# Marcus-Forte/moptimizer_0

Hardware: NVIDIA B200
Metric: point2point_linearized_residuals_per_sec (higher is better)
Workload: dtype f32

## Files before the change

include/mopt_capi.h:

```cpp
#ifndef MOPT_CAPI_H
#define MOPT_CAPI_H

#ifndef __CUDACC_RTC__
#include <stdint.h>
#endif

#ifdef __cplusplus
extern "C" {
#endif

#define MOPT_MAX_PARAMETERS 16
#define MOPT_MAX_OUTPUTS 4
#define MOPT_MAX_COSTS 8
#define MOPT_MAX_TRACE 1024
#define MOPT_NCCL_ID_BYTES 128

#if defined(__GNUC__)
#define MOPT_API __attribute__((visibility("default")))
#else
#define MOPT_API
#endif

typedef struct mopt_ctx mopt_ctx;
typedef struct mopt_store mopt_store;

typedef enum mopt_status {
  MOPT_OK = 0,
  MOPT_ERR_INVALID_ARGUMENT = 1,
  MOPT_ERR_CUDA = 2,
  MOPT_ERR_COMM = 3,
  MOPT_ERR_UNSUPPORTED = 4,
  MOPT_ERR_OUT_OF_MEMORY = 5
} mopt_status;

typedef enum mopt_optimization_status {
  MOPT_CONVERGED = 0,
  MOPT_MAXIMUM_ITERATIONS_REACHED = 1,
  MOPT_SMALL_DELTA = 2,
  MOPT_NUMERIC_ERROR = 3,
  MOPT_FATAL_ERROR = 4
} mopt_optimization_status;

typedef enum mopt_dtype { MOPT_F32 = 0, MOPT_F64 = 1 } mopt_dtype;

typedef enum mopt_model {
  MOPT_MODEL_POINT2POINT = 0,
  MOPT_MODEL_EXP_CURVE = 1,
  MOPT_MODEL_MICHAELIS_MENTEN = 2,
  MOPT_MODEL_PINHOLE = 3,
  MOPT_MODEL_POWELL = 4,
  MOPT_MODEL_POINT_DIST = 5,
  MOPT_MODEL_PINHOLE_DISTORT = 6,
  MOPT_MODEL_COUNT_
} mopt_model;
#define MOPT_MODEL_USER_BASE 1000

typedef enum mopt_jacobian {
  MOPT_JAC_ANALYTICAL = 0,
  MOPT_JAC_FORWARD = 1,
  MOPT_JAC_CENTRAL = 2
} mopt_jacobian;

typedef enum mopt_p2p_variant {
  MOPT_P2P_EXACT = 0,
  MOPT_P2P_REFTEST = 1,
  MOPT_P2P_REFTEST_COLMAJOR = 2,
  MOPT_P2P_LEFT = 3
} mopt_p2p_variant;

typedef enum mopt_manifold { MOPT_MANIFOLD_ADDITIVE = 0, MOPT_MANIFOLD_SO3_LEFT = 1 } mopt_manifold;

typedef enum mopt_loss {
  MOPT_LOSS_NONE = 0,
  MOPT_LOSS_GEMAN_MCCLURE = 1,
  MOPT_LOSS_HUBER = 2
} mopt_loss;

typedef struct mopt_problem {
  int32_t model;
  int32_t variant;
  int32_t num_parameters;
  int32_t num_outputs;
  int32_t jacobian;
  int32_t compute_dtype;
  int32_t loss;
  int32_t has_covariance;
  double loss_param;
  double covariance[MOPT_MAX_OUTPUTS * MOPT_MAX_OUTPUTS];
  double consts[32];
  int32_t manifold;
  int32_t flags;
} mopt_problem;
typedef enum mopt_problem_flags {
  MOPT_FLAG_GENERIC_KERNEL = 1,
  MOPT_FLAG_STABLE_FD = 2,
  MOPT_FLAG_REFERENCE_FLOAT_GUARD = 4
} mopt_problem_flags;

typedef struct mopt_lm_options {
  int32_t max_iterations;
  int32_t lm_max_iterations;
  double lambda_factor;
  int32_t scalar_dtype;
  int32_t speculative;
  int32_t flags;
  int32_t reserved;
} mopt_lm_options;
typedef enum mopt_lm_flags { MOPT_LM_STAGNATION_STOP = 1 } mopt_lm_flags;

typedef struct mopt_lm_trial {
  int32_t outer_iteration, k, accepted, reserved;
  double y0, yi, rho, lambda, nu;
} mopt_lm_trial;

typedef struct mopt_lm_report {
  int32_t status;
  int32_t executed_iterations;
  int32_t num_trials;
  int32_t num_passes;
  double final_cost;
  mopt_lm_trial trials[MOPT_MAX_TRACE];
} mopt_lm_report;

typedef struct mopt_synth {
  uint64_t seed;
  int64_t first_index;
  double gt[MOPT_MAX_PARAMETERS];
  double lo[3], hi[3];
  int64_t n_total;
  double noise_sigma;
  double outlier_fraction, outlier_range;
  double consts[32];
} mopt_synth;

MOPT_API const char* mopt_last_error(void);
MOPT_API const char* mopt_version(void);
MOPT_API int mopt_device_count(int* count);

MOPT_API int mopt_ctx_create(int device, mopt_ctx** out);
MOPT_API int mopt_ctx_create_sharded(int device, int rank, int world_size, const void* nccl_unique_id, mopt_ctx** out);
MOPT_API int mopt_comm_unique_id(void* out_id);
#define MOPT_PEER_HANDLE_BYTES 64
MOPT_API int mopt_ctx_peer_handle(mopt_ctx* ctx, void* out_handle);
MOPT_API int mopt_ctx_open_peers(mopt_ctx* ctx, const void* handles_in_rank_order);
MOPT_API int mopt_ctx_set_exchange_enabled(mopt_ctx* ctx, int enabled);
MOPT_API int mopt_ctx_destroy(mopt_ctx* ctx);
MOPT_API int mopt_ctx_synchronize(mopt_ctx* ctx);
MOPT_API int mopt_ctx_stream(mopt_ctx* ctx, uint64_t* out_stream);
MOPT_API int mopt_ctx_set_launch(mopt_ctx* ctx, int ctas_per_sm, int threads);

MOPT_API int mopt_store_create(mopt_ctx* ctx, int model, int dtype, int64_t n, mopt_store** out);
MOPT_API int mopt_store_destroy(mopt_store* store);
MOPT_API int mopt_store_size(const mopt_store* store, int64_t* n);
MOPT_API int mopt_store_upload(mopt_store* store, int group, const void* host, int host_dtype, int64_t host_stride,
                      int64_t first, int64_t count);
MOPT_API int mopt_store_download(mopt_store* store, int group, void* host, int host_dtype, int64_t first, int64_t count);
MOPT_API int mopt_store_generate(mopt_store* store, const mopt_synth* desc);

MOPT_API int mopt_linearize(mopt_ctx* ctx, mopt_store* store, const mopt_problem* problem, const double* x, double* H,
                   double* b, double* sum);
MOPT_API int mopt_compute_cost(mopt_ctx* ctx, mopt_store* store, const mopt_problem* problem, const double* x, double* sum);
MOPT_API int mopt_linearize_async(mopt_ctx* ctx, mopt_store* store, const mopt_problem* problem, const double* x);
MOPT_API int mopt_ctx_result(mopt_ctx* ctx, int num_parameters, double* H, double* b, double* sum);

MOPT_API int mopt_upload_and_linearize(mopt_ctx* ctx, mopt_store* store, const mopt_problem* problem, const void* host_a,
                              const void* host_b, int host_dtype, int64_t count, const double* x, double* H,
                              double* b, double* sum);

MOPT_API int mopt_lm_minimize(mopt_ctx* ctx, int n_costs, mopt_store* const* stores, const mopt_problem* problems,
                     const mopt_lm_options* options, double* x, mopt_lm_report* report);
MOPT_API void mopt_lm_default_options(mopt_lm_options* options);

MOPT_API int mopt_so3_convert6dof(const double* x, double* T16_rowmajor);
MOPT_API int mopt_ldlt_solve(int n, const double* A_colmajor, const double* rhs, double* out);

typedef struct mopt_nn_index mopt_nn_index;
MOPT_API int mopt_nn_index_create(mopt_ctx* ctx, const void* host_xyz, int host_dtype, int index_dtype, int64_t m,
                                  double max_distance, mopt_nn_index** out);
MOPT_API int mopt_nn_index_destroy(mopt_nn_index* index);
MOPT_API int mopt_store_set_target(mopt_store* store, mopt_nn_index* index);
MOPT_API int mopt_store_reassociate(mopt_store* store, const double* x, int64_t* matched);

MOPT_API int mopt_cloud_read_text(const char* path, int columns, int keep, int host_dtype, int pinned, void** out,
                                  int64_t* n);
MOPT_API int mopt_cloud_write_binary(const char* path, const void* data, int host_dtype, int keep, int64_t n);
MOPT_API int mopt_cloud_read_binary(const char* path, int pinned, int* host_dtype, int* keep, void** out, int64_t* n);
MOPT_API int mopt_cloud_free(void* ptr, int pinned);

typedef struct mopt_user_model_desc {
  int32_t num_parameters;
  int32_t num_outputs;
// ... 29 lines not shown
```

moptimizer_0_b200/capi.py:

```python
from __future__ import annotations

import ctypes as C
import os
from typing import Optional, Sequence

import numpy as np

_PKG = os.path.dirname(os.path.abspath(__file__))
LIB_PATH = os.path.join(_PKG, "libmopt_b200.so")

MAX_PARAMETERS, MAX_OUTPUTS, MAX_COSTS, MAX_TRACE, NCCL_ID_BYTES = 16, 4, 8, 1024, 128
OK = 0
F32, F64 = 0, 1
(MODEL_POINT2POINT, MODEL_EXP_CURVE, MODEL_MICHAELIS_MENTEN, MODEL_PINHOLE, MODEL_POWELL,
 MODEL_POINT_DIST, MODEL_PINHOLE_DISTORT) = range(7)
JAC_ANALYTICAL, JAC_FORWARD, JAC_CENTRAL = range(3)
P2P_EXACT, P2P_REFTEST, P2P_REFTEST_COLMAJOR, P2P_LEFT = range(4)
MANIFOLD_ADDITIVE, MANIFOLD_SO3_LEFT = 0, 1
FLAG_GENERIC_KERNEL = 1
FLAG_STABLE_FD = 2
FLAG_REFERENCE_FLOAT_GUARD = 4
LM_STAGNATION_STOP = 1
LOSS_NONE, LOSS_GEMAN_MCCLURE, LOSS_HUBER = range(3)
STATUS = ["CONVERGED", "MAXIMUM_ITERATIONS_REACHED", "SMALL_DELTA", "NUMERIC_ERROR", "FATAL_ERROR"]
MODEL_SHAPE = {
    MODEL_POINT2POINT: (6, 3, 3, 3), MODEL_EXP_CURVE: (2, 1, 1, 1), MODEL_MICHAELIS_MENTEN: (2, 1, 1, 1),
    MODEL_PINHOLE: (6, 2, 3, 2), MODEL_POWELL: (4, 4, 0, 0), MODEL_POINT_DIST: (0, 3, 3, 3),
    MODEL_PINHOLE_DISTORT: (15, 2, 3, 2),
}

EXPORTS = [
    "mopt_last_error", "mopt_version", "mopt_device_count", "mopt_ctx_create", "mopt_ctx_create_sharded",
    "mopt_comm_unique_id", "mopt_ctx_destroy", "mopt_ctx_synchronize", "mopt_ctx_stream", "mopt_ctx_set_launch",
    "mopt_store_create", "mopt_store_destroy", "mopt_store_size", "mopt_store_upload", "mopt_store_download",
    "mopt_store_generate", "mopt_linearize", "mopt_compute_cost", "mopt_linearize_async", "mopt_ctx_result",
    "mopt_upload_and_linearize", "mopt_lm_minimize", "mopt_lm_default_options", "mopt_so3_convert6dof",
    "mopt_ldlt_solve", "mopt_host_alloc", "mopt_host_free",
    "mopt_cloud_read_text", "mopt_cloud_write_binary", "mopt_cloud_read_binary", "mopt_cloud_free",
    "mopt_nn_index_create", "mopt_nn_index_destroy", "mopt_store_set_target", "mopt_store_reassociate",
    "mopt_ctx_peer_handle", "mopt_ctx_open_peers", "mopt_ctx_set_exchange_enabled",
    "mopt_user_model_compile", "mopt_user_model_release", "mopt_user_model_log",
    "mopt_measure_peaks", "mopt_measure_h2d",
]
MODEL_USER_BASE = 1000
PEER_HANDLE_BYTES = 64


class Problem(C.Structure):
    _fields_ = [("model", C.c_int32), ("variant", C.c_int32), ("num_parameters", C.c_int32),
                ("num_outputs", C.c_int32), ("jacobian", C.c_int32), ("compute_dtype", C.c_int32),
                ("loss", C.c_int32), ("has_covariance", C.c_int32), ("loss_param", C.c_double),
                ("covariance", C.c_double * (MAX_OUTPUTS * MAX_OUTPUTS)), ("consts", C.c_double * 32),
                ("manifold", C.c_int32), ("flags", C.c_int32)]


class LmOptions(C.Structure):
    _fields_ = [("max_iterations", C.c_int32), ("lm_max_iterations", C.c_int32), ("lambda_factor", C.c_double),
                ("scalar_dtype", C.c_int32), ("speculative", C.c_int32), ("flags", C.c_int32),
                ("reserved", C.c_int32)]


class LmTrial(C.Structure):
    _fields_ = [("outer_iteration", C.c_int32), ("k", C.c_int32), ("accepted", C.c_int32), ("reserved", C.c_int32),
                ("y0", C.c_double), ("yi", C.c_double), ("rho", C.c_double), ("lambda_", C.c_double),
                ("nu", C.c_double)]


_TRIAL_DTYPE = np.dtype([("outer_iteration", "<i4"), ("k", "<i4"), ("accepted", "<i4"), ("reserved", "<i4"),
                         ("y0", "<f8"), ("yi", "<f8"), ("rho", "<f8"), ("lambda_", "<f8"), ("nu", "<f8")])


class LmReport(C.Structure):
    _fields_ = [("status", C.c_int32), ("executed_iterations", C.c_int32), ("num_trials", C.c_int32),
                ("num_passes", C.c_int32), ("final_cost", C.c_double), ("trials", LmTrial * MAX_TRACE)]


class Synth(C.Structure):
    _fields_ = [("seed", C.c_uint64), ("first_index", C.c_int64), ("gt", C.c_double * MAX_PARAMETERS),
                ("lo", C.c_double * 3), ("hi", C.c_double * 3), ("n_total", C.c_int64),
                ("noise_sigma", C.c_double), ("outlier_fraction", C.c_double), ("outlier_range", C.c_double),
                ("consts", C.c_double * 32)]


class UserModelDesc(C.Structure):
    _fields_ = [("num_parameters", C.c_int32), ("num_outputs", C.c_int32), ("ncomp_a", C.c_int32),
                ("ncomp_b", C.c_int32), ("has_jacobian", C.c_int32), ("set_size", C.c_int32),
                ("rot_offset", C.c_int32), ("reserved", C.c_int32)]


class Peaks(C.Structure):
    _fields_ = [("fp32_fma_tflops", C.c_double), ("fp32_fma2_tflops", C.c_double),
                ("issue_gwarp_inst_per_s", C.c_double), ("hbm_read_gbs", C.c_double), ("reserved", C.c_double * 4)]


class MoptError(RuntimeError):
    def __init__(self, code: int, msg: str):
        super().__init__(f"mopt error {code}: {msg}")
        self.code = code


_lib = None


def lib():
    global _lib
# ... 128 lines not shown
    @property
    def handle(self):
        return self._h

    def peer_handle(self) -> bytes:
        buf = C.create_string_buffer(PEER_HANDLE_BYTES)
        check(lib().mopt_ctx_peer_handle(self._h, C.cast(buf, C.c_void_p)))
        return buf.raw

    def open_peers(self, handles_in_rank_order: Sequence[bytes]):
        blob = b"".join(bytes(h) for h in handles_in_rank_order)
        buf = C.create_string_buffer(blob, len(blob))
        check(lib().mopt_ctx_open_peers(self._h, C.cast(buf, C.c_void_p)))

    def set_exchange_enabled(self, enabled: bool):
        check(lib().mopt_ctx_set_exchange_enabled(self._h, 1 if enabled else 0))

    def synchronize(self):
        check(lib().mopt_ctx_synchronize(self._h))

    def stream(self) -> int:
        s = C.c_uint64(0)
        check(lib().mopt_ctx_stream(self._h, C.byref(s)))
        return s.value

    def measure_peaks(self) -> dict:
        p = Peaks()
        check(lib().mopt_measure_peaks(self._h, C.byref(p)))
        return {"fp32_fma_tflops": p.fp32_fma_tflops, "fp32_fma2_tflops": p.fp32_fma2_tflops,
                "issue_gwarp_inst_per_s": p.issue_gwarp_inst_per_s, "hbm_read_gbs": p.hbm_read_gbs}

    def measure_h2d(self, nbytes: int = 1 << 30, seconds: float = 1.0) -> float:
        g = C.c_double(0)
        check(lib().mopt_measure_h2d(self._h, int(nbytes), float(seconds), C.byref(g)))
        return g.value

    def set_launch(self, ctas_per_sm: int = 0, threads: int = 0):
        check(lib().mopt_ctx_set_launch(self._h, ctas_per_sm, threads))

    def close(self):
        if self._h:
            lib().mopt_ctx_destroy(self._h)
            self._h = C.c_void_p()

    def linearize(self, store: "Store", problem: Problem, x):
        P = problem.num_parameters
        xs = np.ascontiguousarray(np.asarray(x, dtype=np.float64))
        H = np.zeros((P, P), dtype=np.float64)
        b = np.zeros(P, dtype=np.float64)
        s = C.c_double(0)
        check(lib().mopt_linearize(self._h, store.handle, C.byref(problem), _dp(xs), _dp(H), _dp(b), C.byref(s)))
        return H, b, s.value

    def compute_cost(self, store: "Store", problem: Problem, x) -> float:
        xs = np.ascontiguousarray(np.asarray(x if len(x) else [0.0], dtype=np.float64))
        s = C.c_double(0)
        check(lib().mopt_compute_cost(self._h, store.handle, C.byref(problem), _dp(xs), C.byref(s)))
        return s.value

    def linearize_async(self, store: "Store", problem: Problem, xs: np.ndarray):
        check(lib().mopt_linearize_async(self._h, store.handle, C.byref(problem), _dp(xs)))

    def result(self, P: int):
        H = np.zeros((P, P), dtype=np.float64)
        b = np.zeros(P, dtype=np.float64)
        s = C.c_double(0)
        check(lib().mopt_ctx_result(self._h, P, _dp(H), _dp(b), C.byref(s)))
        return H, b, s.value

    def upload_and_linearize(self, store: "Store", problem: Problem, host_a: np.ndarray, host_b: np.ndarray, x):
        assert host_a.dtype == host_b.dtype and host_a.dtype in (np.float32, np.float64)
        P = problem.num_parameters
        xs = np.ascontiguousarray(np.asarray(x, dtype=np.float64))
        H = np.zeros((P, P), dtype=np.float64)
        b = np.zeros(P, dtype=np.float64)
        s = C.c_double(0)
        dt = F32 if host_a.dtype == np.float32 else F64
        check(lib().mopt_upload_and_linearize(self._h, store.handle, C.byref(problem), host_a.ctypes.data,
                                              host_b.ctypes.data, dt, store.n, _dp(xs), _dp(H), _dp(b), C.byref(s)))
        return H, b, s.value

    def lm_minimize(self, stores: Sequence["Store"], problems: Sequence[Problem], x0, max_iterations: int = 15,
                    lm_iterations: int = 3, scalar_dtype: int = F64, speculative: bool = True,
                    stagnation_stop: bool = True) -> "LmResult":
        n = len(stores)
        hs = (C.c_void_p * n)(*[s.handle for s in stores])
        ps = (Problem * n)(*problems)
        opt = self.__dict__.get("_lm_options")
        if opt is None:
            opt = self._lm_options = LmOptions()
            lib().mopt_lm_default_options(C.byref(opt))
        opt.max_iterations, opt.lm_max_iterations = max_iterations, lm_iterations
        opt.scalar_dtype, opt.speculative = scalar_dtype, 1 if speculative else 0
        opt.flags = LM_STAGNATION_STOP if stagnation_stop else 0
        x = np.array(x0, dtype=np.float64)
        rep = self.__dict__.get("_lm_report")
        if rep is None:
            rep = self._lm_report = LmReport()
        check(lib().mopt_lm_minimize(self._h, n, hs, ps, C.byref(opt), _dp(x), C.byref(rep)))
        return LmResult(x, rep)


class LmResult:
    def __init__(self, x: np.ndarray, rep: LmReport):
        self.x = x
        self.status = STATUS[rep.status]
        self.executed_iterations = rep.executed_iterations
        self.num_passes = rep.num_passes
        self.final_cost = rep.final_cost
        self._raw = C.string_at(C.addressof(rep) + LmReport.trials.offset, rep.num_trials * _TRIAL_DTYPE.itemsize)
        self._trials_arr = None
        self._trace = None

    @property
    def _trials(self) -> np.ndarray:
        if self._trials_arr is None:
            self._trials_arr = np.frombuffer(self._raw, dtype=_TRIAL_DTYPE)
        return self._trials_arr

    @property
    def trace(self) -> np.ndarray:
        if self._trace is None:
            t = self._trials
            self._trace = np.stack([t[f].astype(np.float64) for f in
                                    ("outer_iteration", "k", "y0", "yi", "rho", "lambda_", "nu", "accepted")],
                                   axis=1).reshape(len(t), 8)
        return self._trace

    @property
    def sequence(self) -> str:
        return "".join("A" if a else "R" for a in self._trials["accepted"])


class Store:

    def __init__(self, ctx: Context, model: int, n: int, dtype: int = F32):
        self.ctx, self.model, self.n, self.dtype = ctx, model, int(n), dtype
        self._h = C.c_void_p()
        check(lib().mopt_store_create(ctx.handle, model, dtype, int(n), C.byref(self._h)))

    @property
    def handle(self):
        return self._h

    def upload(self, group: int, host: np.ndarray, first: int = 0, stride: int = 0):
        host = np.ascontiguousarray(host)
        if host.dtype not in (np.float32, np.float64):
            host = host.astype(np.float64)
        ncomp = MODEL_SHAPE[self.model][2 + group]
        count = host.size // (stride if stride else ncomp)
        dt = F32 if host.dtype == np.float32 else F64
        check(lib().mopt_store_upload(self._h, group, host.ctypes.data, dt, stride, first, count))

    def download(self, group: int, dtype=np.float64, first: int = 0, count: Optional[int] = None) -> np.ndarray:
        ncomp = MODEL_SHAPE[self.model][2 + group]
        count = self.n - first if count is None else count
        out = np.zeros((count, ncomp), dtype=dtype)
        dt = F32 if out.dtype == np.float32 else F64
        check(lib().mopt_store_download(self._h, group, out.ctypes.data, dt, first, count))
        return out

    def generate(self, seed: int, gt: Sequence[float], lo=(0, 0, 0), hi=(10, 10, 10), first_index: int = 0,
                 n_total: int = 0, noise_sigma: float = 0.0, outlier_fraction: float = 0.0,
                 outlier_range: float = 0.0, consts=None):
        d = Synth()
        d.seed, d.first_index, d.n_total = seed, first_index, n_total
        for i, v in enumerate(gt):
            d.gt[i] = float(v)
        for k in range(3):
            d.lo[k], d.hi[k] = float(lo[k]), float(hi[k])
        d.noise_sigma, d.outlier_fraction, d.outlier_range = noise_sigma, outlier_fraction, outlier_range
        if consts is not None:
            for i, v in enumerate(np.asarray(consts, dtype=np.float64).reshape(-1)):
                d.consts[i] = float(v)
        check(lib().mopt_store_generate(self._h, C.byref(d)))

    def close(self):
# ... 82 lines not shown
```

moptimizer_0_b200/csrc/mopt_capi.cu:

```cuda
#include <dlfcn.h>

#include <cmath>
#include <atomic>
#include <chrono>
#include <cstdlib>
#include <cstring>
#include <mutex>

#include "mopt_internal.h"

using namespace mopt;

namespace {
thread_local std::string g_last_error;
}
namespace mopt {
void set_last_error(const std::string& msg) { g_last_error = msg; }
int store_upload_async(mopt_store* st, int group, const void* host, int host_dtype, int64_t host_stride, int64_t first,
                       int64_t count);
}

namespace {
struct NcclApi {
  typedef struct ncclComm* comm_t;
  struct unique_id { char internal[MOPT_NCCL_ID_BYTES]; };
  int (*GetUniqueId)(unique_id*) = nullptr;
  int (*CommInitRank)(comm_t*, int, unique_id, int) = nullptr;
  int (*CommDestroy)(comm_t) = nullptr;
  int (*AllReduce)(const void*, void*, size_t, int, int, comm_t, cudaStream_t) = nullptr;
  const char* (*GetErrorString)(int) = nullptr;
  bool ok = false;
  std::string why;
};
NcclApi& nccl() {
  static NcclApi api;
  static std::once_flag once;
  std::call_once(once, [] {
    const char* names[] = {getenv("MOPT_NCCL_LIB"), "libnccl.so.2", "libnccl.so"};
    void* h = nullptr;
    for (const char* n : names) {
      if (!n) continue;
      h = dlopen(n, RTLD_NOW | RTLD_GLOBAL);
      if (h) break;
    }
    if (!h) {
      api.why = std::string("cannot dlopen libnccl: ") + (dlerror() ? dlerror() : "?");
      return;
    }
    api.GetUniqueId = reinterpret_cast<decltype(api.GetUniqueId)>(dlsym(h, "ncclGetUniqueId"));
    api.CommInitRank = reinterpret_cast<decltype(api.CommInitRank)>(dlsym(h, "ncclCommInitRank"));
    api.CommDestroy = reinterpret_cast<decltype(api.CommDestroy)>(dlsym(h, "ncclCommDestroy"));
    api.AllReduce = reinterpret_cast<decltype(api.AllReduce)>(dlsym(h, "ncclAllReduce"));
    api.GetErrorString = reinterpret_cast<decltype(api.GetErrorString)>(dlsym(h, "ncclGetErrorString"));
    api.ok = api.GetUniqueId && api.CommInitRank && api.CommDestroy && api.AllReduce && api.GetErrorString;
    if (!api.ok) api.why = "libnccl is missing required symbols";
  });
  return api;
}
constexpr int kNcclFloat64 = 8;
constexpr int kNcclSum = 0;

#define MOPT_NCCL_TRY(expr)                                                                       \
  do {                                                                                            \
    int _r = (expr);                                                                              \
    if (_r != 0) {                                                                                \
      set_last_error(std::string(#expr) + " failed: " + nccl().GetErrorString(_r));               \
      return MOPT_ERR_COMM;                                                                       \
    }                                                                                             \
  } while (0)
}

namespace {

__global__ void setup_kernel(CostSlot* slot, XArg x) { setup_cost(slot->cost, x.v, &slot->pb, threadIdx.x, blockDim.x); }

__global__ void lm_init_kernel(LmState* st, CostSlot* slots, LmInit in) {
  __shared__ LmStepShared s_sh;
  lm_init_warp(st, slots, in, &s_sh, threadIdx.x);
}

__device__ long long g_step_prof[8];

__global__ void lm_step_kernel(LmState* st, const PassResult* trial, CostSlot* slots, int* flag, const int* xerr, int prof,
                               int P, int scalar_f32) {
  __shared__ LmStepShared s_sh;
  const int lane = threadIdx.x;
  if (*reinterpret_cast<const volatile int*>(xerr)) {
    if (lane == 0) {
      if (!st->done) lm_finish(st, MOPT_FATAL_ERROR);
      *flag = 1;
    }
    return;
  }
  long long stamps[16] = {0};
  const int done = lm_step_warp(st, trial, slots, &s_sh, lane, P, scalar_f32 != 0, LmStepIo{}, prof ? stamps : nullptr);
  if (lane == 0) {
    *flag = done;
    if (prof && stamps[3] - stamps[2] > 1000)
      for (int i = 0; i < 6; ++i) g_step_prof[i] = stamps[i];
  }
}

__global__ void ldlt_warp_test_kernel(int n, const double* A, const double* rhs, double* out) {
  __shared__ LmSolveScratch sc;
  const int lane = threadIdx.x;
  for (int i = lane; i < n * n; i += 32) sc.A[i] = A[i];
  if (lane < n) sc.nb[lane] = rhs[lane];
  __syncwarp();
  if (n == 6) ldlt_solve_warp<double, 6>(n, sc.A, sc.nb, sc.d, sc.tmp, sc.y, sc.tr, lane);
  else ldlt_solve_warp<double>(n, sc.A, sc.nb, sc.d, sc.tmp, sc.y, sc.tr, lane);
  if (lane < n) out[lane] = sc.d[lane];
}

__global__ void peer_reduce_kernel(XSlot* local, int world, unsigned long long seq, PassResult* out, int npk,
                                   const int* mode_ptr, int mode_override, int* err, int* err_dev) {
  const int mode = mode_override >= 0 ? mode_override : *mode_ptr;
  if (mode == PASS_SKIP) return;
  if (*reinterpret_cast<const volatile int*>(err_dev)) return;
  const int base = int(seq & 1ull) * kMaxWorld;
  __shared__ int s_ok;
  if (threadIdx.x == 0) {
    bool ok = true;
    const long long t0 = clock64();
    for (int r = 0; r < world && ok; ++r) {
      const unsigned long long* flag = &local[base + r].seq;
      for (;;) {
        unsigned long long v;
        asm volatile("ld.acquire.sys.global.u64 %0, [%1];" : "=l"(v) : "l"(flag) : "memory");
        if (v == seq) break;
        if (clock64() - t0 > 20000000000LL) {
          ok = false;
          break;
        }
        __nanosleep(64);
      }
    }
    if (!ok) {
      *err = 1;
      *err_dev = 1;
    }
    s_ok = ok ? 1 : 0;
    __threadfence_system();
  }
  __syncthreads();
  if (!s_ok) return;
  for (int k = threadIdx.x; k < npk; k += blockDim.x) {
    double s = 0.0;
    for (int r = 0; r < world; ++r) s += *reinterpret_cast<volatile double*>(&local[base + r].v[k]);
    out->v[k] = s;
  }
}

__global__ void ldlt_test_kernel(int n, double* A, const double* rhs, double* out) { ldlt_solve_dev<double>(n, A, rhs, out); }

}

namespace {

int validate_problem(const mopt_store* st, const mopt_problem* p, bool need_linearize) {
  MOPT_REQUIRE(st && p, "null store/problem");
  MOPT_REQUIRE(p->model == st->model, "problem.model differs from the store's model");
  const ModelShape sh = model_shape(p->model);
  MOPT_REQUIRE(sh.P >= 0, "unknown model kind");
  MOPT_REQUIRE(p->num_parameters == sh.P, "num_parameters does not match the builtin model");
  MOPT_REQUIRE(p->num_outputs == sh.O, "num_outputs does not match the builtin model");
  MOPT_REQUIRE(p->compute_dtype == MOPT_F32 || p->compute_dtype == MOPT_F64, "bad compute dtype");
  MOPT_REQUIRE(p->loss >= MOPT_LOSS_NONE && p->loss <= MOPT_LOSS_HUBER, "unknown loss kind");
  MOPT_REQUIRE(p->jacobian >= MOPT_JAC_ANALYTICAL && p->jacobian <= MOPT_JAC_CENTRAL, "unknown jacobian mode");
  if (need_linearize) {
    MOPT_REQUIRE(sh.P > 0, "this model has no parameters; only mopt_compute_cost is defined for it");
    if (p->jacobian == MOPT_JAC_ANALYTICAL && !sh.has_analytical) {
      set_last_error("Non implemented non-jacobian model function `f_df` being used.");
      return MOPT_ERR_UNSUPPORTED;
    }
  }
  if (p->model == MOPT_MODEL_POINT2POINT)
    MOPT_REQUIRE(p->variant >= MOPT_P2P_EXACT && p->variant <= MOPT_P2P_LEFT, "unknown point2point variant");
  MOPT_REQUIRE(p->manifold == MOPT_MANIFOLD_ADDITIVE || p->manifold == MOPT_MANIFOLD_SO3_LEFT, "unknown manifold");
  if (p->manifold == MOPT_MANIFOLD_SO3_LEFT)
    MOPT_REQUIRE(p->model == MOPT_MODEL_POINT2POINT || p->model == MOPT_MODEL_PINHOLE ||
                     p->model == MOPT_MODEL_PINHOLE_DISTORT ||
                     (p->model >= MOPT_MODEL_USER_BASE && user_model_rot_offset(p->model) >= 0),
                 "MOPT_MANIFOLD_SO3_LEFT needs a model whose x[3..5] is a rotation vector");
  if (p->has_covariance) {
    const int O = sh.O;
    for (int r = 0; r < O; ++r)
      for (int c = 0; c < r; ++c)
        if (p->covariance[r + c * O] != p->covariance[c + r * O]) {
          set_last_error("covariance must be symmetric (only the upper triangle of H is accumulated)");
          return MOPT_ERR_UNSUPPORTED;
        }
  }
  return MOPT_OK;
}

void fill_cost(const mopt_problem* p, CostDev* c) {
  std::memset(c, 0, sizeof(*c));
  c->model = p->model; c->variant = p->variant; c->P = p->num_parameters; c->O = p->num_outputs;
  c->jacobian = p->jacobian; c->loss = p->loss; c->has_cov = p->has_covariance ? 1 : 0;
  c->compute_dtype = p->compute_dtype; c->loss_param = p->loss_param;
  c->manifold = p->manifold;
  c->rot_offset = (p->model == MOPT_MODEL_POINT2POINT || p->model == MOPT_MODEL_PINHOLE ||
                   p->model == MOPT_MODEL_PINHOLE_DISTORT) ? 3 : -1;
  if (p->model >= MOPT_MODEL_USER_BASE) c->rot_offset = user_model_rot_offset(p->model);
  c->so3_guard = ((p->flags & MOPT_FLAG_REFERENCE_FLOAT_GUARD) && p->compute_dtype == MOPT_F32) ? kSo3GuardF32 : kSo3GuardF64;
  const int O = p->num_outputs;
  for (int i = 0; i < O * O; ++i) c->cov[i] = p->has_covariance ? p->covariance[i] : ((i % (O + 1) == 0) ? 1.0 : 0.0);
  std::memcpy(c->consts, p->consts, sizeof(c->consts));
}

int stage_cost(mopt_ctx* ctx, int i, const mopt_problem* p) {
  CostDev c;
  fill_cost(p, &c);
  if (ctx->cached_valid[i] && std::memcmp(&c, &ctx->cached_cost[i], sizeof(c)) == 0) return MOPT_OK;
  MOPT_CUDA_TRY(cudaStreamSynchronize(ctx->stream));
  ctx->h_slot->cost = c;
  MOPT_CUDA_TRY(cudaMemcpyAsync(&ctx->d_slots[i].cost, &ctx->h_slot->cost, sizeof(CostDev), cudaMemcpyHostToDevice, ctx->stream));
  MOPT_CUDA_TRY(cudaStreamSynchronize(ctx->stream));
  ctx->cached_cost[i] = c;
  ctx->cached_valid[i] = true;
  return MOPT_OK;
}

PassArgs make_args(mopt_ctx* ctx, const mopt_store* st, int slot, int accumulate, int mode_override) {
  PassArgs a;
  std::memset(&a, 0, sizeof(a));
  for (int s = 0; s < kMaxStreams; ++s) a.streams.p[s] = st->streams[s];
  a.n = st->n;
  a.pb = &ctx->d_slots[slot].pb;
  a.cost = &ctx->d_slots[slot].cost;
  a.partials = ctx->d_partials;
  a.ticket = ctx->d_ticket;
  a.out = ctx->d_trial;
  a.accumulate = accumulate;
  a.mode_ptr = &ctx->d_lm->pass_mode;
  a.mode_override = mode_override;
  a.masked = st->may_have_invalid ? 1 : 0;
  return a;
}

bool can_fuse_setup(const mopt_ctx* ctx, const mopt_problem* p, const mopt_store* st) {
  static const int env = [] {
    const char* e = getenv("MOPT_FUSED_SETUP");
    return (e && e[0]) ? (e[0] == '0' ? 0 : 1) : -1;
  }();
  if (env == 0) return false;
  if (p->model == MOPT_MODEL_EXP_CURVE && p->jacobian != MOPT_JAC_ANALYTICAL && st->dtype == MOPT_F32 &&
      p->compute_dtype == MOPT_F32 && !(p->flags & MOPT_FLAG_GENERIC_KERNEL) && !p->has_covariance &&
      !st->may_have_invalid && ctx->threads != 1024)
    return true;
  return p->model == MOPT_MODEL_POINT2POINT && p->jacobian == MOPT_JAC_ANALYTICAL &&
         p->manifold == MOPT_MANIFOLD_ADDITIVE;
}

int launch_pass(mopt_ctx* ctx, const mopt_store* st, const mopt_problem* p, int slot, int accumulate, int mode_override,
                bool push, const XArg* fused_x = nullptr) {
  PassArgs a = make_args(ctx, st, slot, accumulate, mode_override);
  if (fused_x) {
    a.fused_setup = 1;
    a.x = *fused_x;
  }
  if (push && ctx->world > 1 && ctx->peers_open && ctx->exchange_enabled) {
    for (int r = 0; r < ctx->world; ++r) a.peer.base[r] = ctx->peer_base[r];
    a.peer.world = ctx->world;
    a.peer.rank = ctx->rank;
    a.peer.push = 1;
    a.peer.fused = ctx->fused_consumer ? 1 : 0;
    a.peer.err = ctx->d_xerr;
    a.peer.err_dev = ctx->d_xerr_dev;
    a.peer.seq = ++ctx->xseq;
  }
  PassLaunch L{ctx->stream, ctx->num_sms, ctx->ctas_per_sm, ctx->threads};
  L.affine_fd = (p->compute_dtype == MOPT_F32) ? !(p->flags & MOPT_FLAG_GENERIC_KERNEL)
                                               : ((p->flags & MOPT_FLAG_STABLE_FD) && !(p->flags & MOPT_FLAG_GENERIC_KERNEL));
  L.identity_cov = !p->has_covariance;
  if (p->model >= MOPT_MODEL_USER_BASE)
    return launch_user(L, ctx->device, p->model, p->jacobian != MOPT_JAC_ANALYTICAL, st->dtype, p->compute_dtype, a);
  if (p->model == MOPT_MODEL_POINT2POINT && p->jacobian == MOPT_JAC_ANALYTICAL)
    return launch_p2p_moment(L, st->dtype, p->compute_dtype, p->loss,
                             p->variant == MOPT_P2P_EXACT || p->variant == MOPT_P2P_LEFT, a);
  if (p->model == MOPT_MODEL_POINT2POINT && !(p->flags & MOPT_FLAG_GENERIC_KERNEL) &&
      !(st->dtype == MOPT_F64 && p->compute_dtype == MOPT_F32))
    return launch_p2p_moment(L, st->dtype, p->compute_dtype, p->loss, false, a);
  if (p->model == MOPT_MODEL_PINHOLE_DISTORT) return launch_wide(L, p->model, st->dtype, p->compute_dtype, a);
  return launch_dense(L, p->model, p->jacobian != MOPT_JAC_ANALYTICAL, st->dtype, p->compute_dtype, a);
}

int allreduce_trial(mopt_ctx* ctx, int P, int mode_override) {
  if (ctx->world <= 1 || !ctx->exchange_enabled) return MOPT_OK;
  if (ctx->peers_open) {
    if (ctx->fused_consumer) return MOPT_OK;
    peer_reduce_kernel<<<1, 64, 0, ctx->stream>>>(ctx->d_xbuf, ctx->world, ctx->xseq, ctx->d_trial, packed_size(P),
                                                  &ctx->d_lm->pass_mode, mode_override, ctx->d_xerr, ctx->d_xerr_dev);
    MOPT_CUDA_TRY(cudaGetLastError());
    return MOPT_OK;
  }
  if (!ctx->nccl_comm) {
    set_last_error("sharded context has neither a NCCL communicator nor an open peer exchange");
    return MOPT_ERR_COMM;
  }
  MOPT_NCCL_TRY(nccl().AllReduce(ctx->d_trial, ctx->d_trial, size_t(packed_size(P)), kNcclFloat64, kNcclSum,
                                 static_cast<NcclApi::comm_t>(ctx->nccl_comm), ctx->stream));
  return MOPT_OK;
}

void unpack_result(const PassResult& r, int P, double* H, double* b, double* sum) {
  if (H)
    for (int i = 0; i < P; ++i)
      for (int j = i; j < P; ++j) {
        const double v = r.v[tri_index(P, i, j)];
        H[i + j * P] = v;
        H[j + i * P] = v;
      }
  if (b)
    for (int i = 0; i < P; ++i) b[i] = r.v[P * (P + 1) / 2 + i];
  if (sum) *sum = r.v[packed_size(P) - 1];
}

int check_exchange_alive(const mopt_ctx* ctx) {
  if (ctx->h_xerr && *reinterpret_cast<volatile int*>(ctx->h_xerr)) {
    set_last_error("an earlier peer exchange on this context timed out (a rank died); destroy the context");
    return MOPT_ERR_COMM;
  }
  return MOPT_OK;
}

int enqueue_pass(mopt_ctx* ctx, mopt_store* st, const mopt_problem* p, const double* x, int mode) {
  MOPT_TRY(check_exchange_alive(ctx));
  MOPT_CUDA_TRY(cudaSetDevice(ctx->device));
  MOPT_TRY(stage_cost(ctx, 0, p));
  const int P = p->num_parameters;
  XArg xa;
  std::memset(&xa, 0, sizeof(xa));
  if (P > 0) {
    MOPT_REQUIRE(x != nullptr, "null parameter vector");
    for (int i = 0; i < P; ++i) xa.v[i] = x[i];
  }
  if (can_fuse_setup(ctx, p, st)) {
    MOPT_TRY(launch_pass(ctx, st, p, 0, 0, mode, true, &xa));
  } else {
    setup_kernel<<<1, 32, 0, ctx->stream>>>(&ctx->d_slots[0], xa);
    MOPT_CUDA_TRY(cudaGetLastError());
    if (user_model_has_setup(p->model))
      MOPT_TRY(launch_user_setup(ctx->stream, ctx->device, p->model, &ctx->d_slots[0], nullptr, xa.v, P));
    MOPT_TRY(launch_pass(ctx, st, p, 0, 0, mode, true));
  }
  MOPT_TRY(allreduce_trial(ctx, P, mode));
  return MOPT_OK;
}

}

namespace mopt {
int setup_slot(mopt_ctx* ctx, int slot, const mopt_problem* problem, const double* x) {
  MOPT_TRY(stage_cost(ctx, slot, problem));
  XArg xa;
  std::memset(&xa, 0, sizeof(xa));
  for (int i = 0; i < problem->num_parameters; ++i) xa.v[i] = x[i];
  setup_kernel<<<1, 32, 0, ctx->stream>>>(&ctx->d_slots[slot], xa);
  MOPT_CUDA_TRY(cudaGetLastError());
  if (user_model_has_setup(problem->model))
    MOPT_TRY(launch_user_setup(ctx->stream, ctx->device, problem->model, &ctx->d_slots[slot], nullptr, xa.v,
                               problem->num_parameters));
  return MOPT_OK;
}
}

namespace {

int fetch_result(mopt_ctx* ctx, int P, double* H, double* b, double* sum) {
  MOPT_CUDA_TRY(cudaMemcpyAsync(ctx->h_result, ctx->d_trial, sizeof(double) * packed_size(P), cudaMemcpyDeviceToHost, ctx->stream));
  MOPT_CUDA_TRY(cudaStreamSynchronize(ctx->stream));
  if (ctx->h_xerr && *reinterpret_cast<volatile int*>(ctx->h_xerr)) {
    set_last_error("peer exchange timed out waiting for another rank");
    return MOPT_ERR_COMM;
  }
  unpack_result(*ctx->h_result, P, H, b, sum);
  return MOPT_OK;
}

int finish_lm(mopt_ctx* ctx, int P, double* x, mopt_lm_report* report, bool on_host = false) {
  LmState* hs = ctx->h_lm;
  constexpr int kFirstTrials = 48;
  const size_t first = offsetof(LmState, trials) + sizeof(mopt_lm_trial) * kFirstTrials;
  if (!on_host) {
    MOPT_CUDA_TRY(cudaMemcpyAsync(hs, ctx->d_lm, first, cudaMemcpyDeviceToHost, ctx->stream));
    MOPT_CUDA_TRY(cudaStreamSynchronize(ctx->stream));
  }
  if (!on_host && hs->num_trials > kFirstTrials) {
    const int more = (hs->num_trials < MOPT_MAX_TRACE ? hs->num_trials : MOPT_MAX_TRACE) - kFirstTrials;
    MOPT_CUDA_TRY(cudaMemcpyAsync(reinterpret_cast<char*>(hs) + first, reinterpret_cast<const char*>(ctx->d_lm) + first,
                                  sizeof(mopt_lm_trial) * size_t(more), cudaMemcpyDeviceToHost, ctx->stream));
    MOPT_CUDA_TRY(cudaStreamSynchronize(ctx->stream));
  }
  if (ctx->h_xerr && *reinterpret_cast<volatile int*>(ctx->h_xerr)) {
    set_last_error("peer exchange timed out waiting for another rank; this context cannot be used any more");
    return MOPT_ERR_COMM;
  }
  if (!hs->done) {
    set_last_error("internal error: the LM state machine did not terminate within its slot budget");
    return MOPT_ERR_CUDA;
  }
  for (int i = 0; i < P; ++i) x[i] = hs->x[i];
  report->status = hs->status;
  report->executed_iterations = hs->executed;
  report->num_trials = hs->num_trials < MOPT_MAX_TRACE ? hs->num_trials : MOPT_MAX_TRACE;
  report->num_passes = hs->num_passes;
  report->final_cost = hs->cur.v[packed_size(P) - 1];
  std::memcpy(report->trials, hs->trials, sizeof(mopt_lm_trial) * size_t(report->num_trials));
  return MOPT_OK;
}

int ctx_alloc(mopt_ctx* ctx) {
  MOPT_CUDA_TRY(cudaSetDevice(ctx->device));
  cudaDeviceProp prop;
  MOPT_CUDA_TRY(cudaGetDeviceProperties(&prop, ctx->device));
  ctx->num_sms = prop.multiProcessorCount;
  MOPT_CUDA_TRY(cudaStreamCreateWithFlags(&ctx->stream, cudaStreamNonBlocking));
  MOPT_CUDA_TRY(cudaStreamCreateWithFlags(&ctx->copy_stream, cudaStreamNonBlocking));
  MOPT_CUDA_TRY(cudaMalloc(&ctx->d_partials, sizeof(double) * kMaxRaw * kMaxGrid));
  MOPT_CUDA_TRY(cudaMalloc(&ctx->d_ticket, sizeof(unsigned int)));
  MOPT_CUDA_TRY(cudaMemset(ctx->d_ticket, 0, sizeof(unsigned int)));
// ... 322 lines not shown
    static const int64_t mono_max = [] {
      const char* e = getenv("MOPT_LM_MONO");
      if (e && e[0] == '0') return int64_t(0);
      const char* m = getenv("MOPT_LM_MONO_MAX");
      return (m && m[0]) ? int64_t(atoll(m)) : int64_t(1) << 22;
    }();
    const mopt_problem& p0 = problems[0];
    const bool moment_path = p0.model == MOPT_MODEL_POINT2POINT &&
                             (p0.jacobian == MOPT_JAC_ANALYTICAL ||
                              (!(p0.flags & MOPT_FLAG_GENERIC_KERNEL) && !(stores[0]->dtype == MOPT_F64 && p0.compute_dtype == MOPT_F32)));
    if (n_costs == 1 && ctx->world == 1 && !has_update && !any_user_setup && moment_path && stores[0]->n <= mono_max &&
        !(stores[0]->dtype == MOPT_F64 && p0.compute_dtype == MOPT_F32)) {
      PassArgs a = make_args(ctx, stores[0], 0, 0, -1);
      PassLaunch L{ctx->stream, ctx->num_sms, ctx->ctas_per_sm, ctx->threads};
      MonoArgs m;
      m.st = ctx->d_lm;
      m.host_st = ctx->d_lm_host;
      m.host_flag = ctx->d_flags;
      reinterpret_cast<volatile int*>(ctx->h_flags)[0] = 0;
      static const int generic_p = [] { const char* e = getenv("MOPT_LM_GENERIC_P"); return (e && e[0] == '1') ? 1 : 0; }();
      m.generic_p = generic_p;
      ctx->h_lm->done = 0;
      m.slots = ctx->d_slots;
      m.rt_words = ctx->d_gen;
      const int64_t slots64 = int64_t(opt.max_iterations) * (int64_t(opt.lm_max_iterations) + 1) + 2;
      m.max_slots = int(slots64 < INT32_MAX ? slots64 : INT32_MAX);
      m.init = in;
      m.gen_base = ctx->mono_gen;
      ctx->mono_gen += (unsigned long long)(m.max_slots) + 2ull;
      m.dbg = nullptr;
      static const bool trace = [] { const char* e = getenv("MOPT_LM_MONO_TRACE"); return e && e[0] == '1'; }();
      unsigned long long* d_dbg = nullptr;
      if (trace) {
        MOPT_CUDA_TRY(cudaMalloc(&d_dbg, sizeof(unsigned long long) * 512));
        MOPT_CUDA_TRY(cudaMemsetAsync(d_dbg, 0, sizeof(unsigned long long) * 512, ctx->stream));
        m.dbg = d_dbg;
      }
      const bool qrot = p0.jacobian == MOPT_JAC_ANALYTICAL && (p0.variant == MOPT_P2P_EXACT || p0.variant == MOPT_P2P_LEFT);
      const auto h0 = std::chrono::steady_clock::now();
      MOPT_TRY(launch_p2p_lm_mono(L, stores[0]->dtype, p0.compute_dtype, p0.loss, qrot, a, m));
      const auto h1 = std::chrono::steady_clock::now();
      if (trace) {
        MOPT_CUDA_TRY(cudaStreamSynchronize(ctx->stream));
      } else {
        for (int spins = 0;; ++spins) {
          if (reinterpret_cast<volatile int*>(ctx->h_flags)[0] != 0) break;
          if ((spins & 4095) == 4095) {
            const cudaError_t q = cudaStreamQuery(ctx->stream);
            if (q == cudaSuccess) break;
            if (q != cudaErrorNotReady) MOPT_CUDA_TRY(q);
          }
        }
        std::atomic_thread_fence(std::memory_order_acquire);
      }
      const auto h2 = std::chrono::steady_clock::now();
      if (d_dbg) {
        std::fprintf(stderr, "mono host: launch call %.1f us, wait for the kernel %.1f us\n",
                     std::chrono::duration<double, std::micro>(h1 - h0).count(),
                     std::chrono::duration<double, std::micro>(h2 - h1).count());
        unsigned long long h[512];
        MOPT_CUDA_TRY(cudaMemcpy(h, d_dbg, sizeof(h), cudaMemcpyDeviceToHost));
        cudaFree(d_dbg);
        std::fprintf(stderr, "mono kernel: init %.2f us, loop %.2f us (CTA 0), last data CTA leaves %+.2f us after CTA 0\n",
                     (h[501] - h[500]) * 1e-3, (h[502] - h[501]) * 1e-3, (double(h[503]) - double(h[502])) * 1e-3);
        for (int s = 0; s < 64 && h[s * 4 + 3]; ++s)
          std::fprintf(stderr, "mono trial %2d: pass %6.2f us  step %6.2f us  open %5.2f us  (next begins +%6.2f us)\n", s,
                       (h[s * 4 + 1] - h[s * 4]) * 1e-3, (h[s * 4 + 2] - h[s * 4 + 1]) * 1e-3, (h[s * 4 + 3] - h[s * 4 + 2]) * 1e-3,
                       h[(s + 1) * 4] ? (double(h[(s + 1) * 4]) - double(h[s * 4 + 3])) * 1e-3 : 0.0);
        for (int s = 0; s < 15 && h[256 + s * 16 + 5]; ++s) {
          const unsigned long long* q = h + 256 + s * 16;
          std::fprintf(stderr, "mono step %2d (cycles): stage-in %llu  state machine %llu  solve+propose %llu  setup %llu  write-back %llu",
                       s, q[1] - q[0], q[2] - q[1], q[3] - q[2], q[4] - q[3], q[5] - q[4]);
          if (q[10] > q[6] && q[6] > q[2])
            std::fprintf(stderr, "  | build A %llu  factor %llu  forward %llu  D %llu  backward %llu  propose %llu", q[6] - q[2],
                         q[7] - q[6], q[8] - q[7], q[9] - q[8], q[10] - q[9], q[3] - q[10]);
          if (q[11] > q[3]) std::fprintf(stderr, "  | barrier opened %llu cycles into the setup", q[11] - q[3]);
          std::fprintf(stderr, "\n");
        }
      }
      return finish_lm(ctx, P, x, report, true);
    }
  }

  MOPT_TRY(launch_init());
  static const bool step_prof = [] { const char* e = getenv("MOPT_LM_MONO_TRACE"); return e && e[0] == '1'; }();
  const int64_t max_slots = int64_t(opt.max_iterations) * (int64_t(opt.lm_max_iterations) + 1) + 2;
  const int kBatch = 2;
  int64_t enq = 0;
  auto slot_index = [&](int64_t slot) { return int(slot % ctx->flags_capacity); };
  auto enqueue_batch = [&](int par, int64_t* last_slot) -> int {
    *last_slot = -1;
    for (int s = 0; s < kBatch && enq < max_slots; ++s, ++enq) {
      ctx->h_flags[slot_index(enq)] = 0;
      for (int c = 0; c < n_costs; ++c) MOPT_TRY(enqueue_reassociate(stores[c], &ctx->d_slots[c].pb, ctx->d_lm));
      for (int c = 0; c < n_costs; ++c)
        MOPT_TRY(launch_pass(ctx, stores[c], &problems[c], c, c > 0 ? 1 : 0, -1, c == n_costs - 1));
      MOPT_TRY(allreduce_trial(ctx, P, -1));
      lm_step_kernel<<<1, 32, 0, ctx->stream>>>(ctx->d_lm, ctx->d_trial, ctx->d_slots, ctx->d_flags + slot_index(enq),
                                                ctx->d_xerr_dev, step_prof ? 1 : 0, in.P, in.scalar_f32);
      MOPT_CUDA_TRY(cudaGetLastError());
      MOPT_TRY(user_setups());
      *last_slot = enq;
    }
    if (*last_slot >= 0) MOPT_CUDA_TRY(cudaEventRecord(ctx->ev_batch[par], ctx->stream));
    return MOPT_OK;
  };
  int par = 0;
  int64_t cur_last = -1, next_last = -1;
  MOPT_TRY(enqueue_batch(par, &cur_last));
  while (cur_last >= 0) {
    MOPT_TRY(enqueue_batch(par ^ 1, &next_last));
    MOPT_CUDA_TRY(cudaEventSynchronize(ctx->ev_batch[par]));
    if (reinterpret_cast<volatile int*>(ctx->h_flags)[slot_index(cur_last)] != 0) break;
    if (ctx->h_xerr && *reinterpret_cast<volatile int*>(ctx->h_xerr)) break;
    par ^= 1;
    cur_last = next_last;
  }
  MOPT_CUDA_TRY(cudaStreamSynchronize(ctx->stream));
  if (step_prof) {
    long long q[8];
    MOPT_CUDA_TRY(cudaMemcpyFromSymbol(q, g_step_prof, sizeof(q)));
    std::fprintf(stderr, "lm_step_kernel (cycles): stage-in %lld  state machine %lld  solve+propose %lld  setup %lld  write-back %lld\n",
                 q[1] - q[0], q[2] - q[1], q[3] - q[2], q[4] - q[3], q[5] - q[4]);
  }

  return finish_lm(ctx, P, x, report);
}
MOPT_ABI_CATCH

int mopt_so3_convert6dof(const double* x, double* T) try {
  MOPT_REQUIRE(x && T, "null argument");
  const double w[3] = {x[3], x[4], x[5]};
  const double n = std::sqrt(w[0] * w[0] + w[1] * w[1] + w[2] * w[2]);
  double R[9] = {1, 0, 0, 0, 1, 0, 0, 0, 1};
  if (n > 10.0 * 2.220446049250313e-16) {
    const double a[3] = {w[0] / n, w[1] / n, w[2] / n};
    const double K[9] = {0, -a[2], a[1], a[2], 0, -a[0], -a[1], a[0], 0};
    const double s = std::sin(n), c = std::cos(n);
    for (int r = 0; r < 3; ++r)
      for (int col = 0; col < 3; ++col) {
        double kk = 0;
        for (int k = 0; k < 3; ++k) kk += K[r * 3 + k] * K[k * 3 + col];
        R[r * 3 + col] += s * K[r * 3 + col] + (1.0 - c) * kk;
      }
  }
  for (int r = 0; r < 3; ++r) {
    for (int c = 0; c < 3; ++c) T[r * 4 + c] = R[r * 3 + c];
    T[r * 4 + 3] = x[r];
  }
  T[12] = T[13] = T[14] = 0.0;
  T[15] = 1.0;
  return MOPT_OK;
}
MOPT_ABI_CATCH

int mopt_ldlt_solve(int n, const double* A, const double* rhs, double* out) try {
  MOPT_REQUIRE(n >= 1 && n <= kMaxP && A && rhs && out, "bad argument");
  double *dA = nullptr, *dr = nullptr, *dout = nullptr;
  MOPT_CUDA_TRY(cudaMalloc(&dA, sizeof(double) * n * n));
  MOPT_CUDA_TRY(cudaMalloc(&dr, sizeof(double) * n));
  MOPT_CUDA_TRY(cudaMalloc(&dout, sizeof(double) * n));
  MOPT_CUDA_TRY(cudaMemcpy(dA, A, sizeof(double) * n * n, cudaMemcpyHostToDevice));
  MOPT_CUDA_TRY(cudaMemcpy(dr, rhs, sizeof(double) * n, cudaMemcpyHostToDevice));
  double out_warp[kMaxP], *dA2 = nullptr;
  ldlt_warp_test_kernel<<<1, 32>>>(n, dA, dr, dout);
  MOPT_CUDA_TRY(cudaGetLastError());
  MOPT_CUDA_TRY(cudaMemcpy(out_warp, dout, sizeof(double) * n, cudaMemcpyDeviceToHost));
  MOPT_CUDA_TRY(cudaMalloc(&dA2, sizeof(double) * n * n));
  MOPT_CUDA_TRY(cudaMemcpy(dA2, A, sizeof(double) * n * n, cudaMemcpyHostToDevice));
  ldlt_test_kernel<<<1, 1>>>(n, dA2, dr, dout);
  MOPT_CUDA_TRY(cudaGetLastError());
  MOPT_CUDA_TRY(cudaMemcpy(out, dout, sizeof(double) * n, cudaMemcpyDeviceToHost));
  cudaFree(dA); cudaFree(dA2); cudaFree(dr); cudaFree(dout);
  if (std::memcmp(out, out_warp, sizeof(double) * n) != 0) {
    set_last_error("internal error: warp-cooperative and serial LDL^T disagree");
    return MOPT_ERR_CUDA;
  }
  return MOPT_OK;
}
MOPT_ABI_CATCH
// ... 16 lines not shown
```

moptimizer_0_b200/csrc/mopt_common.cuh:

```cuda
#pragma once

#ifndef __CUDACC_RTC__
#include <cuda_runtime.h>
#include <stdint.h>

#include <cstdio>
#include <exception>
#include <new>
#include <string>
#else
typedef int int32_t;
typedef unsigned int uint32_t;
typedef long long int64_t;
typedef unsigned long long uint64_t;
#endif

#include "mopt_capi.h"

namespace mopt {

#ifndef __CUDACC_RTC__
void set_last_error(const std::string& msg);

#define MOPT_CUDA_TRY(expr)                                                                  \
  do {                                                                                       \
    cudaError_t _e = (expr);                                                                 \
    if (_e != cudaSuccess) {                                                                 \
      (void)cudaGetLastError();  \
      ::mopt::set_last_error(std::string(#expr) + " failed: " + cudaGetErrorString(_e) +     \
                             " (" __FILE__ ":" + std::to_string(__LINE__) + ")");            \
      return (_e == cudaErrorMemoryAllocation) ? MOPT_ERR_OUT_OF_MEMORY : MOPT_ERR_CUDA;     \
    }                                                                                        \
  } while (0)

#define MOPT_REQUIRE(cond, msg)                                                  \
  do {                                                                           \
    if (!(cond)) {                                                               \
      ::mopt::set_last_error(std::string("invalid argument: ") + (msg));         \
      return MOPT_ERR_INVALID_ARGUMENT;                                          \
    }                                                                            \
  } while (0)

#define MOPT_ABI_CATCH                                                        \
  catch (const std::bad_alloc&) {                                             \
    ::mopt::set_last_error("out of host memory");                             \
    return MOPT_ERR_OUT_OF_MEMORY;                                            \
  }                                                                           \
  catch (const std::exception& e) {                                           \
    ::mopt::set_last_error(std::string("internal error: ") + e.what());       \
    return MOPT_ERR_INVALID_ARGUMENT;                                         \
  }                                                                           \
  catch (...) {                                                               \
    ::mopt::set_last_error("internal error: unknown exception");              \
    return MOPT_ERR_INVALID_ARGUMENT;                                         \
  }

#define MOPT_TRY(expr)              \
  do {                              \
    int _s = (expr);                \
    if (_s != MOPT_OK) return _s;   \
  } while (0)
#endif

constexpr int kMaxP = MOPT_MAX_PARAMETERS;
constexpr int kMaxO = MOPT_MAX_OUTPUTS;
constexpr int kMaxStreams = 6;
constexpr int kSetSize = 24;
constexpr int kMaxRaw = 160;
constexpr int kMaxSets = 1 + 2 * kMaxP;
constexpr int kPackedMax = kMaxP * (kMaxP + 1) / 2 + kMaxP + 1;
constexpr int kMaxGrid = 148 * 8;

enum PassMode : int { PASS_SKIP = 0, PASS_LINEARIZE = 1, PASS_COST = 2 };

struct ParamBlock {
  double x[kMaxP];
  double h[kMaxP];
  double sets[kMaxSets][kSetSize];
  double jaff[4][18];
  double hstep_fwd[kMaxP];
  double hstep_cen[kMaxP];
};

struct CostDev {
  int model, variant, P, O;
  int jacobian, loss, has_cov, compute_dtype;
  double loss_param;
  double cov[kMaxO * kMaxO];
  double consts[32];
  int manifold;
  int rot_offset;
  double so3_guard;
};

struct CostSlot {
  CostDev cost;
  ParamBlock pb;
};

struct XArg {
  double v[kMaxP];
};

struct PassResult {
  double v[kPackedMax];
};

__host__ __device__ inline int packed_size(int P) { return P * (P + 1) / 2 + P + 1; }
__host__ __device__ inline int tri_index(int P, int r, int c) {
  return r * P - r * (r - 1) / 2 + (c - r);
}

struct StreamPtrs {
  const void* p[kMaxStreams];
};

#ifdef __CUDACC__

template <typename T>
__device__ __forceinline__ T shfl_xor(T v, int off) {
  return __shfl_xor_sync(0xffffffffu, v, off);
}

template <int V, typename T>
__device__ __forceinline__ T warp_reduce_transpose(T (&v)[V]) {
  static_assert(V >= 1 && V <= 32 && (V & (V - 1)) == 0, "V must be a power of two <= 32");
  const int lane = threadIdx.x & 31;
  int off = 16;
#pragma unroll
  for (int cnt = V; cnt > 1; cnt >>= 1) {
    const bool up = (lane & off) != 0;
    const int half = cnt >> 1;
#pragma unroll
    for (int k = 0; k < half; ++k) {
      const T keep = up ? v[k + half] : v[k];
      const T send = up ? v[k] : v[k + half];
      v[k] = keep + shfl_xor(send, off);
    }
    off >>= 1;
  }
  T r = v[0];
#pragma unroll
  for (int o = 16; o >= 1; o >>= 1) {
    if (o <= off) r += shfl_xor(r, o);
  }
  return r;
}

template <int V>
struct Log2 {
  static constexpr int value = 1 + Log2<V / 2>::value;
};
template <>
struct Log2<1> {
  static constexpr int value = 0;
};

__host__ __device__ constexpr int next_pow2(int v) {
  int p = 1;
  while (p < v) p <<= 1;
  return p;
}

__device__ __forceinline__ float4 ld_stream(const float4* p) {
  float4 r;
  asm volatile("ld.global.nc.L1::no_allocate.v4.f32 {%0,%1,%2,%3}, [%4];"
               : "=f"(r.x), "=f"(r.y), "=f"(r.z), "=f"(r.w)
               : "l"(p));
  return r;
}
__device__ __forceinline__ double2 ld_stream(const double2* p) {
  double2 r;
  asm volatile("ld.global.nc.L1::no_allocate.v2.f64 {%0,%1}, [%2];" : "=d"(r.x), "=d"(r.y) : "l"(p));
  return r;
}

__device__ __forceinline__ void lds16_reload(const float* p, float (&v)[4]) {
  const unsigned addr = static_cast<unsigned>(__cvta_generic_to_shared(p));
  asm volatile("ld.shared.v4.f32 {%0,%1,%2,%3}, [%4];" : "=f"(v[0]), "=f"(v[1]), "=f"(v[2]), "=f"(v[3]) : "r"(addr));
}
__device__ __forceinline__ void lds16_reload(const double* p, double (&v)[2]) {
  const unsigned addr = static_cast<unsigned>(__cvta_generic_to_shared(p));
  asm volatile("ld.shared.v2.f64 {%0,%1}, [%2];" : "=d"(v[0]), "=d"(v[1]) : "r"(addr));
}

__host__ __device__ __forceinline__ float fast_rcp(float x) {
#ifdef __CUDA_ARCH__
  float r;
  asm("rcp.approx.ftz.f32 %0, %1;" : "=f"(r) : "f"(x));
  return r;
#else
// ... 73 lines not shown
```

moptimizer_0_b200/csrc/mopt_icp.cu:

```cuda
#include <cmath>
#include <cstring>
#include <vector>

#include "mopt_internal.h"

using namespace mopt;

struct mopt_nn_index {
  mopt_ctx* ctx = nullptr;
  int dtype = MOPT_F64;
  int64_t m = 0;
  double max_dist = 0.0, cell = 0.0;
  double origin[3] = {0, 0, 0};
  int dims[3] = {1, 1, 1};
  int64_t ncells = 1;
  void* d_pts = nullptr;
  int* d_orig = nullptr;
  unsigned int* d_start = nullptr;
  long long* d_matched = nullptr;
};

namespace {

struct GridDesc {
// ... 170 lines not shown
template <typename T>
int build_index(mopt_nn_index* ix, const void* host, int host_dtype) {
  mopt_ctx* ctx = ix->ctx;
  const int64_t m = ix->m;
  const size_t esz = sizeof(T);
  T* d_aos = nullptr;
  MOPT_CUDA_TRY(cudaMalloc(&d_aos, esz * 3 * size_t(m > 0 ? m : 1)));
  if ((host_dtype == MOPT_F32) == (sizeof(T) == 4)) {
    MOPT_CUDA_TRY(cudaMemcpyAsync(d_aos, host, esz * 3 * size_t(m), cudaMemcpyHostToDevice, ctx->stream));
  } else {
    std::vector<T> tmp(size_t(m) * 3);
    if (host_dtype == MOPT_F32) { const float* h = static_cast<const float*>(host); for (size_t i = 0; i < tmp.size(); ++i) tmp[i] = T(h[i]); }
    else { const double* h = static_cast<const double*>(host); for (size_t i = 0; i < tmp.size(); ++i) tmp[i] = T(h[i]); }
    MOPT_CUDA_TRY(cudaMemcpyAsync(d_aos, tmp.data(), esz * 3 * size_t(m), cudaMemcpyHostToDevice, ctx->stream));
    MOPT_CUDA_TRY(cudaStreamSynchronize(ctx->stream));
  }
  const int bb_blocks = 296;
  double* d_part = nullptr;
  MOPT_CUDA_TRY(cudaMalloc(&d_part, sizeof(double) * 6 * bb_blocks));
  bbox_kernel<T><<<bb_blocks, 256, 0, ctx->stream>>>(d_aos, m, d_part);
  MOPT_CUDA_TRY(cudaGetLastError());
  std::vector<double> part(6 * bb_blocks);
  MOPT_CUDA_TRY(cudaMemcpyAsync(part.data(), d_part, sizeof(double) * part.size(), cudaMemcpyDeviceToHost, ctx->stream));
  MOPT_CUDA_TRY(cudaStreamSynchronize(ctx->stream));
  cudaFree(d_part);
  double lo[3] = {1e300, 1e300, 1e300}, hi[3] = {-1e300, -1e300, -1e300};
  for (int b = 0; b < bb_blocks; ++b)
    for (int k = 0; k < 3; ++k) {
      lo[k] = std::fmin(lo[k], part[b * 6 + k]);
      hi[k] = std::fmax(hi[k], part[b * 6 + 3 + k]);
    }
  if (m == 0) for (int k = 0; k < 3; ++k) lo[k] = hi[k] = 0.0;
  double cell = ix->max_dist;
  for (;;) {
    double dims[3], total = 1.0;
    for (int k = 0; k < 3; ++k) {
      dims[k] = std::floor((hi[k] - lo[k]) / cell) + 1.0;
      total *= dims[k];
    }
    if (total <= double(1 << 24)) {
      for (int k = 0; k < 3; ++k) ix->dims[k] = int(dims[k]);
      break;
    }
    cell *= 1.26;
  }
  ix->cell = cell;
  ix->ncells = int64_t(ix->dims[0]) * ix->dims[1] * ix->dims[2];
  for (int k = 0; k < 3; ++k) ix->origin[k] = lo[k];
  GridDesc g;
  for (int k = 0; k < 3; ++k) { g.origin[k] = ix->origin[k]; g.dims[k] = ix->dims[k]; }
  g.inv_cell = 1.0 / cell;

  unsigned int *d_cell_of = nullptr, *d_cursor = nullptr, *d_tiles = nullptr;
  const int ntiles = int((ix->ncells + 1 + kScanTile - 1) / kScanTile);
  MOPT_CUDA_TRY(cudaMalloc(&ix->d_start, sizeof(unsigned int) * size_t(ix->ncells + 1)));
  MOPT_CUDA_TRY(cudaMalloc(&d_cursor, sizeof(unsigned int) * size_t(ix->ncells)));
  MOPT_CUDA_TRY(cudaMalloc(&d_cell_of, sizeof(unsigned int) * size_t(m > 0 ? m : 1)));
  MOPT_CUDA_TRY(cudaMalloc(&d_tiles, sizeof(unsigned int) * size_t(ntiles)));
  MOPT_CUDA_TRY(cudaMemsetAsync(ix->d_start, 0, sizeof(unsigned int) * size_t(ix->ncells + 1), ctx->stream));
  MOPT_CUDA_TRY(cudaMemsetAsync(d_cursor, 0, sizeof(unsigned int) * size_t(ix->ncells), ctx->stream));
  int blocks = int(std::min<int64_t>((m + 255) / 256, 148 * 16));
  if (blocks < 1) blocks = 1;
  count_kernel<T><<<blocks, 256, 0, ctx->stream>>>(d_aos, m, g, ix->d_start, d_cell_of);
  MOPT_CUDA_TRY(cudaGetLastError());
  scan_tiles_kernel<<<ntiles, kScanThreads, 0, ctx->stream>>>(ix->d_start, ix->ncells + 1, d_tiles);
  scan_sums_kernel<<<1, 32, 0, ctx->stream>>>(d_tiles, ntiles);
  scan_add_kernel<<<ntiles, kScanThreads, 0, ctx->stream>>>(ix->d_start, ix->ncells + 1, d_tiles);
  MOPT_CUDA_TRY(cudaGetLastError());
  T* pts = nullptr;
  MOPT_CUDA_TRY(cudaMalloc(&pts, esz * 3 * size_t(m > 0 ? m : 1)));
  MOPT_CUDA_TRY(cudaMalloc(&ix->d_orig, sizeof(int) * size_t(m > 0 ? m : 1)));
  ix->d_pts = pts;
  scatter_kernel<T><<<blocks, 256, 0, ctx->stream>>>(d_aos, m, d_cell_of, ix->d_start, d_cursor, pts, pts + m, pts + 2 * m,
                                                     ix->d_orig);
  MOPT_CUDA_TRY(cudaGetLastError());
  MOPT_CUDA_TRY(cudaStreamSynchronize(ctx->stream));
  cudaFree(d_aos); cudaFree(d_cell_of); cudaFree(d_cursor); cudaFree(d_tiles);
  MOPT_CUDA_TRY(cudaMalloc(&ix->d_matched, sizeof(long long)));
  return MOPT_OK;
}

template <typename ST, typename T>
void launch_reassoc(mopt_store* st, mopt_nn_index* ix, const ParamBlock* pb, const LmState* gate) {
  GridDesc g;
  for (int k = 0; k < 3; ++k) { g.origin[k] = ix->origin[k]; g.dims[k] = ix->dims[k]; }
  g.inv_cell = 1.0 / ix->cell;
  const T* pts = static_cast<const T*>(ix->d_pts);
  int blocks = int(std::min<int64_t>((st->n + 255) / 256, 148 * 32));
  if (blocks < 1) blocks = 1;
  reassociate_kernel<ST, T><<<blocks, 256, 0, st->ctx->stream>>>(
      static_cast<const ST*>(st->streams[0]), static_cast<const ST*>(st->streams[1]), static_cast<const ST*>(st->streams[2]),
      static_cast<ST*>(st->streams[3]), static_cast<ST*>(st->streams[4]), static_cast<ST*>(st->streams[5]), st->n, pb, g,
      ix->max_dist, pts, pts + ix->m, pts + 2 * ix->m, ix->d_orig, ix->d_start, ix->d_matched, gate);
}

}

namespace mopt {

int enqueue_reassociate(mopt_store* st, const ParamBlock* pb, const LmState* gate) {
  mopt_nn_index* ix = st->index;
  if (!ix) return MOPT_OK;
  MOPT_CUDA_TRY(cudaMemsetAsync(ix->d_matched, 0, sizeof(long long), st->ctx->stream));
  if (st->dtype == MOPT_F32 && ix->dtype == MOPT_F32) launch_reassoc<float, float>(st, ix, pb, gate);
  else if (st->dtype == MOPT_F32 && ix->dtype == MOPT_F64) launch_reassoc<float, double>(st, ix, pb, gate);
  else if (st->dtype == MOPT_F64 && ix->dtype == MOPT_F32) launch_reassoc<double, float>(st, ix, pb, gate);
  else launch_reassoc<double, double>(st, ix, pb, gate);
  MOPT_CUDA_TRY(cudaGetLastError());
  st->may_have_invalid = true;
  return MOPT_OK;
}

}

extern "C" {

int mopt_nn_index_create(mopt_ctx* ctx, const void* host_xyz, int host_dtype, int index_dtype, int64_t m,
                         double max_distance, mopt_nn_index** out) try {
  MOPT_REQUIRE(ctx && out && (host_xyz || m == 0), "null argument");
  MOPT_REQUIRE(m >= 0 && m < (int64_t(1) << 31), "target cloud size must be below 2^31");
  MOPT_REQUIRE(max_distance > 0.0 && std::isfinite(max_distance), "max_distance must be positive");
  MOPT_REQUIRE((host_dtype == MOPT_F32 || host_dtype == MOPT_F64) && (index_dtype == MOPT_F32 || index_dtype == MOPT_F64),
               "bad dtype");
  MOPT_CUDA_TRY(cudaSetDevice(ctx->device));
  mopt_nn_index* ix = new mopt_nn_index();
  ix->ctx = ctx;
  ix->dtype = index_dtype;
  ix->m = m;
  ix->max_dist = max_distance;
  const int s = index_dtype == MOPT_F32 ? build_index<float>(ix, host_xyz, host_dtype) : build_index<double>(ix, host_xyz, host_dtype);
  if (s != MOPT_OK) {
    mopt_nn_index_destroy(ix);
    return s;
  }
  *out = ix;
  return MOPT_OK;
}
MOPT_ABI_CATCH

int mopt_nn_index_destroy(mopt_nn_index* ix) try {
  if (!ix) return MOPT_OK;
  cudaSetDevice(ix->ctx->device);
  cudaStreamSynchronize(ix->ctx->stream);
  cudaFree(ix->d_pts); cudaFree(ix->d_orig); cudaFree(ix->d_start); cudaFree(ix->d_matched);
  delete ix;
  return MOPT_OK;
}
MOPT_ABI_CATCH

int mopt_store_set_target(mopt_store* store, mopt_nn_index* index) try {
  MOPT_REQUIRE(store, "null store");
  MOPT_REQUIRE(store->model == MOPT_MODEL_POINT2POINT, "correspondence re-association is defined for point2point stores");
  MOPT_REQUIRE(!index || index->ctx == store->ctx, "index and store live on different contexts");
  store->index = index;
  return MOPT_OK;
}
MOPT_ABI_CATCH

int mopt_store_reassociate(mopt_store* store, const double* x, int64_t* matched) try {
  MOPT_REQUIRE(store && x, "null argument");
  MOPT_REQUIRE(store->index, "no target index attached (mopt_store_set_target)");
  mopt_ctx* ctx = store->ctx;
  MOPT_CUDA_TRY(cudaSetDevice(ctx->device));
  mopt_problem p;
  std::memset(&p, 0, sizeof(p));
  p.model = MOPT_MODEL_POINT2POINT; p.num_parameters = 6; p.num_outputs = 3; p.jacobian = MOPT_JAC_ANALYTICAL;
// ... 13 lines not shown
```

moptimizer_0_b200/csrc/mopt_internal.h:

```cpp
#pragma once

#include <cuda_runtime.h>

#include "mopt_common.cuh"
#include "mopt_lm.cuh"
#include "mopt_lm_mono.cuh"
#include "mopt_models.cuh"
#include "mopt_pass.cuh"

struct mopt_ctx {
  int device = 0;
  int num_sms = 148;
  cudaStream_t stream = nullptr;
  cudaStream_t copy_stream = nullptr;
  double* d_partials = nullptr;
  unsigned int* d_ticket = nullptr;
  mopt::PassResult* d_trial = nullptr;
  mopt::CostSlot* d_slots = nullptr;
  mopt::LmState* d_lm = nullptr;
  mopt::PassResult* h_result = nullptr;
  mopt::LmState* h_lm = nullptr;
  mopt::LmState* d_lm_host = nullptr;
  mopt::CostSlot* h_slot = nullptr;
  int* h_flags = nullptr;
  int* d_flags = nullptr;
  int flags_capacity = 0;
  mopt::CostDev cached_cost[MOPT_MAX_COSTS];
  bool cached_valid[MOPT_MAX_COSTS] = {false};
  void* d_stage[2] = {nullptr, nullptr};
  size_t stage_bytes = 0;
  cudaEvent_t ev_copy[2] = {nullptr, nullptr};
  cudaEvent_t ev_free[2] = {nullptr, nullptr};
  cudaEvent_t ev_batch[2] = {nullptr, nullptr};
  int ctas_per_sm = 0;
  int threads = 0;
  void* nccl_comm = nullptr;
  int rank = 0, world = 1;
  mopt::XSlot* d_xbuf = nullptr;
  mopt::XSlot* peer_base[mopt::kMaxWorld] = {nullptr};
  bool peers_open = false;
  bool exchange_enabled = true;
  bool fused_consumer = true;
  unsigned long long xseq = 0;
  int* h_xerr = nullptr;
  int* d_xerr = nullptr;
  unsigned long long* d_gen = nullptr;
  unsigned long long mono_gen = 0;
  int* d_xerr_dev = nullptr;
};

struct mopt_store {
  mopt_ctx* ctx = nullptr;
  int model = 0;
  int dtype = 0;
  int64_t n = 0;
  int nstreams = 0;
  void* streams[mopt::kMaxStreams] = {nullptr};
  struct mopt_nn_index* index = nullptr;
  bool may_have_invalid = false;
};

namespace mopt {

struct PassLaunch {
  cudaStream_t stream;
  int num_sms;
  int ctas_per_sm;
  int threads;
  bool affine_fd = true;
  bool identity_cov = false;
};

int launch_p2p_moment(const PassLaunch& L, int store_dtype, int compute_dtype, int loss, bool qrot, const PassArgs& a);
int launch_p2p_moment_gen2(const PassLaunch& L, int loss, bool qrot, const PassArgs& a);
int launch_p2p_lm_mono(const PassLaunch& L, int store_dtype, int compute_dtype, int loss, bool qrot, const PassArgs& a,
                       const MonoArgs& m);
int launch_dense(const PassLaunch& L, int model, bool numeric, int store_dtype, int compute_dtype, const PassArgs& a);

int setup_slot(mopt_ctx* ctx, int slot, const mopt_problem* problem, const double* x);
int enqueue_reassociate(mopt_store* st, const ParamBlock* pb, const LmState* gate);

int launch_wide(const PassLaunch& L, int model, int store_dtype, int compute_dtype, const PassArgs& a);

int launch_user(const PassLaunch& L, int device, int model, bool numeric, int store_dtype, int compute_dtype,
                const PassArgs& a);
int launch_user_setup(cudaStream_t stream, int device, int model, CostSlot* slot, const double* x_dev,
                      const double* x_host, int P);
int user_model_rot_offset(int model);
bool user_model_has_setup(int model);

int pick_grid(const void* kernel, int threads, const PassLaunch& L, int64_t work_items);

}
```

moptimizer_0_b200/csrc/mopt_lm.cuh:

```cuda
#pragma once

#include <cstddef>

#include "mopt_common.cuh"
#include "mopt_setup.cuh"

namespace mopt {

enum LmPhase : int { LM_PHASE_LIN = 0, LM_PHASE_TRIAL = 1 };

struct LmState {
  int P, n_costs, max_it, lm_max_it, speculative, scalar_f32;
  double lambda_factor;
  int flags;
  int pad0_;
  double x[kMaxP], xi[kMaxP], delta[kMaxP], x_eval[kMaxP];
  PassResult cur;
  double lambda, nu;
  int it, k, phase, status, done, executed, num_trials, num_passes;
  int pass_mode;
  int pad_;
  mopt_lm_trial trials[MOPT_MAX_TRACE];
};

constexpr int kLmHotWords = int(offsetof(LmState, trials) / 8);
static_assert(offsetof(LmState, trials) % 8 == 0, "LmState hot part is copied in 8-byte words");
static_assert(kPackedMax <= 160, "lm_step_warp_t stages the pass result with five loads per lane");

struct LmInit {
  int P, n_costs, max_it, lm_max_it, speculative, scalar_f32;
  double lambda_factor;
  int flags;
  double x0[kMaxP];
};

#ifdef __CUDACC__

template <typename S>
__device__ inline void ldlt_solve_dev(int n, S* A, const S* rhs, S* out) {
  int tr[kMaxP];
  S tmp[kMaxP], y[kMaxP];
#define MOPT_A(r, c) A[(r) + (c) * n]
  bool zero_matrix = false;
  for (int k = 0; k < n && !zero_matrix; ++k) {
    int piv = k;
    S best = fabs(MOPT_A(k, k));
    for (int i = k + 1; i < n; ++i) {
      const S v = fabs(MOPT_A(i, i));
      if (v > best) { best = v; piv = i; }
    }
    tr[k] = piv;
    if (piv != k) {
      for (int c = 0; c < k; ++c) { const S t = MOPT_A(k, c); MOPT_A(k, c) = MOPT_A(piv, c); MOPT_A(piv, c) = t; }
      for (int r = piv + 1; r < n; ++r) { const S t = MOPT_A(r, k); MOPT_A(r, k) = MOPT_A(r, piv); MOPT_A(r, piv) = t; }
      { const S t = MOPT_A(k, k); MOPT_A(k, k) = MOPT_A(piv, piv); MOPT_A(piv, piv) = t; }
      for (int i = k + 1; i < piv; ++i) { const S t = MOPT_A(i, k); MOPT_A(i, k) = MOPT_A(piv, i); MOPT_A(piv, i) = t; }
    }
    if (k > 0) {
      for (int c = 0; c < k; ++c) tmp[c] = MOPT_A(c, c) * MOPT_A(k, c);
      S s = S(0);
      for (int c = 0; c < k; ++c) s += MOPT_A(k, c) * tmp[c];
      MOPT_A(k, k) -= s;
      for (int r = k + 1; r < n; ++r) {
        S t = S(0);
        for (int c = 0; c < k; ++c) t += MOPT_A(r, c) * tmp[c];
        MOPT_A(r, k) -= t;
      }
    }
    const S akk = MOPT_A(k, k);
    const bool valid = fabs(akk) > S(0);
    if (k == 0 && !valid) {
      for (int j = 0; j < n; ++j) tr[j] = j;
      zero_matrix = true;
      break;
    }
    if (valid)
      for (int r = k + 1; r < n; ++r) MOPT_A(r, k) /= akk;
  }
  for (int i = 0; i < n; ++i) y[i] = rhs[i];
  for (int k = 0; k < n; ++k) { const S t = y[k]; y[k] = y[tr[k]]; y[tr[k]] = t; }
  for (int r = 0; r < n; ++r)
    for (int c = 0; c < r; ++c) y[r] -= MOPT_A(r, c) * y[c];
  const S tol = (sizeof(S) == 4) ? S(1.17549435e-38) : S(2.2250738585072014e-308);
  for (int i = 0; i < n; ++i) y[i] = (fabs(MOPT_A(i, i)) > tol) ? y[i] / MOPT_A(i, i) : S(0);
  for (int r = n - 1; r >= 0; --r)
    for (int c = r + 1; c < n; ++c) y[r] -= MOPT_A(c, r) * y[c];
  for (int k = n - 1; k >= 0; --k) { const S t = y[k]; y[k] = y[tr[k]]; y[tr[k]] = t; }
  for (int i = 0; i < n; ++i) out[i] = y[i];
#undef MOPT_A
}

template <typename S>
__device__ inline S scalar_eps() { return (sizeof(S) == 4) ? S(1.1920928955078125e-07) : S(2.220446049250313e-16); }

template <typename S>
__device__ inline bool is_cost_small(S c) { return fabs(c) < S(8) * scalar_eps<S>(); }

__device__ inline void lm_finish(LmState* st, int status) {
  st->status = status;
  st->executed = st->it;
  st->done = 1;
  st->pass_mode = PASS_SKIP;
}

template <typename S, int NC = 0>
__device__ inline void ldlt_solve_warp(int n_rt, S* A, const S* rhs, S* out, S* tmp, S* y, int* tr, int lane,
                                       long long* prof = nullptr) {
  const int n = NC > 0 ? NC : n_rt;
  unsigned long long perm = 0xFEDCBA9876543210ull;
  auto PH = [&](int i) { return int((perm >> (4 * i)) & 15ull); };
#define MOPT_A(pr, pc) A[(pr) + (pc) * n]
  bool zero_matrix = false;
#pragma unroll
  for (int k = 0; k < n && !zero_matrix; ++k) {
    int piv = k;
// ... 31 lines not shown
    }
    if (valid && lane > k && lane < n) MOPT_A(PH(lane), pk) /= akk;
    __syncwarp();
  }
  if (prof && lane == 0) prof[7] = clock64();
  if (lane == 0) {
    for (int i = 0; i < n; ++i) y[i] = rhs[i];
    for (int k = 0; k < n; ++k) { const S t = y[k]; y[k] = y[tr[k]]; y[tr[k]] = t; }
    for (int r = 0; r < n; ++r) {
      const int pr = PH(r);
      S v = y[r];
      for (int c = 0; c < r; ++c) v -= MOPT_A(pr, PH(c)) * y[c];
      y[r] = v;
    }
  }
  __syncwarp();
  if (prof && lane == 0) prof[8] = clock64();
  if (lane < n) {
    const S tol = (sizeof(S) == 4) ? S(1.17549435e-38) : S(2.2250738585072014e-308);
    const S dd = MOPT_A(PH(lane), PH(lane));
    y[lane] = (fabs(dd) > tol) ? y[lane] / dd : S(0);
  }
  __syncwarp();
  if (prof && lane == 0) prof[9] = clock64();
  if (lane == 0) {
    for (int r = n - 1; r >= 0; --r) {
      const int pr = PH(r);
      S v = y[r];
      for (int c = r + 1; c < n; ++c) v -= MOPT_A(PH(c), pr) * y[c];
      y[r] = v;
    }
    for (int k = n - 1; k >= 0; --k) { const S t = y[k]; y[k] = y[tr[k]]; y[tr[k]] = t; }
    for (int i = 0; i < n; ++i) out[i] = y[i];
  }
  __syncwarp();
  if (prof && lane == 0) prof[10] = clock64();
#undef MOPT_A
}

struct LmSolveScratch {
  double A[kMaxP * kMaxP], nb[kMaxP], d[kMaxP], tmp[kMaxP], y[kMaxP];
  int tr[kMaxP];
};

template <typename S, int PC = 0>
__device__ inline void lm_solve_propose_warp(LmState* st, const CostDev& cost0, LmSolveScratch* sc, int lane,
                                             long long* prof = nullptr) {
  const int P = PC > 0 ? PC : st->P;
  S* A = reinterpret_cast<S*>(sc->A);
  S* nb = reinterpret_cast<S*>(sc->nb);
  S* d = reinterpret_cast<S*>(sc->d);
  const S lam = S(st->lambda);
  for (int e = lane; e < P * P; e += 32) {
    const int r = e % P, c = e / P;
    const S h = S(st->cur.v[r <= c ? tri_index(P, r, c) : tri_index(P, c, r)]);
    A[r + c * P] = (r == c) ? h + lam * h : h;
  }
  if (lane < P) nb[lane] = -S(st->cur.v[P * (P + 1) / 2 + lane]);
  __syncwarp();
  if (prof && lane == 0) prof[6] = clock64();
  ldlt_solve_warp<S, PC>(P, A, nb, d, reinterpret_cast<S*>(sc->tmp), reinterpret_cast<S*>(sc->y), sc->tr, lane, prof);
  if (cost0.manifold == MOPT_MANIFOLD_SO3_LEFT) {
    if (lane == 0) {
      for (int i = 0; i < P; ++i) st->delta[i] = double(d[i]);
      retract_dev(cost0, st->x, st->delta, st->xi, sizeof(S) == 4);
      for (int i = 0; i < P; ++i) st->x_eval[i] = st->xi[i];
    }
  } else if (lane < P) {
    const S dl = d[lane];
    const double xi = double(S(st->x[lane]) + dl);
    st->delta[lane] = double(dl);
    st->xi[lane] = xi;
    st->x_eval[lane] = xi;
  }
  if (lane == 0) {
    st->phase = LM_PHASE_TRIAL;
    st->pass_mode = st->speculative ? PASS_LINEARIZE : PASS_COST;
  }
  __syncwarp();
}

constexpr int kLmCopyTrial = 4;
template <typename S, int PC = 0>
__device__ inline int lm_step_thread(LmState* st, const PassResult* trial, const CostDev& cost0, mopt_lm_trial* trials) {
  if (st->done) return 0;
  const int P = PC > 0 ? PC : st->P;
  const int npk = packed_size(P);
  st->num_passes += 1;
  int copy = 0;
  const PassResult* lin = &st->cur;
  if (st->phase == LM_PHASE_LIN) {
    copy = kLmCopyTrial;
    lin = trial;
  } else {
    const S yi = S(trial->v[npk - 1]);
    const S y0 = S(st->cur.v[npk - 1]);
    if (isnan(yi)) {
      lm_finish(st, MOPT_NUMERIC_ERROR);
      return 0;
    }
    const S lam = S(st->lambda);
    S den = S(0);
    for (int i = 0; i < P; ++i) {
      const S d = S(st->delta[i]);
      den += d * (lam * d - S(st->cur.v[P * (P + 1) / 2 + i]));
    }
    const S rho = (y0 - yi) / den;
    if (st->num_trials < MOPT_MAX_TRACE) {
      mopt_lm_trial& t = trials[st->num_trials];
      t.outer_iteration = st->it; t.k = st->k; t.accepted = !(rho < S(0)); t.reserved = 0;
      t.y0 = double(y0); t.yi = double(yi); t.rho = double(rho); t.lambda = st->lambda; t.nu = st->nu;
    }
    st->num_trials += 1;
    if (rho < S(0)) {
      S m = S(0);
      for (int i = 0; i < P; ++i) m = fmax(m, fabs(S(st->delta[i])));
      if (m < sqrt(scalar_eps<S>())) {
        lm_finish(st, is_cost_small<S>(yi) ? MOPT_CONVERGED : MOPT_SMALL_DELTA);
        return 0;
      }
      st->lambda = double(S(st->nu) * lam);
      st->nu = double(S(2) * S(st->nu));
      st->k += 1;
      if (st->k < st->lm_max_it) {
        return 2;
      }
      st->it += 1;
      if (st->it >= st->max_it) {
        lm_finish(st, MOPT_MAXIMUM_ITERATIONS_REACHED);
        return 0;
      }
    } else {
      for (int i = 0; i < P; ++i) st->x[i] = st->xi[i];
      if ((st->flags & MOPT_LM_STAGNATION_STOP) && yi == y0) {
        S m = S(0);
        for (int i = 0; i < P; ++i) m = fmax(m, fabs(S(st->delta[i])));
        if (m < sqrt(scalar_eps<S>())) {
          lm_finish(st, is_cost_small<S>(yi) ? MOPT_CONVERGED : MOPT_SMALL_DELTA);
          return 0;
        }
      }
      const double v = double(S(2) * rho - S(1));
      const double f = fmax(1.0 / 3.0, 1.0 - v * v * v);
      st->lambda = double(S(double(lam) * f));
      st->it += 1;
      if (st->it >= st->max_it) {
        if (st->speculative) {
          lm_finish(st, MOPT_MAXIMUM_ITERATIONS_REACHED);
          return kLmCopyTrial;
        }
        st->cur.v[npk - 1] = trial->v[npk - 1];
        lm_finish(st, MOPT_MAXIMUM_ITERATIONS_REACHED);
        return 0;
      }
      if (st->speculative) {
        copy = kLmCopyTrial;
        lin = trial;
      } else {
        st->cur.v[npk - 1] = trial->v[npk - 1];
        for (int i = 0; i < P; ++i) st->x_eval[i] = st->x[i];
        st->phase = LM_PHASE_LIN;
        st->pass_mode = PASS_LINEARIZE;
        return 1;
      }
    }
  }
  for (;;) {
    const S y0 = S(lin->v[npk - 1]);
    if (is_cost_small<S>(y0)) {
      lm_finish(st, MOPT_CONVERGED);
      return copy;
    }
    if (st->lambda < 0.0) {
      S mx = S(0);
      for (int i = 0; i < P; ++i) mx = fmax(mx, fabs(S(lin->v[tri_index(P, i, i)])));
      st->lambda = double(S(st->lambda_factor) * mx);
    }
    st->nu = 2.0;
    st->k = 0;
    if (st->lm_max_it > 0) {
      return 2 | copy;
    }
    st->it += 1;
    if (st->it >= st->max_it) {
      lm_finish(st, MOPT_MAXIMUM_ITERATIONS_REACHED);
      return copy;
    }
  }
}

struct LmStepShared {
  LmSolveScratch sc;
  double hot[kLmHotWords];
  PassResult trial;
};

struct LmStepIo {
  bool load_state = true, store_state = true, trial_staged = false;
  const CostDev* cost0 = nullptr;
  unsigned long long* rt_words = nullptr;
  unsigned long long gen_target = 0;
  int* opened = nullptr;
  bool generic_p = false;
  LmState* host_state = nullptr;
  int* host_flag = nullptr;
};

static __device__ __noinline__ void lm_init_warp(LmState* st, CostSlot* slots, const LmInit& in, LmStepShared* sh, int lane,
                                                 bool resident = false, const CostDev* cost0 = nullptr) {
  if (lane == 0) {
    st->P = in.P; st->n_costs = in.n_costs; st->max_it = in.max_it; st->lm_max_it = in.lm_max_it;
    st->speculative = in.speculative; st->scalar_f32 = in.scalar_f32; st->lambda_factor = in.lambda_factor;
    st->flags = in.flags;
    st->pad0_ = 0;
    st->lambda = -1.0; st->nu = 2.0;
    st->it = 0; st->k = 0; st->phase = LM_PHASE_LIN; st->status = MOPT_MAXIMUM_ITERATIONS_REACHED;
    st->done = 0; st->executed = 0; st->num_trials = 0; st->num_passes = 0;
    st->pass_mode = PASS_LINEARIZE;
    st->pad_ = 0;
  }
  if (lane < kMaxP) {
    const double v = lane < in.P ? (in.scalar_f32 ? double(float(in.x0[lane])) : in.x0[lane]) : 0.0;
    st->x[lane] = v; st->xi[lane] = v; st->x_eval[lane] = v; st->delta[lane] = 0.0;
    if (!resident) sh->hot[lane] = v;
  }
  for (int i = lane; i < kPackedMax; i += 32) st->cur.v[i] = 0.0;
  __syncwarp();
  const double* x = resident ? st->x_eval : sh->hot;
  for (int c = 0; c < in.n_costs; ++c)
    setup_cost((c == 0 && cost0) ? *cost0 : slots[c].cost, x, &slots[c].pb, lane, 32, sh->sc.tmp);
}

template <typename S, int PC>
__device__ inline int lm_step_warp_t(LmState* gst, const PassResult* gtrial, CostSlot* slots, LmStepShared* sh, int lane,
                                     int P_rt, const LmStepIo& io, long long* prof = nullptr) {
  LmState* st = reinterpret_cast<LmState*>(sh->hot);
  if (prof && lane == 0) prof[0] = clock64();
  const int npk = packed_size(PC > 0 ? PC : P_rt);
  {
    const double* g = reinterpret_cast<const double*>(gst);
    constexpr int kPerLane = (kLmHotWords + 31) / 32;
    double tmp[kPerLane];
    if (io.load_state) {
#pragma unroll
      for (int q = 0; q < kPerLane; ++q) tmp[q] = (lane + 32 * q < kLmHotWords) ? __ldcg(g + lane + 32 * q) : 0.0;
    }
    double tr0 = 0.0, tr1 = 0.0, tr2 = 0.0, tr3 = 0.0, tr4 = 0.0;
    if (!io.trial_staged) {
      if (lane < npk) tr0 = __ldcg(&gtrial->v[lane]);
      if (lane + 32 < npk) tr1 = __ldcg(&gtrial->v[lane + 32]);
      if (lane + 64 < npk) tr2 = __ldcg(&gtrial->v[lane + 64]);
      if (lane + 96 < npk) tr3 = __ldcg(&gtrial->v[lane + 96]);
      if (lane + 128 < npk) tr4 = __ldcg(&gtrial->v[lane + 128]);
    }
    if (io.load_state) {
#pragma unroll
      for (int q = 0; q < kPerLane; ++q)
        if (lane + 32 * q < kLmHotWords) sh->hot[lane + 32 * q] = tmp[q];
    }
    if (!io.trial_staged) {
      if (lane < npk) sh->trial.v[lane] = tr0;
      if (lane + 32 < npk) sh->trial.v[lane + 32] = tr1;
      if (lane + 64 < npk) sh->trial.v[lane + 64] = tr2;
      if (lane + 96 < npk) sh->trial.v[lane + 96] = tr3;
      if (lane + 128 < npk) sh->trial.v[lane + 128] = tr4;
    }
  }
  __syncwarp();
  if (prof && lane == 0) prof[1] = clock64();
  const CostDev& cost0 = io.cost0 ? *io.cost0 : slots[0].cost;
  int act = 0;
  if (lane == 0) act = lm_step_thread<S, PC>(st, &sh->trial, cost0, io.host_state ? io.host_state->trials : gst->trials);
  act = __shfl_sync(0xffffffffu, act, 0);
  __syncwarp();
  if (act & kLmCopyTrial) {
    for (int i = lane; i < npk; i += 32) st->cur.v[i] = sh->trial.v[i];
    __syncwarp();
    act &= ~kLmCopyTrial;
  }
  if (prof && lane == 0) prof[2] = clock64();
  if (act == 2) {
    lm_solve_propose_warp<S, PC>(st, cost0, &sh->sc, lane, prof);
    __syncwarp();
  }
  if (prof && lane == 0) prof[3] = clock64();
  if (act) {
    const int nc = st->n_costs;
    const SetupEarlyOpen eo{io.rt_words, (io.gen_target << 2) | (unsigned long long)(st->pass_mode), io.opened, prof};
    for (int c = 0; c < nc; ++c)
      setup_cost(c == 0 ? cost0 : slots[c].cost, st->x_eval, &slots[c].pb, lane, 32, sh->sc.tmp,
                 (io.rt_words != nullptr && nc == 1) ? &eo : nullptr);
  }
  __syncwarp();
  if (prof && lane == 0) prof[4] = clock64();
  if (io.store_state || st->done) {
    double* g = reinterpret_cast<double*>(gst);
    for (int i = lane; i < kLmHotWords; i += 32) g[i] = sh->hot[i];
    if (io.host_state) {
      double* h = reinterpret_cast<double*>(io.host_state);
      for (int i = lane; i < kLmHotWords; i += 32) h[i] = sh->hot[i];
      __threadfence_system();
      __syncwarp();
      if (lane == 0 && io.host_flag) *reinterpret_cast<volatile int*>(io.host_flag) = 1;
    }
  }
  __syncwarp();
  if (prof && lane == 0) prof[5] = clock64();
  return st->done;
}
static __device__ __noinline__ int lm_step_warp(LmState* st, const PassResult* trial, CostSlot* slots, LmStepShared* sh, int lane,
                                                int P, bool f32, const LmStepIo& io, long long* prof = nullptr) {
  if (P == 6 && !io.generic_p) {
    return f32 ? lm_step_warp_t<float, 6>(st, trial, slots, sh, lane, P, io, prof)
               : lm_step_warp_t<double, 6>(st, trial, slots, sh, lane, P, io, prof);
  }
  return f32 ? lm_step_warp_t<float, 0>(st, trial, slots, sh, lane, P, io, prof)
             : lm_step_warp_t<double, 0>(st, trial, slots, sh, lane, P, io, prof);
}

#endif
}
```

moptimizer_0_b200/csrc/mopt_pass.cuh:

```cuda
#pragma once

#include "mopt_common.cuh"
#include "mopt_setup.cuh"

namespace mopt {

constexpr int kMaxWorld = 8;
struct XSlot {
  double v[kPackedMax];
  unsigned long long seq;
  unsigned long long pad;
};
struct PeerArgs {
  XSlot* base[kMaxWorld];
  int world, rank, push;
  int fused;
  unsigned long long seq;
  int* err;
  int* err_dev;
};

struct PassArgs {
  PeerArgs peer;
  StreamPtrs streams;
  int64_t n;
  const ParamBlock* pb;
  const CostDev* cost;
  double* partials;
  unsigned int* ticket;
  PassResult* out;
  int accumulate;
  const int* mode_ptr;
  int mode_override;
  int masked;
  int fused_setup;
  int no_ring;
  XArg x;
};

#ifdef __CUDACC__

template <int NRAW, int THREADS>
__device__ __forceinline__ void grid_final_reduce(const double* partials, int G, double* s_tot) {
  constexpr int NW = THREADS / 32;
  const int lane = threadIdx.x & 31, warp = threadIdx.x >> 5;
  constexpr int ROWS = (NRAW + NW - 1) / NW;
  constexpr int RB = ROWS < 4 ? ROWS : 4;
  for (int q0 = 0; q0 < ROWS; q0 += RB) {
    double s[RB];
#pragma unroll
    for (int q = 0; q < RB; ++q) s[q] = 0.0;
    for (int c = lane; c < G; c += 32) {
      double v[RB];
#pragma unroll
      for (int q = 0; q < RB; ++q) {
        const int i = warp + (q0 + q) * NW;
        v[q] = (i < NRAW) ? __ldcg(partials + size_t(i) * G + c) : 0.0;
      }
#pragma unroll
      for (int q = 0; q < RB; ++q) s[q] += v[q];
    }
#pragma unroll
    for (int o = 16; o >= 1; o >>= 1) {
#pragma unroll
      for (int q = 0; q < RB; ++q) s[q] += shfl_xor(s[q], o);
    }
    if (lane == 0) {
#pragma unroll
      for (int q = 0; q < RB; ++q)
        if (warp + (q0 + q) * NW < NRAW) s_tot[warp + (q0 + q) * NW] = s[q];
    }
  }
}

template <int NRAW, int STRIDE, int THREADS, bool MASTER = false>
__device__ __forceinline__ bool grid_reduce_shared(const PassArgs& a, double* s_tot, const double* s_warp) {
  constexpr int NW = THREADS / 32;
  __shared__ bool s_last;
  const int G = MASTER ? int(gridDim.x) - 1 : int(gridDim.x);
  const int bid = MASTER ? int(blockIdx.x) - 1 : int(blockIdx.x);
  for (int i = threadIdx.x; i < NRAW; i += THREADS) {
    double s = 0.0;
#pragma unroll
    for (int w = 0; w < NW; ++w) s += s_warp[w * STRIDE + i];
    a.partials[size_t(i) * G + bid] = s;
  }
  __threadfence();
  __syncthreads();
  if constexpr (MASTER) {
    if (threadIdx.x == 0) atomicAdd(a.ticket, 1u);
    return false;
  } else {
    if (threadIdx.x == 0) {
      const unsigned int t = atomicAdd(a.ticket, 1u);
      s_last = (t == unsigned(G - 1));
    }
    __syncthreads();
    if (!s_last) return false;
  }
  __threadfence();
  grid_final_reduce<NRAW, THREADS>(a.partials, G, s_tot);
  if (threadIdx.x == 0) *a.ticket = 0u;
  __syncthreads();
  return true;
}

template <int NRAW, int V, int NCH, int THREADS, bool MASTER = false>
__device__ __forceinline__ bool grid_reduce(const double (&lane_val)[NCH], const PassArgs& a, double* s_tot,
                                            double* s_warp ) {
  constexpr int SHIFT = 5 - Log2<V>::value;
  const int lane = threadIdx.x & 31, warp = threadIdx.x >> 5;
  if ((lane & ((1 << SHIFT) - 1)) == 0) {
#pragma unroll
    for (int ch = 0; ch < NCH; ++ch) s_warp[warp * (NCH * V) + ch * V + (lane >> SHIFT)] = lane_val[ch];
  }
  __syncthreads();
  return grid_reduce_shared<NRAW, NCH * V, THREADS, MASTER>(a, s_tot, s_warp);
}

__device__ __forceinline__ bool peer_failed(const PassArgs& a) {
// ... 90 lines not shown
  const CT e2 = fma(r0, r0, fma(r1, r1, r2 * r2));
  acc[22] += (masked && (yx != yx)) ? CT(0) : e2;
}

static __device__ __noinline__ void p2p_fused_set0(const CostDev* c, const double* x, double* set) {
  const bool f32 = (c->compute_dtype == MOPT_F32);
  double xs[6];
  for (int i = 0; i < 6; ++i) xs[i] = f32 ? double(float(x[i])) : x[i];
  const double w[3] = {xs[3], xs[4], xs[5]};
  double R[9];
  if (f32) so3_exp_dev<float>(w, R, c->so3_guard); else so3_exp_dev<double>(w, R, c->so3_guard);
  for (int i = 0; i < 9; ++i) set[i] = R[i];
  set[9] = xs[0]; set[10] = xs[1]; set[11] = xs[2];
}
static __device__ __noinline__ void p2p_fused_left_jacobian(const CostDev* c, const double* x, double* Jl) {
  for (int i = 0; i < 9; ++i) Jl[i] = (i % 4 == 0) ? 1.0 : 0.0;
  if (c->variant == MOPT_P2P_EXACT) {
    const double w[3] = {x[3], x[4], x[5]};
    so3_left_jacobian_dev(w, Jl);
  }
}
__device__ inline void p2p_assemble_inner(const double (*jaff)[18], const CostDev* cost, bool has_cov, int tid, int nthreads,
                                          double* scratch) {
  constexpr int P = 6, NH = P * (P + 1) / 2;
  double C[9];
  for (int i = 0; i < 9; ++i) C[i] = has_cov ? cost->cov[i] : ((i % 4 == 0) ? 1.0 : 0.0);
  for (int w = tid; w < NH * 16; w += nthreads) {
    const int e = w >> 4, k = (w >> 2) & 3, l = w & 3;
    int i = 0, rem = e;
    while (rem >= P - i) { rem -= P - i; ++i; }
    const int j = i + rem;
    double s = 0.0;
    if (has_cov) {
      for (int a = 0; a < 3; ++a)
        for (int b = 0; b < 3; ++b) s = __fma_rn(__dmul_rn(jaff[k][a * 6 + i], C[a + 3 * b]), jaff[l][b * 6 + j], s);
    } else {
      for (int a = 0; a < 3; ++a) s = __fma_rn(jaff[k][a * 6 + i], jaff[l][a * 6 + j], s);
    }
    scratch[w] = s;
  }
}
__device__ inline void p2p_assemble_outer(const double* tot, const double (*jaff)[18], const CostDev* cost, bool has_cov,
                                          PassResult* out, int accumulate, int tid, int nthreads, const double* scratch) {
  constexpr int P = 6, NH = P * (P + 1) / 2;
  double C[9];
  for (int i = 0; i < 9; ++i) C[i] = has_cov ? cost->cov[i] : ((i % 4 == 0) ? 1.0 : 0.0);
  double Mt[4][4], St[4][3];
  Mt[0][0] = tot[0];
  for (int k = 0; k < 3; ++k) Mt[0][k + 1] = Mt[k + 1][0] = tot[1 + k];
  Mt[1][1] = tot[4]; Mt[1][2] = Mt[2][1] = tot[5]; Mt[1][3] = Mt[3][1] = tot[6];
  Mt[2][2] = tot[7]; Mt[2][3] = Mt[3][2] = tot[8]; Mt[3][3] = tot[9];
  for (int m = 0; m < 3; ++m) St[0][m] = tot[10 + m];
  for (int k = 0; k < 3; ++k)
    for (int m = 0; m < 3; ++m) St[k + 1][m] = tot[13 + k * 3 + m];
  const int npk = packed_size(P);
  for (int e = tid; e < npk; e += nthreads) {
    double val = 0.0;
    if (e < NH) {
      for (int k = 0; k < 4; ++k)
        for (int l = 0; l < 4; ++l) val = __fma_rn(Mt[k][l], scratch[e * 16 + k * 4 + l], val);
    } else if (e < npk - 1) {
      const int i = e - NH;
      if (has_cov) {
        for (int k = 0; k < 4; ++k)
          for (int a = 0; a < 3; ++a)
            for (int b = 0; b < 3; ++b) val = __fma_rn(__dmul_rn(jaff[k][a * 6 + i], C[a + 3 * b]), St[k][b], val);
      } else {
        for (int k = 0; k < 4; ++k)
          for (int a = 0; a < 3; ++a) val = __fma_rn(jaff[k][a * 6 + i], St[k][a], val);
      }
    } else {
      val = tot[22];
    }
    out->v[e] = accumulate ? out->v[e] + val : val;
  }
}
__device__ inline void p2p_assemble(const double* tot, const double (*jaff)[18], const CostDev* cost, bool has_cov,
                                    PassResult* out, int accumulate, int tid, int nthreads, double* scratch) {
  p2p_assemble_inner(jaff, cost, has_cov, tid, nthreads, scratch);
  __syncthreads();
  p2p_assemble_outer(tot, jaff, cost, has_cov, out, accumulate, tid, nthreads, scratch);
}

template <bool FUSED, int THREADS, bool COHERENT = false>
__device__ __forceinline__ bool p2p_finish(const PassArgs& a, int mode, const double (&dacc)[1], double* s_tot,
                                           double* s_warp) {
  if (!grid_reduce<kP2PRaw, 32, 1, THREADS, COHERENT>(dacc, a, s_tot, s_warp)) return false;
  if constexpr (COHERENT) {
    return false;
  } else {
    const bool has_cov = a.cost->has_cov != 0;
    if (mode == PASS_COST) {
      if (threadIdx.x == 0) {
        const int e = packed_size(6) - 1;
        a.out->v[e] = a.accumulate ? a.out->v[e] + s_tot[22] : s_tot[22];
      }
    } else {
      __shared__ double s_jl[FUSED ? 9 : 1];
      __shared__ double s_jaff[FUSED ? 4 : 1][18];
      const double(*jaff)[18] = FUSED ? s_jaff : a.pb->jaff;
      if constexpr (FUSED) {
        if (threadIdx.x == 0) {
          double xl[6];
#pragma unroll
          for (int i = 0; i < 6; ++i) xl[i] = a.x.v[i];
          p2p_fused_left_jacobian(a.cost, xl, s_jl);
        }
        __syncthreads();
        for (int i = threadIdx.x; i < 4 * 18; i += THREADS) s_jaff[i / 18][i % 18] = p2p_affine_entry(a.cost->variant, s_jl, i / 18, i % 18);
        __syncthreads();
      }
      __shared__ double s_asm[21 * 16];
      p2p_assemble(s_tot, jaff, a.cost, has_cov, a.out, a.accumulate, threadIdx.x, THREADS, s_asm);
    }
    peer_push(a, packed_size(6));
    return true;
  }
}

template <int THREADS>
__device__ __forceinline__ void p2p_master_tail(const PassArgs& a, int mode, PassResult* out) {
  static_assert(THREADS >= 4 * 18, "one ParamBlock::jaff entry per thread");
  __shared__ double s_tot[32];
  __shared__ double s_jaff[4][18];
  __shared__ double s_asm[21 * 16];
  const int G = int(gridDim.x) - 1;
  const bool has_cov = a.cost->has_cov != 0;
  if (mode != PASS_COST) {
    if (threadIdx.x < 4 * 18) (&s_jaff[0][0])[threadIdx.x] = __ldcg(&a.pb->jaff[0][0] + threadIdx.x);
    __syncthreads();
    p2p_assemble_inner(s_jaff, a.cost, has_cov, threadIdx.x, THREADS, s_asm);
  }
  if (threadIdx.x == 0) {
    while (*reinterpret_cast<volatile unsigned int*>(a.ticket) != unsigned(G)) {}
  }
  __syncthreads();
  __threadfence();
  grid_final_reduce<kP2PRaw, THREADS>(a.partials, G, s_tot);
  if (threadIdx.x == 0) *a.ticket = 0u;
  __syncthreads();
  if (mode == PASS_COST) {
    if (threadIdx.x == 0) {
      const int e = packed_size(6) - 1;
      out->v[e] = a.accumulate ? out->v[e] + s_tot[22] : s_tot[22];
    }
  } else {
    p2p_assemble_outer(s_tot, s_jaff, a.cost, has_cov, out, a.accumulate, threadIdx.x, THREADS, s_asm);
  }
}

template <typename ST, typename CT, int LOSS, bool QROT, int THREADS, int UNROLL, int FLUSH_ROUNDS, int PF, bool SWP,
          bool FUSED, bool COHERENT>
__device__ __forceinline__ bool p2p_moment_body(const PassArgs& a, const int mode, const double* rt = nullptr) {
  const int bid = COHERENT ? int(blockIdx.x) - 1 : int(blockIdx.x);
  const int nb = COHERENT ? int(gridDim.x) - 1 : int(gridDim.x);
  constexpr int VEC = VecOf<ST>::N;
  constexpr bool kFp32Acc = (sizeof(CT) == 4);

  __shared__ double s_warp[(THREADS / 32) * 32];
  __shared__ double s_tot[32];

  __shared__ double s_set0[FUSED ? 12 : 1];
  const double* set0 = FUSED ? s_set0 : (COHERENT ? rt : a.pb->sets[0]);
  if constexpr (FUSED) {
    if (threadIdx.x == 0) {
      double xl[6];
#pragma unroll
      for (int i = 0; i < 6; ++i) xl[i] = a.x.v[i];
      p2p_fused_set0(a.cost, xl, s_set0);
    }
    __syncthreads();
  }
  CT R[9], t[3];
#pragma unroll
  for (int i = 0; i < 9; ++i) R[i] = CT(set0[i]);
#pragma unroll
  for (int i = 0; i < 3; ++i) t[i] = CT(set0[9 + i]);
  const CT lossp = CT(a.cost->loss_param);
  const bool masked = a.masked != 0;

  const ST* __restrict__ sx = static_cast<const ST*>(a.streams.p[0]);
  const ST* __restrict__ sy = static_cast<const ST*>(a.streams.p[1]);
  const ST* __restrict__ sz = static_cast<const ST*>(a.streams.p[2]);
  const ST* __restrict__ tx = static_cast<const ST*>(a.streams.p[3]);
  const ST* __restrict__ ty = static_cast<const ST*>(a.streams.p[4]);
  const ST* __restrict__ tz = static_cast<const ST*>(a.streams.p[5]);

  CT acc[32];
#pragma unroll
  for (int i = 0; i < 32; ++i) acc[i] = CT(0);
  double dacc[1] = {0.0};

  const int64_t ngroups = a.n / VEC;
  const int64_t stride = int64_t(nb) * THREADS;
  const int64_t full_rounds = ngroups / stride;
  const int64_t g0 = int64_t(bid) * THREADS + threadIdx.x;

  auto flush = [&]() {
// ... 740 lines not shown
```

moptimizer_0_b200/csrc/mopt_pass_p2p2.cu:

```cuda
#include "mopt_internal.h"
#include "mopt_pass_p2p2.cuh"

namespace mopt {
namespace {

struct ShapeGen2 {
  static constexpr int THREADS = 384, STAGES = 2, U = 2, FLUSH = 16;
};

template <int LOSS, bool QROT, bool MASKED, bool FUSED, class S>
int launch_gen2_one(const PassLaunch& L, const PassArgs& a0) {
  auto kern = p2p_moment2_kernel<LOSS, QROT, MASKED, FUSED, S::THREADS, 1, S::STAGES, S::U, S::FLUSH, 0>;
  constexpr size_t smem = p2p2_ring_bytes(S::THREADS, S::STAGES, S::U);
  static bool configured[64] = {false};
  int dev = 0;
  MOPT_CUDA_TRY(cudaGetDevice(&dev));
  if (dev < 0 || dev >= 64 || !configured[dev]) {
    MOPT_CUDA_TRY(cudaFuncSetAttribute(kern, cudaFuncAttributeMaxDynamicSharedMemorySize, int(smem)));
    if (dev >= 0 && dev < 64) configured[dev] = true;
  }
  PassArgs a = a0;
  for (int k = 0; k < 6; ++k)
    if (reinterpret_cast<uintptr_t>(a.streams.p[k]) & 15u) a.no_ring = 1;
  const int64_t groups = a.n / 4;
  int64_t grid = int64_t(L.ctas_per_sm > 0 ? L.ctas_per_sm : 1) * L.num_sms;
  if (grid > L.num_sms) grid = L.num_sms;
  const int64_t need = (groups + S::THREADS - 1) / S::THREADS;
  if (need < grid) grid = need;
  if (grid < 1) grid = 1;
  kern<<<int(grid), S::THREADS, smem, L.stream>>>(a);
  MOPT_CUDA_TRY(cudaGetLastError());
  return MOPT_OK;
}

template <int LOSS, bool QROT, class S>
int launch_gen2_flags(const PassLaunch& L, const PassArgs& a) {
  if (a.masked)
    return a.fused_setup ? launch_gen2_one<LOSS, QROT, true, true, S>(L, a) : launch_gen2_one<LOSS, QROT, true, false, S>(L, a);
  return a.fused_setup ? launch_gen2_one<LOSS, QROT, false, true, S>(L, a) : launch_gen2_one<LOSS, QROT, false, false, S>(L, a);
}

template <class S>
int launch_gen2(const PassLaunch& L, int loss, bool qrot, const PassArgs& a) {
  switch (loss) {
    case MOPT_LOSS_NONE:
      return qrot ? launch_gen2_flags<MOPT_LOSS_NONE, true, S>(L, a) : launch_gen2_flags<MOPT_LOSS_NONE, false, S>(L, a);
    case MOPT_LOSS_GEMAN_MCCLURE:
      return qrot ? launch_gen2_flags<MOPT_LOSS_GEMAN_MCCLURE, true, S>(L, a)
                  : launch_gen2_flags<MOPT_LOSS_GEMAN_MCCLURE, false, S>(L, a);
    case MOPT_LOSS_HUBER:
      return qrot ? launch_gen2_flags<MOPT_LOSS_HUBER, true, S>(L, a) : launch_gen2_flags<MOPT_LOSS_HUBER, false, S>(L, a);
    default:
      set_last_error("unknown loss kind");
      return MOPT_ERR_INVALID_ARGUMENT;
  }
}

}

int launch_p2p_moment_gen2(const PassLaunch& L, int loss, bool qrot, const PassArgs& a) {
  return launch_gen2<ShapeGen2>(L, loss, qrot, a);
}

}
```

moptimizer_0_b200/csrc/mopt_pass_p2p2.cuh:

```cuda
#pragma once

#include "mopt_pass.cuh"

namespace mopt {
#ifdef __CUDACC__

__device__ __forceinline__ float2 bc2(float a) { return make_float2(a, a); }
__device__ __forceinline__ float2 neg2(float2 a) { return make_float2(-a.x, -a.y); }
__device__ __forceinline__ float2 fma2(float2 a, float2 b, float2 c) { return __ffma2_rn(a, b, c); }
__device__ __forceinline__ float2 add2(float2 a, float2 b) { return __fadd2_rn(a, b); }
__device__ __forceinline__ float2 sub2(float2 a, float2 b) { return __fadd2_rn(a, neg2(b)); }
__device__ __forceinline__ float2 mul2(float2 a, float2 b) { return __fmul2_rn(a, b); }

__device__ __forceinline__ unsigned smem_u32(const void* p) { return static_cast<unsigned>(__cvta_generic_to_shared(p)); }
__device__ __forceinline__ void mbar_init(uint64_t* bar, unsigned count) {
  asm volatile("mbarrier.init.shared::cta.b64 [%0], %1;" ::"r"(smem_u32(bar)), "r"(count) : "memory");
}
__device__ __forceinline__ void mbar_expect_tx(uint64_t* bar, unsigned bytes) {
  asm volatile("mbarrier.arrive.expect_tx.shared::cta.b64 _, [%0], %1;" ::"r"(smem_u32(bar)), "r"(bytes) : "memory");
}
__device__ __forceinline__ void mbar_arrive(uint64_t* bar) {
  asm volatile("mbarrier.arrive.shared::cta.b64 _, [%0];" ::"r"(smem_u32(bar)) : "memory");
}
__device__ __forceinline__ void mbar_wait(uint64_t* bar, unsigned parity) {
  asm volatile(
      "{\n"
      ".reg .pred p;\n"
      "MOPT_WAIT:\n"
      "mbarrier.try_wait.parity.shared::cta.b64 p, [%0], %1;\n"
      "@p bra MOPT_DONE;\n"
      "bra MOPT_WAIT;\n"
      "MOPT_DONE:\n"
      "}\n" ::"r"(smem_u32(bar)),
      "r"(parity)
      : "memory");
}
__device__ __forceinline__ void bulk_g2s(void* dst, const void* src, unsigned bytes, uint64_t* bar) {
  asm volatile("cp.async.bulk.shared::cluster.global.mbarrier::complete_tx::bytes [%0], [%1], %2, [%3];" ::"r"(smem_u32(dst)),
               "l"(src), "r"(bytes), "r"(smem_u32(bar))
               : "memory");
}

template <int LOSS>
__device__ __forceinline__ float loss_weight_fast(float k, float e2) {
  if constexpr (LOSS == MOPT_LOSS_HUBER) {
    float rs;
    asm("rsqrt.approx.ftz.f32 %0, %1;" : "=f"(rs) : "f"(fmaxf(e2, 1.17549435e-38f)));
    return (e2 <= k * k) ? 1.0f : k * rs;
  } else {
    return loss_weight<float>(LOSS, k, e2);
  }
}

template <int LOSS, bool QROT, bool MASKED>
__device__ __forceinline__ void p2p_moments_x2(const float (&R)[9], const float (&t)[3], float lossp, float2 px, float2 py,
                                               float2 pz, float2 yx, float2 yy, float2 yz, float2 (&acc)[kP2PRaw]) {
  bool skip0 = false, skip1 = false;
  if constexpr (MASKED) {
    skip0 = yx.x != yx.x; skip1 = yx.y != yx.y;
    if (skip0) { px.x = py.x = pz.x = 0.f; yx.x = t[0]; yy.x = t[1]; yz.x = t[2]; }
    if (skip1) { px.y = py.y = pz.y = 0.f; yx.y = t[0]; yy.y = t[1]; yz.y = t[2]; }
  }
  const float2 q0 = fma2(px, bc2(R[0]), fma2(py, bc2(R[1]), mul2(pz, bc2(R[2]))));
  const float2 q1 = fma2(px, bc2(R[3]), fma2(py, bc2(R[4]), mul2(pz, bc2(R[5]))));
  const float2 q2 = fma2(px, bc2(R[6]), fma2(py, bc2(R[7]), mul2(pz, bc2(R[8]))));
  const float2 r0 = sub2(add2(q0, bc2(t[0])), yx);
  const float2 r1 = sub2(add2(q1, bc2(t[1])), yy);
  const float2 r2 = sub2(add2(q2, bc2(t[2])), yz);
  const float2 e2 = fma2(r0, r0, fma2(r1, r1, mul2(r2, r2)));
  float2 w;
  w.x = loss_weight_fast<LOSS>(lossp, e2.x);
  w.y = loss_weight_fast<LOSS>(lossp, e2.y);
  if constexpr (MASKED) {
    if (skip0) w.x = 0.f;
    if (skip1) w.y = 0.f;
  }
  const float2 a0 = QROT ? q0 : px, a1 = QROT ? q1 : py, a2 = QROT ? q2 : pz;
  const float2 w0 = mul2(w, a0), w1 = mul2(w, a1), w2 = mul2(w, a2);
  acc[0] = add2(acc[0], w);
  acc[1] = add2(acc[1], w0); acc[2] = add2(acc[2], w1); acc[3] = add2(acc[3], w2);
  acc[4] = fma2(w0, a0, acc[4]); acc[5] = fma2(w0, a1, acc[5]); acc[6] = fma2(w0, a2, acc[6]);
  acc[7] = fma2(w1, a1, acc[7]); acc[8] = fma2(w1, a2, acc[8]); acc[9] = fma2(w2, a2, acc[9]);
  acc[10] = fma2(w, r0, acc[10]); acc[11] = fma2(w, r1, acc[11]); acc[12] = fma2(w, r2, acc[12]);
  acc[13] = fma2(w0, r0, acc[13]); acc[14] = fma2(w0, r1, acc[14]); acc[15] = fma2(w0, r2, acc[15]);
  acc[16] = fma2(w1, r0, acc[16]); acc[17] = fma2(w1, r1, acc[17]); acc[18] = fma2(w1, r2, acc[18]);
  acc[19] = fma2(w2, r0, acc[19]); acc[20] = fma2(w2, r1, acc[20]); acc[21] = fma2(w2, r2, acc[21]);
  acc[22] = add2(acc[22], e2);
}

template <bool MASKED>
__device__ __forceinline__ void p2p_cost_x2(const float (&R)[9], const float (&t)[3], float2 px, float2 py, float2 pz,
                                            float2 yx, float2 yy, float2 yz, float2 (&acc)[kP2PRaw]) {
  const float2 r0 = sub2(add2(fma2(px, bc2(R[0]), fma2(py, bc2(R[1]), mul2(pz, bc2(R[2])))), bc2(t[0])), yx);
  const float2 r1 = sub2(add2(fma2(px, bc2(R[3]), fma2(py, bc2(R[4]), mul2(pz, bc2(R[5])))), bc2(t[1])), yy);
  const float2 r2 = sub2(add2(fma2(px, bc2(R[6]), fma2(py, bc2(R[7]), mul2(pz, bc2(R[8])))), bc2(t[2])), yz);
  float2 e2 = fma2(r0, r0, fma2(r1, r1, mul2(r2, r2)));
  if constexpr (MASKED) {
    if (yx.x != yx.x) e2.x = 0.f;
    if (yx.y != yx.y) e2.y = 0.f;
  }
  acc[22] = add2(acc[22], e2);
}

constexpr size_t p2p2_ring_bytes(int threads, int stages, int u) { return size_t(stages) * 6 * size_t(u) * threads * 16; }

template <int LOSS, bool QROT, bool MASKED, bool FUSED, int THREADS, int MINB, int STAGES, int U, int FLUSH_ROUNDS,
          int PF = 0>
__global__ void __launch_bounds__(THREADS, MINB) p2p_moment2_kernel(const PassArgs a) {
  const int mode = a.mode_override >= 0 ? a.mode_override : *a.mode_ptr;
  if (mode == PASS_SKIP) return;
  if (peer_failed(a)) return;
  constexpr int NW = THREADS / 32;
  constexpr int CHUNK = THREADS * U;

  __shared__ double s_warp[NW * 32];
  __shared__ double s_tot[32];
  __shared__ double s_set0[FUSED ? 12 : 1];
  __shared__ __align__(8) uint64_t s_full[STAGES > 0 ? STAGES : 1];
  __shared__ __align__(8) uint64_t s_empty[STAGES > 0 ? STAGES : 1];
  extern __shared__ __align__(128) unsigned char p2p2_ring[];
  float4* ring = reinterpret_cast<float4*>(p2p2_ring);

  const int lane = threadIdx.x & 31;
  const double* set0 = FUSED ? s_set0 : a.pb->sets[0];
  if constexpr (FUSED) {
    if (threadIdx.x == 0) {
      double xl[6];
#pragma unroll
      for (int i = 0; i < 6; ++i) xl[i] = a.x.v[i];
      p2p_fused_set0(a.cost, xl, s_set0);
    }
  }
  if constexpr (STAGES > 0) {
    if (threadIdx.x == 0) {
#pragma unroll
      for (int s = 0; s < STAGES; ++s) {
        mbar_init(&s_full[s], 1);
        mbar_init(&s_empty[s], NW);
      }
      asm volatile("fence.mbarrier_init.release.cluster;" ::: "memory");
    }
  }
  if constexpr (FUSED || STAGES > 0) __syncthreads();

  const float* __restrict__ sp[6];
#pragma unroll
  for (int k = 0; k < 6; ++k) sp[k] = static_cast<const float*>(a.streams.p[k]);

  const int64_t ngroups = a.n / 4;
  const int64_t stride = int64_t(gridDim.x) * CHUNK;
  const int64_t full_rounds = (STAGES > 0 && a.no_ring) ? 0 : ngroups / stride;

  auto issue_to = [&](int64_t rr, int s) {
    const int64_t g = rr * stride + int64_t(blockIdx.x) * CHUNK;
    mbar_expect_tx(&s_full[s], 6u * CHUNK * 16u);
#pragma unroll
    for (int k = 0; k < 6; ++k)
      bulk_g2s(ring + (size_t(s) * 6 + k) * CHUNK, reinterpret_cast<const float4*>(sp[k]) + g, CHUNK * 16u, &s_full[s]);
  };
  if constexpr (STAGES > 0) {
    if (threadIdx.x == 0)
      for (int rr = 0; rr < STAGES && rr < full_rounds; ++rr) issue_to(rr, rr);
  }
  auto prefetch_round = [&](int64_t rr) {
    if (PF > 0 && threadIdx.x == 0 && rr < full_rounds) {
      const int64_t g = rr * stride + int64_t(blockIdx.x) * CHUNK;
#pragma unroll
      for (int k = 0; k < 6; ++k) l2_prefetch_bulk(reinterpret_cast<const float4*>(sp[k]) + g, CHUNK * 16u);
    }
  };
  if constexpr (STAGES == 0 && PF > 0)
    for (int64_t rr = 0; rr < PF; ++rr) prefetch_round(rr);

  float R[9], t[3];
#pragma unroll
  for (int i = 0; i < 9; ++i) R[i] = float(set0[i]);
#pragma unroll
  for (int i = 0; i < 3; ++i) t[i] = float(set0[9 + i]);
  const float lossp = float(a.cost->loss_param);

  float2 acc[kP2PRaw];
#pragma unroll
  for (int i = 0; i < kP2PRaw; ++i) acc[i] = make_float2(0.f, 0.f);
  double dacc[1] = {0.0};

  auto flush = [&]() {
    float s[32];
#pragma unroll
    for (int i = 0; i < kP2PRaw; ++i) s[i] = acc[i].x + acc[i].y;
#pragma unroll
    for (int i = kP2PRaw; i < 32; ++i) s[i] = 0.f;
    const float v = warp_reduce_transpose<32>(s);
    dacc[0] += double(v);
#pragma unroll
    for (int i = 0; i < kP2PRaw; ++i) acc[i] = make_float2(0.f, 0.f);
  };

  auto consume = [&](const float4 (&v)[6]) {
    if (mode == PASS_COST) {
      p2p_cost_x2<MASKED>(R, t, make_float2(v[0].x, v[0].y), make_float2(v[1].x, v[1].y), make_float2(v[2].x, v[2].y),
                          make_float2(v[3].x, v[3].y), make_float2(v[4].x, v[4].y), make_float2(v[5].x, v[5].y), acc);
      p2p_cost_x2<MASKED>(R, t, make_float2(v[0].z, v[0].w), make_float2(v[1].z, v[1].w), make_float2(v[2].z, v[2].w),
                          make_float2(v[3].z, v[3].w), make_float2(v[4].z, v[4].w), make_float2(v[5].z, v[5].w), acc);
    } else {
      p2p_moments_x2<LOSS, QROT, MASKED>(R, t, lossp, make_float2(v[0].x, v[0].y), make_float2(v[1].x, v[1].y),
                                         make_float2(v[2].x, v[2].y), make_float2(v[3].x, v[3].y),
                                         make_float2(v[4].x, v[4].y), make_float2(v[5].x, v[5].y), acc);
      p2p_moments_x2<LOSS, QROT, MASKED>(R, t, lossp, make_float2(v[0].z, v[0].w), make_float2(v[1].z, v[1].w),
                                         make_float2(v[2].z, v[2].w), make_float2(v[3].z, v[3].w),
                                         make_float2(v[4].z, v[4].w), make_float2(v[5].z, v[5].w), acc);
    }
  };
  auto direct_group = [&](int64_t g) {
    float4 v[6];
#pragma unroll
    for (int k = 0; k < 6; ++k) v[k] = ld_stream(reinterpret_cast<const float4*>(sp[k]) + g);
    consume(v);
  };

  int since_flush = 0;
  if constexpr (STAGES > 0) {
    int s = 0;
    unsigned ph = 0;
    const float4* st = ring + threadIdx.x;
    for (int64_t r = 0; r < full_rounds; ++r) {
      mbar_wait(&s_full[s], ph);
      float4 v[U][6];
#pragma unroll
      for (int u = 0; u < U; ++u)
#pragma unroll
        for (int k = 0; k < 6; ++k) v[u][k] = st[(s * 6 + k) * CHUNK + u * THREADS];
      __syncwarp();
      if (lane == 0) mbar_arrive(&s_empty[s]);
      if (threadIdx.x == 0 && r + STAGES < full_rounds) {
        mbar_wait(&s_empty[s], ph);
        issue_to(r + STAGES, s);
      }
#pragma unroll
      for (int u = 0; u < U; ++u) consume(v[u]);
      if (++since_flush >= FLUSH_ROUNDS) {
        flush();
        since_flush = 0;
      }
      if (++s == STAGES) {
        s = 0;
        ph ^= 1u;
      }
    }
  } else {
    for (int64_t r = 0; r < full_rounds; ++r) {
      if (PF > 0) prefetch_round(r + PF);
      const int64_t g = r * stride + int64_t(blockIdx.x) * CHUNK + threadIdx.x;
      float4 v[U][6];
#pragma unroll
      for (int u = 0; u < U; ++u)
#pragma unroll
        for (int k = 0; k < 6; ++k) v[u][k] = ld_stream(reinterpret_cast<const float4*>(sp[k]) + g + u * THREADS);
#pragma unroll
      for (int u = 0; u < U; ++u) consume(v[u]);
      if (++since_flush >= FLUSH_ROUNDS) {
        flush();
        since_flush = 0;
      }
    }
  }
  {
    for (int64_t g = full_rounds * stride + int64_t(blockIdx.x) * THREADS + threadIdx.x; g < ngroups;
         g += int64_t(gridDim.x) * THREADS) {
      direct_group(g);
      if (++since_flush >= FLUSH_ROUNDS) {
        flush();
        since_flush = 0;
      }
    }
    if (blockIdx.x == 0 && threadIdx.x == 0) {
      for (int64_t i = ngroups * 4; i < a.n; ++i) {
        float2 one[kP2PRaw];
#pragma unroll
        for (int k = 0; k < kP2PRaw; ++k) one[k] = make_float2(0.f, 0.f);
        const float2 px = make_float2(sp[0][i], 0.f), py = make_float2(sp[1][i], 0.f), pz = make_float2(sp[2][i], 0.f);
        const float2 yx = make_float2(sp[3][i], t[0]), yy = make_float2(sp[4][i], t[1]), yz = make_float2(sp[5][i], t[2]);
        if (mode == PASS_COST) p2p_cost_x2<MASKED>(R, t, px, py, pz, yx, yy, yz, one);
        else p2p_moments_x2<LOSS, QROT, MASKED>(R, t, lossp, px, py, pz, yx, yy, yz, one);
#pragma unroll
        for (int k = 0; k < kP2PRaw; ++k) acc[k].x += one[k].x;
      }
    }
  }
  flush();
  p2p_finish<FUSED, THREADS>(a, mode, dacc, s_tot, s_warp);
}

#endif
}
```

moptimizer_0_b200/csrc/mopt_setup.cuh:

```cuda
#pragma once

#include "mopt_common.cuh"

namespace mopt {

constexpr double kSo3GuardF64 = 10.0 * 2.220446049250313e-16;
constexpr double kSo3GuardF32 = 10.0 * 1.1920928955078125e-07;
__device__ inline double so3_norm2_dev(const double w[3]) {
  return __fma_rn(w[2], w[2], __fma_rn(w[1], w[1], __dmul_rn(w[0], w[0])));
}
__device__ inline double so3_hat_entry(const double v[3], int i, int j) {
  if (i == j) return 0.0;
  const int k = 3 - i - j;
  const double x = k == 0 ? v[0] : (k == 1 ? v[1] : v[2]);
  return ((j - i + 3) % 3 == 1) ? -x : x;
}
__device__ inline double so3_hat2_entry(const double v[3], int r, int c) {
  return __fma_rn(so3_hat_entry(v, r, 2), so3_hat_entry(v, 2, c),
                  __fma_rn(so3_hat_entry(v, r, 1), so3_hat_entry(v, 1, c),
                           __dmul_rn(so3_hat_entry(v, r, 0), so3_hat_entry(v, 0, c))));
}
__device__ inline double so3_exp_entry(const double a[3], double sn, double cs, int r, int c) {
  const double omc = __dsub_rn(1.0, cs);
  return __dadd_rn(r == c ? 1.0 : 0.0, __fma_rn(sn, so3_hat_entry(a, r, c), __dmul_rn(omc, so3_hat2_entry(a, r, c))));
// ... 260 lines not shown
  if (lane == 0) {
    for (int i = 0; i < P; ++i) pb->x[i] = x[i];
    if (c.model == MOPT_MODEL_POINT2POINT && c.jacobian == MOPT_JAC_ANALYTICAL) setup_p2p_affine(c, x, pb->jaff);
    if (c.model == MOPT_MODEL_POINT2POINT && c.jacobian != MOPT_JAC_ANALYTICAL) {
      const bool central = (c.jacobian == MOPT_JAC_CENTRAL);
      for (int k = 0; k < 4; ++k)
        for (int i = 0; i < 18; ++i) pb->jaff[k][i] = 0.0;
      for (int j = 0; j < P; ++j) {
        const double* sp = pb->sets[1 + j];
        const double* sm = central ? pb->sets[1 + P + j] : pb->sets[0];
        const double inv = 1.0 / (central ? 2.0 * pb->h[j] : pb->h[j]);
        for (int r = 0; r < 3; ++r) {
          const double dt = f32 ? double(float(sp[9 + r])) - double(float(sm[9 + r])) : sp[9 + r] - sm[9 + r];
          pb->jaff[0][r * 6 + j] = dt * inv;
          for (int k = 0; k < 3; ++k) {
            const double dr = f32 ? double(float(sp[r * 3 + k])) - double(float(sm[r * 3 + k])) : sp[r * 3 + k] - sm[r * 3 + k];
            pb->jaff[k + 1][r * 6 + j] = dr * inv;
          }
        }
      }
    }
  }
}

__device__ inline double p2p_affine_entry(int variant, const double* Jl, int k, int idx) {
  int r = idx / 6, col = idx % 6;
  if (variant == MOPT_P2P_REFTEST_COLMAJOR) {
    const int cc = idx / 3, rr = idx % 3;
    r = rr; col = cc;
  }
  if (k == 0) return (col < 3 && r == col) ? 1.0 : 0.0;
  if (col < 3) return 0.0;
  const double E[3][9] = {{0, 0, 0, 0, 0, 1, 0, -1, 0}, {0, 0, -1, 0, 0, 0, 1, 0, 0}, {0, 1, 0, -1, 0, 0, 0, 0, 0}};
  double s = 0.0;
  for (int m = 0; m < 3; ++m) s += E[k - 1][r * 3 + m] * Jl[m * 3 + (col - 3)];
  return s;
}

__device__ inline void setup_p2p_analytical_warp(const CostDev& c, const double* x, ParamBlock* pb, int lane, double* Jl,
                                                 const SetupEarlyOpen* early) {
  const bool f32 = (c.compute_dtype == MOPT_F32);
  double xs[6];
#pragma unroll
  for (int i = 0; i < 6; ++i) xs[i] = f32 ? double(float(x[i])) : x[i];
  const double w[3] = {xs[3], xs[4], xs[5]};
  const double wj[3] = {x[3], x[4], x[5]};
  double R[9], J[9], A, B;
  so3_exp_jl_warp(w, wj, c.so3_guard, lane, R, A, B);
  if (early && early->rt_words) {
    const int idx = lane >> 1;
    double v = R[0];
#pragma unroll
    for (int i = 1; i < 9; ++i) v = (idx == i) ? R[i] : v;
    v = (idx == 9) ? xs[0] : (idx == 10 ? xs[1] : (idx == 11 ? xs[2] : v));
    publish_rt(early->rt_words, early->value, v, lane);
    if (lane == 0) {
      *early->opened = 1;
      if (early->prof) early->prof[11] = clock64();
    }
  }
#pragma unroll
  for (int i = 0; i < 9; ++i) J[i] = (i % 4 == 0) ? 1.0 : 0.0;
  if (c.variant == MOPT_P2P_EXACT) so3_left_jacobian_entries(wj, A, B, J);
  if (lane < 9) {
    double v = R[0];
#pragma unroll
    for (int i = 1; i < 9; ++i) v = (lane == i) ? R[i] : v;
    pb->sets[0][lane] = v;
    double j = J[0];
#pragma unroll
    for (int i = 1; i < 9; ++i) j = (lane == i) ? J[i] : j;
    Jl[lane] = j;
  } else if (lane < 12) {
    pb->sets[0][lane] = lane == 9 ? xs[0] : (lane == 10 ? xs[1] : xs[2]);
  } else if (lane < kSetSize) {
    pb->sets[0][lane] = 0.0;
  }
  if (lane < c.P) pb->x[lane] = x[lane];
  __syncwarp();
  for (int i = lane; i < 4 * 18; i += 32) pb->jaff[i / 18][i % 18] = p2p_affine_entry(c.variant, Jl, i / 18, i % 18);
  __syncwarp();
}

}
```

moptimizer_0_b200/csrc/mopt_store.cu:

```cuda
#include <cstring>

#include "mopt_internal.h"

using namespace mopt;

namespace {

template <typename HT, typename ST>
__global__ void deinterleave_kernel(const HT* __restrict__ aos, int64_t stride, int ncomp, ST* __restrict__ s0,
                                    ST* __restrict__ s1, ST* __restrict__ s2, int64_t first, int64_t count) {
  for (int64_t i = int64_t(blockIdx.x) * blockDim.x + threadIdx.x; i < count; i += int64_t(gridDim.x) * blockDim.x) {
    const HT* e = aos + i * stride;
    s0[first + i] = ST(e[0]);
    if (ncomp > 1) s1[first + i] = ST(e[1]);
    if (ncomp > 2) s2[first + i] = ST(e[2]);
  }
}

template <typename HT, typename ST>
__global__ void interleave_kernel(HT* __restrict__ aos, int ncomp, const ST* __restrict__ s0, const ST* __restrict__ s1,
                                  const ST* __restrict__ s2, int64_t first, int64_t count) {
  for (int64_t i = int64_t(blockIdx.x) * blockDim.x + threadIdx.x; i < count; i += int64_t(gridDim.x) * blockDim.x) {
    HT* e = aos + i * ncomp;
    e[0] = HT(s0[first + i]);
// ... 64 lines not shown
    float p[3];
    for (int k = 0; k < 3; ++k) p[k] = d.lo[k] + (d.hi[k] - d.lo[k]) * u01(d.seed, gi, k);
    float w[3];
    for (int k = 0; k < 3; ++k) w[k] = d.gt[k * 4 + 0] * p[0] + d.gt[k * 4 + 1] * p[1] + d.gt[k * 4 + 2] * p[2] + d.gt[k * 4 + 3];
    float uu = w[0] / w[2], vv = w[1] / w[2];
    if (d.distort) {
      const float xn = uu, yn = vv, r2 = xn * xn + yn * yn;
      const float radial = 1.0f + r2 * (d.gt[16] + r2 * (d.gt[17] + r2 * d.gt[20]));
      const float xy2 = 2.0f * xn * yn;
      const float xd = xn * radial + d.gt[18] * xy2 + d.gt[19] * (r2 + 2.0f * xn * xn);
      const float yd = yn * radial + d.gt[18] * (r2 + 2.0f * yn * yn) + d.gt[19] * xy2;
      uu = d.gt[12] * xd + d.gt[14];
      vv = d.gt[13] * yd + d.gt[15];
    }
    if (d.sigma > 0.0f) {
      uu += d.sigma * approx_normal(d.seed, gi, 3);
      vv += d.sigma * approx_normal(d.seed, gi, 7);
    }
    X[i] = ST(p[0]); Y[i] = ST(p[1]); Z[i] = ST(p[2]);
    u[i] = ST(uu); v[i] = ST(vv);
  }
}

size_t dtype_size(int dt) { return dt == MOPT_F32 ? 4 : 8; }

void rodrigues_host(const double* w, double* R) {
  const double n = std::sqrt(w[0] * w[0] + w[1] * w[1] + w[2] * w[2]);
  for (int i = 0; i < 9; ++i) R[i] = (i % 4 == 0) ? 1.0 : 0.0;
  if (n > 0.0) {
    const double a[3] = {w[0] / n, w[1] / n, w[2] / n};
    const double K[9] = {0, -a[2], a[1], a[2], 0, -a[0], -a[1], a[0], 0};
    const double s = std::sin(n), c = std::cos(n);
    for (int r = 0; r < 3; ++r)
      for (int col = 0; col < 3; ++col) {
        double kk = 0;
        for (int k = 0; k < 3; ++k) kk += K[r * 3 + k] * K[k * 3 + col];
        R[r * 3 + col] += s * K[r * 3 + col] + (1.0 - c) * kk;
      }
  }
}

int ensure_stage(mopt_ctx* ctx, size_t bytes) {
  if (ctx->stage_bytes >= bytes) return MOPT_OK;
  for (int i = 0; i < 2; ++i) {
    if (ctx->d_stage[i]) cudaFree(ctx->d_stage[i]);
    ctx->d_stage[i] = nullptr;
  }
  ctx->stage_bytes = 0;
  for (int i = 0; i < 2; ++i) MOPT_CUDA_TRY(cudaMalloc(&ctx->d_stage[i], bytes));
  ctx->stage_bytes = bytes;
  return MOPT_OK;
}

template <typename HT, typename ST>
void launch_deinterleave(cudaStream_t s, const void* aos, int64_t stride, int ncomp, void* const* streams, int64_t first,
                         int64_t count) {
  const int threads = 256;
  int64_t blocks = (count + threads - 1) / threads;
  if (blocks > 148 * 16) blocks = 148 * 16;
  if (blocks < 1) blocks = 1;
  deinterleave_kernel<HT, ST><<<int(blocks), threads, 0, s>>>(static_cast<const HT*>(aos), stride, ncomp,
                                                             static_cast<ST*>(streams[0]), static_cast<ST*>(streams[1]),
                                                             static_cast<ST*>(streams[2]), first, count);
}

template <typename HT, typename ST>
void launch_interleave(cudaStream_t s, void* aos, int ncomp, void* const* streams, int64_t first, int64_t count) {
  const int threads = 256;
  int64_t blocks = (count + threads - 1) / threads;
  if (blocks > 148 * 16) blocks = 148 * 16;
  if (blocks < 1) blocks = 1;
  interleave_kernel<HT, ST><<<int(blocks), threads, 0, s>>>(static_cast<HT*>(aos), ncomp, static_cast<const ST*>(streams[0]),
                                                           static_cast<const ST*>(streams[1]),
                                                           static_cast<const ST*>(streams[2]), first, count);
}

}

namespace mopt {

int store_upload_async(mopt_store* st, int group, const void* host, int host_dtype, int64_t host_stride, int64_t first,
                       int64_t count) {
  mopt_ctx* ctx = st->ctx;
  const ModelShape sh = model_shape(st->model);
  MOPT_REQUIRE(group == 0 || group == 1, "group must be 0 (A) or 1 (B)");
  const int ncomp = group == 0 ? sh.ncomp_a : sh.ncomp_b;
  MOPT_REQUIRE(ncomp > 0, "this model has no such data group");
  MOPT_REQUIRE(first >= 0 && count >= 0 && first + count <= st->n, "upload range outside the store");
  MOPT_REQUIRE(host_dtype == MOPT_F32 || host_dtype == MOPT_F64, "bad host dtype");
  if (count == 0) return MOPT_OK;
  MOPT_REQUIRE(host != nullptr, "null host pointer");
  if (host_stride == 0) host_stride = ncomp;
  MOPT_REQUIRE(host_stride >= ncomp, "host stride smaller than the component count");
  void* const* streams = st->streams + (group == 0 ? 0 : sh.NA);
  const size_t hsz = dtype_size(host_dtype);
  const size_t chunk_bytes_target = size_t(64) << 20;
  int64_t chunk_elems = int64_t(chunk_bytes_target / (hsz * size_t(host_stride)));
  if (chunk_elems < 1) chunk_elems = 1;
  if (chunk_elems > count) chunk_elems = count;
  MOPT_TRY(ensure_stage(ctx, size_t(chunk_elems) * size_t(host_stride) * hsz));
  int buf = 0;
  for (int64_t off = 0; off < count; off += chunk_elems, buf ^= 1) {
    const int64_t m = (count - off < chunk_elems) ? (count - off) : chunk_elems;
    const size_t bytes = (size_t(m - 1) * size_t(host_stride) + size_t(ncomp)) * hsz;
    MOPT_CUDA_TRY(cudaStreamWaitEvent(ctx->copy_stream, ctx->ev_free[buf], 0));
    MOPT_CUDA_TRY(cudaMemcpyAsync(ctx->d_stage[buf], static_cast<const char*>(host) + size_t(off) * size_t(host_stride) * hsz,
                                  bytes, cudaMemcpyHostToDevice, ctx->copy_stream));
    MOPT_CUDA_TRY(cudaEventRecord(ctx->ev_copy[buf], ctx->copy_stream));
    MOPT_CUDA_TRY(cudaStreamWaitEvent(ctx->stream, ctx->ev_copy[buf], 0));
    if (host_dtype == MOPT_F32 && st->dtype == MOPT_F32)
      launch_deinterleave<float, float>(ctx->stream, ctx->d_stage[buf], host_stride, ncomp, streams, first + off, m);
    else if (host_dtype == MOPT_F64 && st->dtype == MOPT_F32)
      launch_deinterleave<double, float>(ctx->stream, ctx->d_stage[buf], host_stride, ncomp, streams, first + off, m);
    else if (host_dtype == MOPT_F32 && st->dtype == MOPT_F64)
      launch_deinterleave<float, double>(ctx->stream, ctx->d_stage[buf], host_stride, ncomp, streams, first + off, m);
    else
      launch_deinterleave<double, double>(ctx->stream, ctx->d_stage[buf], host_stride, ncomp, streams, first + off, m);
    MOPT_CUDA_TRY(cudaGetLastError());
    MOPT_CUDA_TRY(cudaEventRecord(ctx->ev_free[buf], ctx->stream));
  }
  return MOPT_OK;
}

}

extern "C" {

int mopt_store_create(mopt_ctx* ctx, int model, int dtype, int64_t n, mopt_store** out) try {
  MOPT_REQUIRE(ctx && out, "null ctx/out");
  const ModelShape sh = model_shape(model);
  MOPT_REQUIRE(sh.P >= 0, "unknown model kind");
  MOPT_REQUIRE(dtype == MOPT_F32 || dtype == MOPT_F64, "store dtype must be MOPT_F32 or MOPT_F64");
  MOPT_REQUIRE(n >= 0, "negative store size");
  MOPT_CUDA_TRY(cudaSetDevice(ctx->device));
  mopt_store* st = new mopt_store();
  st->ctx = ctx;
  st->model = model;
  st->dtype = dtype;
  st->n = n;
  st->nstreams = sh.NS;
  const size_t bytes = ((size_t(n) * dtype_size(dtype) + 255) / 256) * 256 + 256;
  for (int s = 0; s < sh.NS; ++s) {
    cudaError_t e = cudaMalloc(&st->streams[s], bytes);
    if (e != cudaSuccess) {
      set_last_error(std::string("cudaMalloc of a store stream failed: ") + cudaGetErrorString(e));
      for (int k = 0; k < s; ++k) cudaFree(st->streams[k]);
      delete st;
      return e == cudaErrorMemoryAllocation ? MOPT_ERR_OUT_OF_MEMORY : MOPT_ERR_CUDA;
    }
  }
  *out = st;
  return MOPT_OK;
}
MOPT_ABI_CATCH

int mopt_store_destroy(mopt_store* st) try {
  if (!st) return MOPT_OK;
  cudaSetDevice(st->ctx->device);
  cudaStreamSynchronize(st->ctx->stream);
  for (int s = 0; s < st->nstreams; ++s) cudaFree(st->streams[s]);
  delete st;
  return MOPT_OK;
}
MOPT_ABI_CATCH

int mopt_store_size(const mopt_store* st, int64_t* n) try {
  MOPT_REQUIRE(st && n, "null store/n");
  *n = st->n;
  return MOPT_OK;
}
MOPT_ABI_CATCH

int mopt_store_upload(mopt_store* st, int group, const void* host, int host_dtype, int64_t host_stride, int64_t first,
                      int64_t count) try {
  MOPT_REQUIRE(st, "null store");
  MOPT_CUDA_TRY(cudaSetDevice(st->ctx->device));
  MOPT_TRY(store_upload_async(st, group, host, host_dtype, host_stride, first, count));
  MOPT_CUDA_TRY(cudaStreamSynchronize(st->ctx->stream));
  return MOPT_OK;
}
MOPT_ABI_CATCH

int mopt_store_download(mopt_store* st, int group, void* host, int host_dtype, int64_t first, int64_t count) try {
  MOPT_REQUIRE(st && host, "null store/host");
  mopt_ctx* ctx = st->ctx;
  MOPT_CUDA_TRY(cudaSetDevice(ctx->device));
  const ModelShape sh = model_shape(st->model);
  MOPT_REQUIRE(group == 0 || group == 1, "group must be 0 (A) or 1 (B)");
  const int ncomp = group == 0 ? sh.ncomp_a : sh.ncomp_b;
  MOPT_REQUIRE(ncomp > 0, "this model has no such data group");
  MOPT_REQUIRE(first >= 0 && count >= 0 && first + count <= st->n, "download range outside the store");
  MOPT_REQUIRE(host_dtype == MOPT_F32 || host_dtype == MOPT_F64, "bad host dtype");
  void* const* streams = st->streams + (group == 0 ? 0 : sh.NA);
  const size_t hsz = dtype_size(host_dtype);
  const int64_t chunk_elems_max = int64_t((size_t(64) << 20) / (hsz * ncomp));
  const int64_t chunk = count < chunk_elems_max ? count : chunk_elems_max;
  if (count == 0) return MOPT_OK;
  MOPT_TRY(ensure_stage(ctx, size_t(chunk) * ncomp * hsz));
  for (int64_t off = 0; off < count; off += chunk) {
    const int64_t m = (count - off < chunk) ? (count - off) : chunk;
    if (host_dtype == MOPT_F32 && st->dtype == MOPT_F32)
      launch_interleave<float, float>(ctx->stream, ctx->d_stage[0], ncomp, streams, first + off, m);
    else if (host_dtype == MOPT_F64 && st->dtype == MOPT_F32)
      launch_interleave<double, float>(ctx->stream, ctx->d_stage[0], ncomp, streams, first + off, m);
    else if (host_dtype == MOPT_F32 && st->dtype == MOPT_F64)
      launch_interleave<float, double>(ctx->stream, ctx->d_stage[0], ncomp, streams, first + off, m);
    else
      launch_interleave<double, double>(ctx->stream, ctx->d_stage[0], ncomp, streams, first + off, m);
    MOPT_CUDA_TRY(cudaGetLastError());
    MOPT_CUDA_TRY(cudaMemcpyAsync(static_cast<char*>(host) + size_t(off) * ncomp * hsz, ctx->d_stage[0],
                                  size_t(m) * ncomp * hsz, cudaMemcpyDeviceToHost, ctx->stream));
    MOPT_CUDA_TRY(cudaStreamSynchronize(ctx->stream));
  }
  return MOPT_OK;
}
MOPT_ABI_CATCH

int mopt_store_generate(mopt_store* st, const mopt_synth* desc) try {
  MOPT_REQUIRE(st && desc, "null store/desc");
  mopt_ctx* ctx = st->ctx;
  MOPT_CUDA_TRY(cudaSetDevice(ctx->device));
  SynthDev d;
  std::memset(&d, 0, sizeof(d));
  d.seed = desc->seed;
  d.first_index = desc->first_index;
  d.n_total = desc->n_total > 0 ? desc->n_total : st->n;
  for (int k = 0; k < 3; ++k) {
    d.lo[k] = float(desc->lo[k]);
    d.hi[k] = float(desc->hi[k]);
  }
  d.sigma = float(desc->noise_sigma);
  d.outlier_fraction = float(desc->outlier_fraction);
  d.outlier_range = float(desc->outlier_range);
  const int threads = 256;
  int64_t blocks = (st->n + threads - 1) / threads;
  if (blocks > 148 * 16) blocks = 148 * 16;
  if (blocks < 1) blocks = 1;
  const bool f32 = st->dtype == MOPT_F32;
  switch (st->model) {
    case MOPT_MODEL_POINT2POINT:
    case MOPT_MODEL_POINT_DIST: {
      double R[9];
      rodrigues_host(desc->gt + 3, R);
      for (int i = 0; i < 9; ++i) d.gt[i] = float(R[i]);
      for (int i = 0; i < 3; ++i) d.gt[9 + i] = float(desc->gt[i]);
      if (f32)
        generate_p2p_kernel<float><<<int(blocks), threads, 0, ctx->stream>>>(
            d, st->n, (float*)st->streams[0], (float*)st->streams[1], (float*)st->streams[2], (float*)st->streams[3],
            (float*)st->streams[4], (float*)st->streams[5]);
      else
        generate_p2p_kernel<double><<<int(blocks), threads, 0, ctx->stream>>>(
            d, st->n, (double*)st->streams[0], (double*)st->streams[1], (double*)st->streams[2], (double*)st->streams[3],
            (double*)st->streams[4], (double*)st->streams[5]);
      break;
    }
    case MOPT_MODEL_EXP_CURVE: {
      d.gt[0] = float(desc->gt[0]);
      d.gt[1] = float(desc->gt[1]);
      if (f32)
        generate_curve_kernel<float><<<int(blocks), threads, 0, ctx->stream>>>(d, st->n, (float*)st->streams[0],
                                                                               (float*)st->streams[1]);
      else
        generate_curve_kernel<double><<<int(blocks), threads, 0, ctx->stream>>>(d, st->n, (double*)st->streams[0],
                                                                                (double*)st->streams[1]);
      break;
    }
    case MOPT_MODEL_PINHOLE:
    case MOPT_MODEL_PINHOLE_DISTORT: {
      if (st->model == MOPT_MODEL_PINHOLE) {
        for (int i = 0; i < 12; ++i) d.gt[i] = float(desc->gt[i]);
      } else {
        double R[9];
        rodrigues_host(desc->gt + 3, R);
        for (int r = 0; r < 3; ++r)
          for (int col = 0; col < 4; ++col) {
            double s = desc->gt[r] * desc->consts[12 + col];
            for (int k = 0; k < 3; ++k) s += R[r * 3 + k] * desc->consts[k * 4 + col];
            d.gt[r * 4 + col] = float(s);
          }
        for (int i = 0; i < 9; ++i) d.gt[12 + i] = float(desc->gt[6 + i]);
        d.distort = 1;
      }
      if (f32)
        generate_pinhole_kernel<float><<<int(blocks), threads, 0, ctx->stream>>>(
            d, st->n, (float*)st->streams[0], (float*)st->streams[1], (float*)st->streams[2], (float*)st->streams[3],
            (float*)st->streams[4]);
      else
        generate_pinhole_kernel<double><<<int(blocks), threads, 0, ctx->stream>>>(
            d, st->n, (double*)st->streams[0], (double*)st->streams[1], (double*)st->streams[2], (double*)st->streams[3],
            (double*)st->streams[4]);
      break;
    }
    default:
      set_last_error("no synthetic generator for this model");
      return MOPT_ERR_UNSUPPORTED;
  }
  MOPT_CUDA_TRY(cudaGetLastError());
  MOPT_CUDA_TRY(cudaStreamSynchronize(ctx->stream));
  return MOPT_OK;
}
MOPT_ABI_CATCH

}
// ... 1 lines not shown
```

Measured before the change: 289.5.

## Evaluate multiple LM damping candidates per data pass and overlap fused passes via PDL

Adds multi-candidate Levenberg-Marquardt steps for the f32 point-to-point problem. Each data pass also evaluates the cost at extra trial poses (from successive lambda increases) alongside the linearization, so rejected steps need no extra pass. It also adds programmatic dependent launch so a fused-setup pass can overlap the previous kernel's tail. The cost is extra per-point arithmetic, more registers, and more complex LM state handling.

After: 291.3 (median of 6 runs). About the same (+0.6%).

```diff
diff --git a/include/mopt_capi.h b/include/mopt_capi.h
--- a/include/mopt_capi.h
+++ b/include/mopt_capi.h
@@ -106,7 +106,7 @@
   int32_t flags;
   int32_t reserved;
 } mopt_lm_options;
-typedef enum mopt_lm_flags { MOPT_LM_STAGNATION_STOP = 1 } mopt_lm_flags;
+typedef enum mopt_lm_flags { MOPT_LM_STAGNATION_STOP = 1, MOPT_LM_ONE_TRIAL_PER_PASS = 2 } mopt_lm_flags;
 
 typedef struct mopt_lm_trial {
   int32_t outer_iteration, k, accepted, reserved;
diff --git a/moptimizer_0_b200/capi.py b/moptimizer_0_b200/capi.py
--- a/moptimizer_0_b200/capi.py
+++ b/moptimizer_0_b200/capi.py
@@ -21,6 +21,7 @@
 FLAG_STABLE_FD = 2
 FLAG_REFERENCE_FLOAT_GUARD = 4
 LM_STAGNATION_STOP = 1
+LM_ONE_TRIAL_PER_PASS = 2
 LOSS_NONE, LOSS_GEMAN_MCCLURE, LOSS_HUBER = range(3)
 STATUS = ["CONVERGED", "MAXIMUM_ITERATIONS_REACHED", "SMALL_DELTA", "NUMERIC_ERROR", "FATAL_ERROR"]
 MODEL_SHAPE = {
@@ -315,7 +316,7 @@
 
     def lm_minimize(self, stores: Sequence["Store"], problems: Sequence[Problem], x0, max_iterations: int = 15,
                     lm_iterations: int = 3, scalar_dtype: int = F64, speculative: bool = True,
-                    stagnation_stop: bool = True) -> "LmResult":
+                    stagnation_stop: bool = True, one_trial_per_pass: bool = False) -> "LmResult":
         n = len(stores)
         hs = (C.c_void_p * n)(*[s.handle for s in stores])
         ps = (Problem * n)(*problems)
@@ -325,7 +326,7 @@
             lib().mopt_lm_default_options(C.byref(opt))
         opt.max_iterations, opt.lm_max_iterations = max_iterations, lm_iterations
         opt.scalar_dtype, opt.speculative = scalar_dtype, 1 if speculative else 0
-        opt.flags = LM_STAGNATION_STOP if stagnation_stop else 0
+        opt.flags = (LM_STAGNATION_STOP if stagnation_stop else 0) | (LM_ONE_TRIAL_PER_PASS if one_trial_per_pass else 0)
         x = np.array(x0, dtype=np.float64)
         rep = self.__dict__.get("_lm_report")
         if rep is None:
diff --git a/moptimizer_0_b200/csrc/mopt_capi.cu b/moptimizer_0_b200/csrc/mopt_capi.cu
--- a/moptimizer_0_b200/csrc/mopt_capi.cu
+++ b/moptimizer_0_b200/csrc/mopt_capi.cu
@@ -84,6 +84,7 @@
 __global__ void lm_step_kernel(LmState* st, const PassResult* trial, CostSlot* slots, int* flag, const int* xerr, int prof,
                                int P, int scalar_f32) {
   __shared__ LmStepShared s_sh;
+  __shared__ double s_cand[kLmHotWords];
   const int lane = threadIdx.x;
   if (*reinterpret_cast<const volatile int*>(xerr)) {
     if (lane == 0) {
@@ -93,7 +94,9 @@
     return;
   }
   long long stamps[16] = {0};
-  const int done = lm_step_warp(st, trial, slots, &s_sh, lane, P, scalar_f32 != 0, LmStepIo{}, prof ? stamps : nullptr);
+  LmStepIo io;
+  io.cand_scratch = s_cand;
+  const int done = lm_step_warp(st, trial, slots, &s_sh, lane, P, scalar_f32 != 0, io, prof ? stamps : nullptr);
   if (lane == 0) {
     *flag = done;
     if (prof && stamps[3] - stamps[2] > 1000)
@@ -254,8 +257,9 @@
 }
 
 int launch_pass(mopt_ctx* ctx, const mopt_store* st, const mopt_problem* p, int slot, int accumulate, int mode_override,
-                bool push, const XArg* fused_x = nullptr) {
+                bool push, const XArg* fused_x = nullptr, int ncand = 1) {
   PassArgs a = make_args(ctx, st, slot, accumulate, mode_override);
+  a.ncand = ncand;
   if (fused_x) {
     a.fused_setup = 1;
     a.x = *fused_x;
@@ -271,6 +275,7 @@
     a.peer.seq = ++ctx->xseq;
   }
   PassLaunch L{ctx->stream, ctx->num_sms, ctx->ctas_per_sm, ctx->threads};
+  L.overlap_prev = fused_x != nullptr && !a.peer.push && st->pass_may_overlap;
   L.affine_fd = (p->compute_dtype == MOPT_F32) ? !(p->flags & MOPT_FLAG_GENERIC_KERNEL)
                                                : ((p->flags & MOPT_FLAG_STABLE_FD) && !(p->flags & MOPT_FLAG_GENERIC_KERNEL));
   L.identity_cov = !p->has_covariance;
@@ -286,11 +291,12 @@
   return launch_dense(L, p->model, p->jacobian != MOPT_JAC_ANALYTICAL, st->dtype, p->compute_dtype, a);
 }
 
-int allreduce_trial(mopt_ctx* ctx, int P, int mode_override) {
+int allreduce_trial(mopt_ctx* ctx, int P, int mode_override, int ncand = 1) {
   if (ctx->world <= 1 || !ctx->exchange_enabled) return MOPT_OK;
+  const int count = packed_size(P) + ncand - 1;
   if (ctx->peers_open) {
     if (ctx->fused_consumer) return MOPT_OK;
-    peer_reduce_kernel<<<1, 64, 0, ctx->stream>>>(ctx->d_xbuf, ctx->world, ctx->xseq, ctx->d_trial, packed_size(P),
+    peer_reduce_kernel<<<1, 64, 0, ctx->stream>>>(ctx->d_xbuf, ctx->world, ctx->xseq, ctx->d_trial, count,
                                                   &ctx->d_lm->pass_mode, mode_override, ctx->d_xerr, ctx->d_xerr_dev);
     MOPT_CUDA_TRY(cudaGetLastError());
     return MOPT_OK;
@@ -299,7 +305,7 @@
     set_last_error("sharded context has neither a NCCL communicator nor an open peer exchange");
     return MOPT_ERR_COMM;
   }
-  MOPT_NCCL_TRY(nccl().AllReduce(ctx->d_trial, ctx->d_trial, size_t(packed_size(P)), kNcclFloat64, kNcclSum,
+  MOPT_NCCL_TRY(nccl().AllReduce(ctx->d_trial, ctx->d_trial, size_t(count), kNcclFloat64, kNcclSum,
                                  static_cast<NcclApi::comm_t>(ctx->nccl_comm), ctx->stream));
   return MOPT_OK;
 }
@@ -338,6 +344,7 @@
   }
   if (can_fuse_setup(ctx, p, st)) {
     MOPT_TRY(launch_pass(ctx, st, p, 0, 0, mode, true, &xa));
+    st->pass_may_overlap = true;
   } else {
     setup_kernel<<<1, 32, 0, ctx->stream>>>(&ctx->d_slots[0], xa);
     MOPT_CUDA_TRY(cudaGetLastError());
@@ -826,6 +833,19 @@
     }
   }
 
+  {
+    const int env_k = [] {
+      const char* e = getenv("MOPT_LM_CANDIDATES");
+      const int v = (e && e[0]) ? atoi(e) : kLmCandDefault;
+      return v < 1 ? 1 : (v > kMaxLmCand ? kMaxLmCand : v);
+    }();
+    const mopt_problem& p0 = problems[0];
+    if (in.speculative && n_costs == 1 && !any_user_setup && !(opt.flags & MOPT_LM_ONE_TRIAL_PER_PASS) &&
+        p0.model == MOPT_MODEL_POINT2POINT && p0.jacobian == MOPT_JAC_ANALYTICAL && stores[0]->dtype == MOPT_F32 &&
+        p0.compute_dtype == MOPT_F32 && ctx->threads != 1024)
+      in.ncand = env_k;
+  }
+  const int ncand = in.ncand > 1 ? in.ncand : 1;
   MOPT_TRY(launch_init());
   static const bool step_prof = [] { const char* e = getenv("MOPT_LM_MONO_TRACE"); return e && e[0] == '1'; }();
   const int64_t max_slots = int64_t(opt.max_iterations) * (int64_t(opt.lm_max_iterations) + 1) + 2;
@@ -838,8 +858,8 @@
       ctx->h_flags[slot_index(enq)] = 0;
       for (int c = 0; c < n_costs; ++c) MOPT_TRY(enqueue_reassociate(stores[c], &ctx->d_slots[c].pb, ctx->d_lm));
       for (int c = 0; c < n_costs; ++c)
-        MOPT_TRY(launch_pass(ctx, stores[c], &problems[c], c, c > 0 ? 1 : 0, -1, c == n_costs - 1));
-      MOPT_TRY(allreduce_trial(ctx, P, -1));
+        MOPT_TRY(launch_pass(ctx, stores[c], &problems[c], c, c > 0 ? 1 : 0, -1, c == n_costs - 1, nullptr, ncand));
+      MOPT_TRY(allreduce_trial(ctx, P, -1, ncand));
       lm_step_kernel<<<1, 32, 0, ctx->stream>>>(ctx->d_lm, ctx->d_trial, ctx->d_slots, ctx->d_flags + slot_index(enq),
                                                 ctx->d_xerr_dev, step_prof ? 1 : 0, in.P, in.scalar_f32);
       MOPT_CUDA_TRY(cudaGetLastError());
diff --git a/moptimizer_0_b200/csrc/mopt_common.cuh b/moptimizer_0_b200/csrc/mopt_common.cuh
--- a/moptimizer_0_b200/csrc/mopt_common.cuh
+++ b/moptimizer_0_b200/csrc/mopt_common.cuh
@@ -106,7 +106,7 @@
   double v[kPackedMax];
 };
 
-__host__ __device__ inline int packed_size(int P) { return P * (P + 1) / 2 + P + 1; }
+__host__ __device__ constexpr int packed_size(int P) { return P * (P + 1) / 2 + P + 1; }
 __host__ __device__ inline int tri_index(int P, int r, int c) {
   return r * P - r * (r - 1) / 2 + (c - r);
 }
diff --git a/moptimizer_0_b200/csrc/mopt_icp.cu b/moptimizer_0_b200/csrc/mopt_icp.cu
--- a/moptimizer_0_b200/csrc/mopt_icp.cu
+++ b/moptimizer_0_b200/csrc/mopt_icp.cu
@@ -276,6 +276,7 @@
 
 template <typename ST, typename T>
 void launch_reassoc(mopt_store* st, mopt_nn_index* ix, const ParamBlock* pb, const LmState* gate) {
+  st->pass_may_overlap = false;
   GridDesc g;
   for (int k = 0; k < 3; ++k) { g.origin[k] = ix->origin[k]; g.dims[k] = ix->dims[k]; }
   g.inv_cell = 1.0 / ix->cell;
diff --git a/moptimizer_0_b200/csrc/mopt_internal.h b/moptimizer_0_b200/csrc/mopt_internal.h
--- a/moptimizer_0_b200/csrc/mopt_internal.h
+++ b/moptimizer_0_b200/csrc/mopt_internal.h
@@ -58,6 +58,7 @@
   void* streams[mopt::kMaxStreams] = {nullptr};
   struct mopt_nn_index* index = nullptr;
   bool may_have_invalid = false;
+  bool pass_may_overlap = false;
 };
 
 namespace mopt {
@@ -69,6 +70,7 @@
   int threads;
   bool affine_fd = true;
   bool identity_cov = false;
+  bool overlap_prev = false;
 };
 
 int launch_p2p_moment(const PassLaunch& L, int store_dtype, int compute_dtype, int loss, bool qrot, const PassArgs& a);
diff --git a/moptimizer_0_b200/csrc/mopt_lm.cuh b/moptimizer_0_b200/csrc/mopt_lm.cuh
--- a/moptimizer_0_b200/csrc/mopt_lm.cuh
+++ b/moptimizer_0_b200/csrc/mopt_lm.cuh
@@ -8,29 +8,39 @@
 namespace mopt {
 
 enum LmPhase : int { LM_PHASE_LIN = 0, LM_PHASE_TRIAL = 1 };
+
+constexpr int kMaxLmCand = 3;
+constexpr int kLmCandDefault = 3;
+
+struct LmCandidates {
+  double delta[kMaxLmCand - 1][kMaxP], xi[kMaxLmCand - 1][kMaxP];
+};
 
 struct LmState {
   int P, n_costs, max_it, lm_max_it, speculative, scalar_f32;
   double lambda_factor;
   int flags;
-  int pad0_;
+  int ncand;
   double x[kMaxP], xi[kMaxP], delta[kMaxP], x_eval[kMaxP];
   PassResult cur;
   double lambda, nu;
   int it, k, phase, status, done, executed, num_trials, num_passes;
   int pass_mode;
-  int pad_;
+  int cand_ready;
   mopt_lm_trial trials[MOPT_MAX_TRACE];
+  LmCandidates cand;
 };
 
 constexpr int kLmHotWords = int(offsetof(LmState, trials) / 8);
 static_assert(offsetof(LmState, trials) % 8 == 0, "LmState hot part is copied in 8-byte words");
 static_assert(kPackedMax <= 160, "lm_step_warp_t stages the pass result with five loads per lane");
+static_assert(packed_size(6) + kMaxLmCand - 1 <= kPackedMax, "candidate sums follow the packed result of the 6-DoF problem");
 
 struct LmInit {
   int P, n_costs, max_it, lm_max_it, speculative, scalar_f32;
   double lambda_factor;
   int flags;
+  int ncand;
   double x0[kMaxP];
 };
 
@@ -228,18 +238,71 @@
 
 constexpr int kLmCopyTrial = 4;
 template <typename S, int PC = 0>
-__device__ inline int lm_step_thread(LmState* st, const PassResult* trial, const CostDev& cost0, mopt_lm_trial* trials) {
+__device__ inline int lm_outer_start(LmState* st, const PassResult* lin, int copy) {
+  const int P = PC > 0 ? PC : st->P;
+  const int npk = packed_size(P);
+  for (;;) {
+    const S y0 = S(lin->v[npk - 1]);
+    if (is_cost_small<S>(y0)) {
+      lm_finish(st, MOPT_CONVERGED);
+      return copy;
+    }
+    if (st->lambda < 0.0) {
+      S mx = S(0);
+      for (int i = 0; i < P; ++i) mx = fmax(mx, fabs(S(lin->v[tri_index(P, i, i)])));
+      st->lambda = double(S(st->lambda_factor) * mx);
+    }
+    st->nu = 2.0;
+    st->k = 0;
+    if (st->lm_max_it > 0) {
+      return 2 | copy;
+    }
+    st->it += 1;
+    if (st->it >= st->max_it) {
+      lm_finish(st, MOPT_MAXIMUM_ITERATIONS_REACHED);
+      return copy;
+    }
+  }
+}
+
+template <typename S, int PC = 0>
+__device__ inline int lm_reject(LmState* st, S yi) {
+  const int P = PC > 0 ? PC : st->P;
+  S m = S(0);
+  for (int i = 0; i < P; ++i) m = fmax(m, fabs(S(st->delta[i])));
+  if (m < sqrt(scalar_eps<S>())) {
+    lm_finish(st, is_cost_small<S>(yi) ? MOPT_CONVERGED : MOPT_SMALL_DELTA);
+    return 0;
+  }
+  const S lam = S(st->lambda);
+  st->lambda = double(S(st->nu) * lam);
+  st->nu = double(S(2) * S(st->nu));
+  st->k += 1;
+  if (st->k < st->lm_max_it) {
+    return 2;
+  }
+  st->it += 1;
+  if (st->it >= st->max_it) {
+    lm_finish(st, MOPT_MAXIMUM_ITERATIONS_REACHED);
+    return 0;
+  }
+  return lm_outer_start<S, PC>(st, &st->cur, 0);
+}
+
+template <typename S, int PC = 0>
+__device__ inline int lm_step_thread(LmState* st, const PassResult* trial, const CostDev& cost0, mopt_lm_trial* trials,
+                                     int cand = 0) {
   if (st->done) return 0;
   const int P = PC > 0 ? PC : st->P;
   const int npk = packed_size(P);
-  st->num_passes += 1;
+  if (cand == 0) st->num_passes += 1;
   int copy = 0;
   const PassResult* lin = &st->cur;
   if (st->phase == LM_PHASE_LIN) {
     copy = kLmCopyTrial;
     lin = trial;
   } else {
-    const S yi = S(trial->v[npk - 1]);
+    const S yi = S(trial->v[npk - 1 + cand]);
     const S y0 = S(st->cur.v[npk - 1]);
     if (isnan(yi)) {
       lm_finish(st, MOPT_NUMERIC_ERROR);
@@ -259,23 +322,7 @@
     }
     st->num_trials += 1;
     if (rho < S(0)) {
-      S m = S(0);
-      for (int i = 0; i < P; ++i) m = fmax(m, fabs(S(st->delta[i])));
-      if (m < sqrt(scalar_eps<S>())) {
-        lm_finish(st, is_cost_small<S>(yi) ? MOPT_CONVERGED : MOPT_SMALL_DELTA);
-        return 0;
-      }
-      st->lambda = double(S(st->nu) * lam);
-      st->nu = double(S(2) * S(st->nu));
-      st->k += 1;
-      if (st->k < st->lm_max_it) {
-        return 2;
-      }
-      st->it += 1;
-      if (st->it >= st->max_it) {
-        lm_finish(st, MOPT_MAXIMUM_ITERATIONS_REACHED);
-        return 0;
-      }
+      return lm_reject<S, PC>(st, yi);
     } else {
       for (int i = 0; i < P; ++i) st->x[i] = st->xi[i];
       if ((st->flags & MOPT_LM_STAGNATION_STOP) && yi == y0) {
@@ -290,20 +337,21 @@
       const double f = fmax(1.0 / 3.0, 1.0 - v * v * v);
       st->lambda = double(S(double(lam) * f));
       st->it += 1;
+      const bool speculative = st->speculative && cand == 0;
       if (st->it >= st->max_it) {
-        if (st->speculative) {
+        if (speculative) {
           lm_finish(st, MOPT_MAXIMUM_ITERATIONS_REACHED);
           return kLmCopyTrial;
         }
-        st->cur.v[npk - 1] = trial->v[npk - 1];
+        st->cur.v[npk - 1] = trial->v[npk - 1 + cand];
         lm_finish(st, MOPT_MAXIMUM_ITERATIONS_REACHED);
         return 0;
       }
-      if (st->speculative) {
+      if (speculative) {
         copy = kLmCopyTrial;
         lin = trial;
       } else {
-        st->cur.v[npk - 1] = trial->v[npk - 1];
+        st->cur.v[npk - 1] = trial->v[npk - 1 + cand];
         for (int i = 0; i < P; ++i) st->x_eval[i] = st->x[i];
         st->phase = LM_PHASE_LIN;
         st->pass_mode = PASS_LINEARIZE;
@@ -311,28 +359,7 @@
       }
     }
   }
-  for (;;) {
-    const S y0 = S(lin->v[npk - 1]);
-    if (is_cost_small<S>(y0)) {
-      lm_finish(st, MOPT_CONVERGED);
-      return copy;
-    }
-    if (st->lambda < 0.0) {
-      S mx = S(0);
-      for (int i = 0; i < P; ++i) mx = fmax(mx, fabs(S(lin->v[tri_index(P, i, i)])));
-      st->lambda = double(S(st->lambda_factor) * mx);
-    }
-    st->nu = 2.0;
-    st->k = 0;
-    if (st->lm_max_it > 0) {
-      return 2 | copy;
-    }
-    st->it += 1;
-    if (st->it >= st->max_it) {
-      lm_finish(st, MOPT_MAXIMUM_ITERATIONS_REACHED);
-      return copy;
-    }
-  }
+  return lm_outer_start<S, PC>(st, lin, copy);
 }
 
 struct LmStepShared {
@@ -350,6 +377,7 @@
   bool generic_p = false;
   LmState* host_state = nullptr;
   int* host_flag = nullptr;
+  double* cand_scratch = nullptr;
 };
 
 static __device__ __noinline__ void lm_init_warp(LmState* st, CostSlot* slots, const LmInit& in, LmStepShared* sh, int lane,
@@ -358,12 +386,12 @@
     st->P = in.P; st->n_costs = in.n_costs; st->max_it = in.max_it; st->lm_max_it = in.lm_max_it;
     st->speculative = in.speculative; st->scalar_f32 = in.scalar_f32; st->lambda_factor = in.lambda_factor;
     st->flags = in.flags;
-    st->pad0_ = 0;
+    st->ncand = in.ncand > 1 ? in.ncand : 1;
     st->lambda = -1.0; st->nu = 2.0;
     st->it = 0; st->k = 0; st->phase = LM_PHASE_LIN; st->status = MOPT_MAXIMUM_ITERATIONS_REACHED;
     st->done = 0; st->executed = 0; st->num_trials = 0; st->num_passes = 0;
     st->pass_mode = PASS_LINEARIZE;
-    st->pad_ = 0;
+    st->cand_ready = 1;
   }
   if (lane < kMaxP) {
     const double v = lane < in.P ? (in.scalar_f32 ? double(float(in.x0[lane])) : in.x0[lane]) : 0.0;
@@ -375,6 +403,38 @@
   const double* x = resident ? st->x_eval : sh->hot;
   for (int c = 0; c < in.n_costs; ++c)
     setup_cost((c == 0 && cost0) ? *cost0 : slots[c].cost, x, &slots[c].pb, lane, 32, sh->sc.tmp);
+}
+
+template <typename S, int PC>
+__device__ inline int lm_propose_candidates(LmState* st, LmState* gst, CostSlot* slots, const CostDev& cost0,
+                                            LmStepShared* sh, LmState* sc, int lane, int P) {
+  int cands = 1;
+  LmState* target = st;
+  for (;;) {
+    lm_solve_propose_warp<S, PC>(target, cost0, &sh->sc, lane);
+    __syncwarp();
+    if (target != st) {
+      if (lane < P) {
+        gst->cand.delta[cands - 2][lane] = target->delta[lane];
+        gst->cand.xi[cands - 2][lane] = target->xi[lane];
+      }
+      setup_p2p_rt_warp(cost0, target->x_eval, slots[0].pb.sets[cands - 1], lane);
+      __syncwarp();
+    } else {
+      double* w = reinterpret_cast<double*>(sc);
+      for (int i = lane; i < kLmHotWords; i += 32) w[i] = sh->hot[i];
+      target = sc;
+      __syncwarp();
+    }
+    if (cands == st->ncand) break;
+    int r = 0;
+    if (lane == 0) r = lm_reject<S, PC>(sc, S(0));
+    r = __shfl_sync(0xffffffffu, r, 0);
+    __syncwarp();
+    if (r != 2) break;
+    ++cands;
+  }
+  return cands;
 }
 
 template <typename S, int PC>
@@ -382,7 +442,9 @@
                                      int P_rt, const LmStepIo& io, long long* prof = nullptr) {
   LmState* st = reinterpret_cast<LmState*>(sh->hot);
   if (prof && lane == 0) prof[0] = clock64();
-  const int npk = packed_size(PC > 0 ? PC : P_rt);
+  const int P = PC > 0 ? PC : P_rt;
+  const int npk = packed_size(P);
+  const int nst = npk + kMaxLmCand - 1 < kPackedMax ? npk + kMaxLmCand - 1 : kPackedMax;
   {
     const double* g = reinterpret_cast<const double*>(gst);
     constexpr int kPerLane = (kLmHotWords + 31) / 32;
@@ -393,11 +455,11 @@
     }
     double tr0 = 0.0, tr1 = 0.0, tr2 = 0.0, tr3 = 0.0, tr4 = 0.0;
     if (!io.trial_staged) {
-      if (lane < npk) tr0 = __ldcg(&gtrial->v[lane]);
-      if (lane + 32 < npk) tr1 = __ldcg(&gtrial->v[lane + 32]);
-      if (lane + 64 < npk) tr2 = __ldcg(&gtrial->v[lane + 64]);
-      if (lane + 96 < npk) tr3 = __ldcg(&gtrial->v[lane + 96]);
-      if (lane + 128 < npk) tr4 = __ldcg(&gtrial->v[lane + 128]);
+      if (lane < nst) tr0 = __ldcg(&gtrial->v[lane]);
+      if (lane + 32 < nst) tr1 = __ldcg(&gtrial->v[lane + 32]);
+      if (lane + 64 < nst) tr2 = __ldcg(&gtrial->v[lane + 64]);
+      if (lane + 96 < nst) tr3 = __ldcg(&gtrial->v[lane + 96]);
+      if (lane + 128 < nst) tr4 = __ldcg(&gtrial->v[lane + 128]);
     }
     if (io.load_state) {
 #pragma unroll
@@ -405,11 +467,11 @@
         if (lane + 32 * q < kLmHotWords) sh->hot[lane + 32 * q] = tmp[q];
     }
     if (!io.trial_staged) {
-      if (lane < npk) sh->trial.v[lane] = tr0;
-      if (lane + 32 < npk) sh->trial.v[lane + 32] = tr1;
-      if (lane + 64 < npk) sh->trial.v[lane + 64] = tr2;
-      if (lane + 96 < npk) sh->trial.v[lane + 96] = tr3;
-      if (lane + 128 < npk) sh->trial.v[lane + 128] = tr4;
+      if (lane < nst) sh->trial.v[lane] = tr0;
+      if (lane + 32 < nst) sh->trial.v[lane + 32] = tr1;
+      if (lane + 64 < nst) sh->trial.v[lane + 64] = tr2;
+      if (lane + 96 < nst) sh->trial.v[lane + 96] = tr3;
+      if (lane + 128 < nst) sh->trial.v[lane + 128] = tr4;
     }
   }
   __syncwarp();
@@ -419,16 +481,35 @@
   if (lane == 0) act = lm_step_thread<S, PC>(st, &sh->trial, cost0, io.host_state ? io.host_state->trials : gst->trials);
   act = __shfl_sync(0xffffffffu, act, 0);
   __syncwarp();
+  const int ready = st->cand_ready;
+  for (int j = 1; act == 2 && j < ready; ++j) {
+    if (lane < P) {
+      const double xi = gst->cand.xi[j - 1][lane];
+      st->delta[lane] = gst->cand.delta[j - 1][lane];
+      st->xi[lane] = xi;
+      st->x_eval[lane] = xi;
+    }
+    __syncwarp();
+    if (lane == 0) act = lm_step_thread<S, PC>(st, &sh->trial, cost0, io.host_state ? io.host_state->trials : gst->trials, j);
+    act = __shfl_sync(0xffffffffu, act, 0);
+    __syncwarp();
+  }
   if (act & kLmCopyTrial) {
     for (int i = lane; i < npk; i += 32) st->cur.v[i] = sh->trial.v[i];
     __syncwarp();
     act &= ~kLmCopyTrial;
   }
   if (prof && lane == 0) prof[2] = clock64();
+  int cands = 1;
   if (act == 2) {
-    lm_solve_propose_warp<S, PC>(st, cost0, &sh->sc, lane, prof);
-    __syncwarp();
-  }
+    if (io.cand_scratch != nullptr && st->ncand > 1) {
+      cands = lm_propose_candidates<S, PC>(st, gst, slots, cost0, sh, reinterpret_cast<LmState*>(io.cand_scratch), lane, P);
+    } else {
+      lm_solve_propose_warp<S, PC>(st, cost0, &sh->sc, lane, prof);
+      __syncwarp();
+    }
+  }
+  if (lane == 0) st->cand_ready = cands;
   if (prof && lane == 0) prof[3] = clock64();
   if (act) {
     const int nc = st->n_costs;
diff --git a/moptimizer_0_b200/csrc/mopt_pass.cuh b/moptimizer_0_b200/csrc/mopt_pass.cuh
--- a/moptimizer_0_b200/csrc/mopt_pass.cuh
+++ b/moptimizer_0_b200/csrc/mopt_pass.cuh
@@ -36,6 +36,7 @@
   int fused_setup;
   int no_ring;
   XArg x;
+  int ncand;
 };
 
 #ifdef __CUDACC__
@@ -292,10 +293,10 @@
   p2p_assemble_outer(tot, jaff, cost, has_cov, out, accumulate, tid, nthreads, scratch);
 }
 
-template <bool FUSED, int THREADS, bool COHERENT = false>
+template <bool FUSED, int THREADS, bool COHERENT = false, int NC = 1>
 __device__ __forceinline__ bool p2p_finish(const PassArgs& a, int mode, const double (&dacc)[1], double* s_tot,
                                            double* s_warp) {
-  if (!grid_reduce<kP2PRaw, 32, 1, THREADS, COHERENT>(dacc, a, s_tot, s_warp)) return false;
+  if (!grid_reduce<kP2PRaw + NC - 1, 32, 1, THREADS, COHERENT>(dacc, a, s_tot, s_warp)) return false;
   if constexpr (COHERENT) {
     return false;
   } else {
@@ -323,7 +324,11 @@
       __shared__ double s_asm[21 * 16];
       p2p_assemble(s_tot, jaff, a.cost, has_cov, a.out, a.accumulate, threadIdx.x, THREADS, s_asm);
     }
-    peer_push(a, packed_size(6));
+    if (NC > 1 && threadIdx.x < NC - 1) {
+      const int e = packed_size(6) + threadIdx.x;
+      a.out->v[e] = a.accumulate ? a.out->v[e] + s_tot[kP2PRaw + threadIdx.x] : s_tot[kP2PRaw + threadIdx.x];
+    }
+    peer_push(a, packed_size(6) + NC - 1);
     return true;
   }
 }
diff --git a/moptimizer_0_b200/csrc/mopt_pass_p2p2.cu b/moptimizer_0_b200/csrc/mopt_pass_p2p2.cu
--- a/moptimizer_0_b200/csrc/mopt_pass_p2p2.cu
+++ b/moptimizer_0_b200/csrc/mopt_pass_p2p2.cu
@@ -8,9 +8,11 @@
   static constexpr int THREADS = 384, STAGES = 2, U = 2, FLUSH = 16;
 };
 
-template <int LOSS, bool QROT, bool MASKED, bool FUSED, class S>
+template <int LOSS, bool QROT, bool MASKED, bool FUSED, class S, int NC = 1>
 int launch_gen2_one(const PassLaunch& L, const PassArgs& a0) {
-  auto kern = p2p_moment2_kernel<LOSS, QROT, MASKED, FUSED, S::THREADS, 1, S::STAGES, S::U, S::FLUSH, 0>;
+  void (*kern)(const PassArgs);
+  if constexpr (NC == 1) kern = p2p_moment2_kernel<LOSS, QROT, MASKED, FUSED, S::THREADS, 1, S::STAGES, S::U, S::FLUSH, 0>;
+  else kern = p2p_moment2_cand_kernel<LOSS, QROT, MASKED, S::THREADS, 1, S::STAGES, S::U, S::FLUSH, NC>;
   constexpr size_t smem = p2p2_ring_bytes(S::THREADS, S::STAGES, S::U);
   static bool configured[64] = {false};
   int dev = 0;
@@ -28,13 +30,40 @@
   const int64_t need = (groups + S::THREADS - 1) / S::THREADS;
   if (need < grid) grid = need;
   if (grid < 1) grid = 1;
+  if (FUSED && L.overlap_prev) {
+    cudaLaunchConfig_t cfg = {};
+    cfg.gridDim = dim3(unsigned(grid));
+    cfg.blockDim = dim3(S::THREADS);
+    cfg.dynamicSmemBytes = smem;
+    cfg.stream = L.stream;
+    cudaLaunchAttribute attr[1];
+    attr[0].id = cudaLaunchAttributeProgrammaticStreamSerialization;
+    attr[0].val.programmaticStreamSerializationAllowed = 1;
+    cfg.attrs = attr;
+    cfg.numAttrs = 1;
+    MOPT_CUDA_TRY(cudaLaunchKernelEx(&cfg, kern, a));
+    return MOPT_OK;
+  }
   kern<<<int(grid), S::THREADS, smem, L.stream>>>(a);
   MOPT_CUDA_TRY(cudaGetLastError());
   return MOPT_OK;
 }
 
+template <int LOSS, bool QROT, bool MASKED, class S>
+int launch_gen2_cand(const PassLaunch& L, const PassArgs& a) {
+  switch (a.ncand) {
+    case 2: return launch_gen2_one<LOSS, QROT, MASKED, false, S, 2>(L, a);
+    case 3: return launch_gen2_one<LOSS, QROT, MASKED, false, S, 3>(L, a);
+    default:
+      set_last_error("point2point: unsupported number of LM candidates per pass");
+      return MOPT_ERR_INVALID_ARGUMENT;
+  }
+}
+
 template <int LOSS, bool QROT, class S>
 int launch_gen2_flags(const PassLaunch& L, const PassArgs& a) {
+  if (a.ncand > 1 && !a.fused_setup)
+    return a.masked ? launch_gen2_cand<LOSS, QROT, true, S>(L, a) : launch_gen2_cand<LOSS, QROT, false, S>(L, a);
   if (a.masked)
     return a.fused_setup ? launch_gen2_one<LOSS, QROT, true, true, S>(L, a) : launch_gen2_one<LOSS, QROT, true, false, S>(L, a);
   return a.fused_setup ? launch_gen2_one<LOSS, QROT, false, true, S>(L, a) : launch_gen2_one<LOSS, QROT, false, false, S>(L, a);
diff --git a/moptimizer_0_b200/csrc/mopt_pass_p2p2.cuh b/moptimizer_0_b200/csrc/mopt_pass_p2p2.cuh
--- a/moptimizer_0_b200/csrc/mopt_pass_p2p2.cuh
+++ b/moptimizer_0_b200/csrc/mopt_pass_p2p2.cuh
@@ -90,7 +90,7 @@
 
 template <bool MASKED>
 __device__ __forceinline__ void p2p_cost_x2(const float (&R)[9], const float (&t)[3], float2 px, float2 py, float2 pz,
-                                            float2 yx, float2 yy, float2 yz, float2 (&acc)[kP2PRaw]) {
+                                            float2 yx, float2 yy, float2 yz, float2& sum) {
   const float2 r0 = sub2(add2(fma2(px, bc2(R[0]), fma2(py, bc2(R[1]), mul2(pz, bc2(R[2])))), bc2(t[0])), yx);
   const float2 r1 = sub2(add2(fma2(px, bc2(R[3]), fma2(py, bc2(R[4]), mul2(pz, bc2(R[5])))), bc2(t[1])), yy);
   const float2 r2 = sub2(add2(fma2(px, bc2(R[6]), fma2(py, bc2(R[7]), mul2(pz, bc2(R[8])))), bc2(t[2])), yz);
@@ -99,14 +99,15 @@
     if (yx.x != yx.x) e2.x = 0.f;
     if (yx.y != yx.y) e2.y = 0.f;
   }
-  acc[22] = add2(acc[22], e2);
+  sum = add2(sum, e2);
 }
 
 constexpr size_t p2p2_ring_bytes(int threads, int stages, int u) { return size_t(stages) * 6 * size_t(u) * threads * 16; }
 
-template <int LOSS, bool QROT, bool MASKED, bool FUSED, int THREADS, int MINB, int STAGES, int U, int FLUSH_ROUNDS,
-          int PF = 0>
-__global__ void __launch_bounds__(THREADS, MINB) p2p_moment2_kernel(const PassArgs a) {
+template <int LOSS, bool QROT, bool MASKED, bool FUSED, int THREADS, int STAGES, int U, int FLUSH_ROUNDS, int PF, int NC>
+__device__ __forceinline__ void p2p_moment2_body(const PassArgs a) {
+  static_assert(NC >= 1 && kP2PRaw + NC - 1 <= 32 && !(FUSED && NC > 1), "candidate sums ride in the free lanes of the 32-wide reduction");
+  constexpr int NX = NC - 1, NXA = NX > 0 ? NX : 1;
   const int mode = a.mode_override >= 0 ? a.mode_override : *a.mode_ptr;
   if (mode == PASS_SKIP) return;
   if (peer_failed(a)) return;
@@ -123,6 +124,32 @@
 
   const int lane = threadIdx.x & 31;
   const double* set0 = FUSED ? s_set0 : a.pb->sets[0];
+  const float* __restrict__ sp[6];
+#pragma unroll
+  for (int k = 0; k < 6; ++k) sp[k] = static_cast<const float*>(a.streams.p[k]);
+
+  const int64_t ngroups = a.n / 4;
+  const int64_t stride = int64_t(gridDim.x) * CHUNK;
+  const int64_t full_rounds = (STAGES > 0 && a.no_ring) ? 0 : ngroups / stride;
+
+  auto issue_to = [&](int64_t rr, int s) {
+    const int64_t g = rr * stride + int64_t(blockIdx.x) * CHUNK;
+    mbar_expect_tx(&s_full[s], 6u * CHUNK * 16u);
+#pragma unroll
+    for (int k = 0; k < 6; ++k)
+      bulk_g2s(ring + (size_t(s) * 6 + k) * CHUNK, reinterpret_cast<const float4*>(sp[k]) + g, CHUNK * 16u, &s_full[s]);
+  };
+  if constexpr (STAGES > 0) {
+    if (threadIdx.x == 0) {
+#pragma unroll
+      for (int s = 0; s < STAGES; ++s) {
+        mbar_init(&s_full[s], 1);
+        mbar_init(&s_empty[s], NW);
+      }
+      asm volatile("fence.mbarrier_init.release.cluster;" ::: "memory");
+      for (int rr = 0; rr < STAGES && rr < full_rounds; ++rr) issue_to(rr, rr);
+    }
+  }
   if constexpr (FUSED) {
     if (threadIdx.x == 0) {
       double xl[6];
@@ -131,37 +158,8 @@
       p2p_fused_set0(a.cost, xl, s_set0);
     }
   }
-  if constexpr (STAGES > 0) {
-    if (threadIdx.x == 0) {
-#pragma unroll
-      for (int s = 0; s < STAGES; ++s) {
-        mbar_init(&s_full[s], 1);
-        mbar_init(&s_empty[s], NW);
-      }
-      asm volatile("fence.mbarrier_init.release.cluster;" ::: "memory");
-    }
-  }
   if constexpr (FUSED || STAGES > 0) __syncthreads();
 
-  const float* __restrict__ sp[6];
-#pragma unroll
-  for (int k = 0; k < 6; ++k) sp[k] = static_cast<const float*>(a.streams.p[k]);
-
-  const int64_t ngroups = a.n / 4;
-  const int64_t stride = int64_t(gridDim.x) * CHUNK;
-  const int64_t full_rounds = (STAGES > 0 && a.no_ring) ? 0 : ngroups / stride;
-
-  auto issue_to = [&](int64_t rr, int s) {
-    const int64_t g = rr * stride + int64_t(blockIdx.x) * CHUNK;
-    mbar_expect_tx(&s_full[s], 6u * CHUNK * 16u);
-#pragma unroll
-    for (int k = 0; k < 6; ++k)
-      bulk_g2s(ring + (size_t(s) * 6 + k) * CHUNK, reinterpret_cast<const float4*>(sp[k]) + g, CHUNK * 16u, &s_full[s]);
-  };
-  if constexpr (STAGES > 0) {
-    if (threadIdx.x == 0)
-      for (int rr = 0; rr < STAGES && rr < full_rounds; ++rr) issue_to(rr, rr);
-  }
   auto prefetch_round = [&](int64_t rr) {
     if (PF > 0 && threadIdx.x == 0 && rr < full_rounds) {
       const int64_t g = rr * stride + int64_t(blockIdx.x) * CHUNK;
@@ -178,6 +176,16 @@
 #pragma unroll
   for (int i = 0; i < 3; ++i) t[i] = float(set0[9 + i]);
   const float lossp = float(a.cost->loss_param);
+  float cR[NXA][9], ct[NXA][3];
+  float2 cacc[NXA];
+#pragma unroll
+  for (int j = 0; j < NX; ++j) {
+#pragma unroll
+    for (int i = 0; i < 9; ++i) cR[j][i] = float(a.pb->sets[1 + j][i]);
+#pragma unroll
+    for (int i = 0; i < 3; ++i) ct[j][i] = float(a.pb->sets[1 + j][9 + i]);
+    cacc[j] = make_float2(0.f, 0.f);
+  }
 
   float2 acc[kP2PRaw];
 #pragma unroll
@@ -189,19 +197,23 @@
 #pragma unroll
     for (int i = 0; i < kP2PRaw; ++i) s[i] = acc[i].x + acc[i].y;
 #pragma unroll
-    for (int i = kP2PRaw; i < 32; ++i) s[i] = 0.f;
+    for (int j = 0; j < NX; ++j) s[kP2PRaw + j] = cacc[j].x + cacc[j].y;
+#pragma unroll
+    for (int i = kP2PRaw + NX; i < 32; ++i) s[i] = 0.f;
     const float v = warp_reduce_transpose<32>(s);
     dacc[0] += double(v);
 #pragma unroll
     for (int i = 0; i < kP2PRaw; ++i) acc[i] = make_float2(0.f, 0.f);
+#pragma unroll
+    for (int j = 0; j < NX; ++j) cacc[j] = make_float2(0.f, 0.f);
   };
 
   auto consume = [&](const float4 (&v)[6]) {
     if (mode == PASS_COST) {
       p2p_cost_x2<MASKED>(R, t, make_float2(v[0].x, v[0].y), make_float2(v[1].x, v[1].y), make_float2(v[2].x, v[2].y),
-                          make_float2(v[3].x, v[3].y), make_float2(v[4].x, v[4].y), make_float2(v[5].x, v[5].y), acc);
+                          make_float2(v[3].x, v[3].y), make_float2(v[4].x, v[4].y), make_float2(v[5].x, v[5].y), acc[22]);
       p2p_cost_x2<MASKED>(R, t, make_float2(v[0].z, v[0].w), make_float2(v[1].z, v[1].w), make_float2(v[2].z, v[2].w),
-                          make_float2(v[3].z, v[3].w), make_float2(v[4].z, v[4].w), make_float2(v[5].z, v[5].w), acc);
+                          make_float2(v[3].z, v[3].w), make_float2(v[4].z, v[4].w), make_float2(v[5].z, v[5].w), acc[22]);
     } else {
       p2p_moments_x2<LOSS, QROT, MASKED>(R, t, lossp, make_float2(v[0].x, v[0].y), make_float2(v[1].x, v[1].y),
                                          make_float2(v[2].x, v[2].y), make_float2(v[3].x, v[3].y),
@@ -209,6 +221,15 @@
       p2p_moments_x2<LOSS, QROT, MASKED>(R, t, lossp, make_float2(v[0].z, v[0].w), make_float2(v[1].z, v[1].w),
                                          make_float2(v[2].z, v[2].w), make_float2(v[3].z, v[3].w),
                                          make_float2(v[4].z, v[4].w), make_float2(v[5].z, v[5].w), acc);
+    }
+#pragma unroll
+    for (int j = 0; j < NX; ++j) {
+      p2p_cost_x2<MASKED>(cR[j], ct[j], make_float2(v[0].x, v[0].y), make_float2(v[1].x, v[1].y),
+                          make_float2(v[2].x, v[2].y), make_float2(v[3].x, v[3].y), make_float2(v[4].x, v[4].y),
+                          make_float2(v[5].x, v[5].y), cacc[j]);
+      p2p_cost_x2<MASKED>(cR[j], ct[j], make_float2(v[0].z, v[0].w), make_float2(v[1].z, v[1].w),
+                          make_float2(v[2].z, v[2].w), make_float2(v[3].z, v[3].w), make_float2(v[4].z, v[4].w),
+                          make_float2(v[5].z, v[5].w), cacc[j]);
     }
   };
   auto direct_group = [&](int64_t g) {
@@ -280,15 +301,36 @@
         for (int k = 0; k < kP2PRaw; ++k) one[k] = make_float2(0.f, 0.f);
         const float2 px = make_float2(sp[0][i], 0.f), py = make_float2(sp[1][i], 0.f), pz = make_float2(sp[2][i], 0.f);
         const float2 yx = make_float2(sp[3][i], t[0]), yy = make_float2(sp[4][i], t[1]), yz = make_float2(sp[5][i], t[2]);
-        if (mode == PASS_COST) p2p_cost_x2<MASKED>(R, t, px, py, pz, yx, yy, yz, one);
+        if (mode == PASS_COST) p2p_cost_x2<MASKED>(R, t, px, py, pz, yx, yy, yz, one[22]);
         else p2p_moments_x2<LOSS, QROT, MASKED>(R, t, lossp, px, py, pz, yx, yy, yz, one);
 #pragma unroll
         for (int k = 0; k < kP2PRaw; ++k) acc[k].x += one[k].x;
-      }
-    }
+#pragma unroll
+        for (int j = 0; j < NX; ++j) {
+          float2 c1 = make_float2(0.f, 0.f);
+          p2p_cost_x2<MASKED>(cR[j], ct[j], px, py, pz, yx, yy, yz, c1);
+          cacc[j].x += c1.x;
+        }
+      }
+    }
+  }
+  if constexpr (FUSED) {
+    asm volatile("griddepcontrol.launch_dependents;" ::: "memory");
+    asm volatile("griddepcontrol.wait;" ::: "memory");
   }
   flush();
-  p2p_finish<FUSED, THREADS>(a, mode, dacc, s_tot, s_warp);
+  p2p_finish<FUSED, THREADS, false, NC>(a, mode, dacc, s_tot, s_warp);
+}
+
+template <int LOSS, bool QROT, bool MASKED, bool FUSED, int THREADS, int MINB, int STAGES, int U, int FLUSH_ROUNDS,
+          int PF = 0>
+__global__ void __launch_bounds__(THREADS, MINB) p2p_moment2_kernel(const PassArgs a) {
+  p2p_moment2_body<LOSS, QROT, MASKED, FUSED, THREADS, STAGES, U, FLUSH_ROUNDS, PF, 1>(a);
+}
+
+template <int LOSS, bool QROT, bool MASKED, int THREADS, int MINB, int STAGES, int U, int FLUSH_ROUNDS, int NC>
+__global__ void __launch_bounds__(THREADS, MINB) p2p_moment2_cand_kernel(const PassArgs a) {
+  p2p_moment2_body<LOSS, QROT, MASKED, false, THREADS, STAGES, U, FLUSH_ROUNDS, 0, NC>(a);
 }
 
 #endif
diff --git a/moptimizer_0_b200/csrc/mopt_setup.cuh b/moptimizer_0_b200/csrc/mopt_setup.cuh
--- a/moptimizer_0_b200/csrc/mopt_setup.cuh
+++ b/moptimizer_0_b200/csrc/mopt_setup.cuh
@@ -366,4 +366,25 @@
   __syncwarp();
 }
 
-}
+__device__ inline void setup_p2p_rt_warp(const CostDev& c, const double* x, double* set, int lane) {
+  const bool f32 = (c.compute_dtype == MOPT_F32);
+  double xs[6];
+#pragma unroll
+  for (int i = 0; i < 6; ++i) xs[i] = f32 ? double(float(x[i])) : x[i];
+  const double w[3] = {xs[3], xs[4], xs[5]};
+  const double wj[3] = {x[3], x[4], x[5]};
+  double R[9], A, B;
+  so3_exp_jl_warp(w, wj, c.so3_guard, lane, R, A, B);
+  if (lane < 9) {
+    double v = R[0];
+#pragma unroll
+    for (int i = 1; i < 9; ++i) v = (lane == i) ? R[i] : v;
+    set[lane] = v;
+  } else if (lane < 12) {
+    set[lane] = lane == 9 ? xs[0] : (lane == 10 ? xs[1] : xs[2]);
+  } else if (lane < kSetSize) {
+    set[lane] = 0.0;
+  }
+}
+
+}
diff --git a/moptimizer_0_b200/csrc/mopt_store.cu b/moptimizer_0_b200/csrc/mopt_store.cu
--- a/moptimizer_0_b200/csrc/mopt_store.cu
+++ b/moptimizer_0_b200/csrc/mopt_store.cu
@@ -170,6 +170,7 @@
 int store_upload_async(mopt_store* st, int group, const void* host, int host_dtype, int64_t host_stride, int64_t first,
                        int64_t count) {
   mopt_ctx* ctx = st->ctx;
+  st->pass_may_overlap = false;
   const ModelShape sh = model_shape(st->model);
   MOPT_REQUIRE(group == 0 || group == 1, "group must be 0 (A) or 1 (B)");
   const int ncomp = group == 0 ? sh.ncomp_a : sh.ncomp_b;
@@ -307,6 +308,7 @@
 int mopt_store_generate(mopt_store* st, const mopt_synth* desc) try {
   MOPT_REQUIRE(st && desc, "null store/desc");
   mopt_ctx* ctx = st->ctx;
+  st->pass_may_overlap = false;
   MOPT_CUDA_TRY(cudaSetDevice(ctx->device));
   SynthDev d;
   std::memset(&d, 0, sizeof(d));
```
